# LinjianMa/pairwise-perturbation

Measured on AMD Instinct MI355X. Metric: ALS sweeps/sec (exact dimension-tree sweep, CP order-4 s=200 R=10), higher is better.
Workload: dtype f32

## Files before the change

__graft_entry__.py:

```python
import os
import subprocess
import sys

ROOT = os.path.dirname(os.path.abspath(__file__))
PKG = os.path.join(ROOT, "pairwise-perturbation_amd")


def _run(cmd, **kw):
    print("+", " ".join(cmd), flush=True)
    subprocess.check_call(cmd, **kw)


def build():
    jobs = str(min(8, os.cpu_count() or 1))
    _run(["make", "-j", jobs, "-C", PKG, "ARCH=gfx950"])
    _run(["make", "-C", os.path.join(ROOT, "oracle")])
    if os.path.isdir("/root/reference"):
        _run(["make", "-C", os.path.join(ROOT, "oracle"), "ref"])
    _run(["make", "-C", os.path.join(ROOT, "tests", "hostsim")])
    _run(["make", "-j", jobs, "-C", os.path.join(ROOT, "tests", "hipsim"), "ARCH=gfx950"])
    _run(["make", "-C", os.path.join(ROOT, "tests", "opshim")])
    _run(["make", "-C", os.path.join(ROOT, "tests", "slices_shim")])
    _run(["make", "-C", os.path.join(ROOT, "tests", "polar_shim")])
    _run(["make", "-C", os.path.join(ROOT, "tests", "shape_shim")])
    _run(["make", "-C", os.path.join(ROOT, "tests", "huber_shim")])
    _run(["make", "-C", os.path.join(ROOT, "tests", "parafac2_shim")])
    sys.path.insert(0, PKG)
    import ppals
    lib = ppals.lib()
    missing = [s for s in ppals.EXPORTS if not hasattr(lib, s)]
    if missing:
        raise RuntimeError(f"libppals.so lacks exported symbols: {missing}")
    print("built:", lib.ppals_version().decode(), flush=True)


def smoke():
    sys.path.insert(0, PKG)
    sys.path.insert(0, os.path.join(ROOT, "tests"))
    import numpy as np
    import ppals
    import oracle_lib as O

    lens, R = [24, 20, 16, 12], 5
    ctx = ppals.Context(0)
    Wt = ppals.init_factors(lens, R, 1000)
    W0 = ppals.init_factors(lens, R, 2000)
    G0 = ppals.init_factors(lens, R, 3000)
    V_ref = O.build_V(O.init_factors(lens, R, 1000))
    for dtype, tol in ((ppals.F32, 1e-5), (ppals.F64, 1e-9)):
        V = ppals.Tensor(ctx, lens, dtype).fill_cp(Wt)
        assert abs(V.norm() - np.linalg.norm(V_ref)) < 1e-6 * np.linalg.norm(V_ref)
        cp = ppals.CP(ctx, V, R)
        cp.set_factors(W0, G0)
        got = cp.tree_node("ab")
        want = O.tree_node(V_ref, W0, "ab").ravel(order="F")
        err = np.linalg.norm(got - want) / np.linalg.norm(want)
        assert err < (2e-6 if dtype == ppals.F32 else 1e-11), err
        cp.sweeps_dt(3)
        W = cp.get_factors()
        _, _, W_ref, _ = O.als_cp_dt(V_ref, W0, G0, tol=0.0, maxiter=2, resprint=10 ** 9)
        for a, b in zip(W, W_ref):
            e = np.linalg.norm(a - b) / np.linalg.norm(b)
            assert e < tol, (dtype, e)
        cp.close()
        V.close()
    ctx.close()
    print("smoke OK: HIP engine matches the fp64 oracle (f32 storage 1e-5, f64 storage 1e-9)")


if __name__ == "__main__":
    build()
    if len(sys.argv) > 1 and sys.argv[1] == "smoke":
        smoke()
```

pairwise-perturbation_amd/csrc/engine.cpp:

```cpp
#include "engine.h"
#include "assignment.h"
#include "run_report.h"

#include <algorithm>
#include <cmath>
#include <cstdio>
#include <cstdlib>
#include <cstring>
#include <fstream>
#include <iostream>
#include <limits>
#include <stdexcept>

namespace ppals {

int tensor_create(Ops &ops, Comm &comm, int order, const int64_t *glens, int dtype,
                  TensorDesc *out, std::string *err) {
  if (order < 2 || order > MAX_ORDER) {
    *err = "tensor order must be in [2, 8]";
    return -1;
  }
  if (!ops.supports_storage(dtype))
    throw Unsupported(dtype == BF16 ? "ppals: this back end cannot store a bf16 tensor"
                                    : "ppals: this back end cannot store this tensor type");
// ... 467 lines not shown
    for (int g = 0; g < f; g++) {
      const double ww = npls_ww(d, wall.data(), g, f);
      for (int64_t i = 0; i < I; i++) T[(size_t)(i + I * f)] -= T[(size_t)(i + I * g)] * ww;
    }
    for (int c = 0; c < M; c++) Q[(size_t)(c + M * f)] = q[(size_t)c];
    for (int64_t i = 0; i < I; i++) {
      double u = 0;
      for (int c = 0; c < M; c++) u += Yres[(size_t)(i + I * c)] * q[(size_t)c];
      Uy[(size_t)(i + I * f)] = u;
    }
    const int n = f + 1;
    std::vector<double> G((size_t)n * n), b((size_t)n);
    for (int g = 0; g < n; g++) {
      for (int h = 0; h < n; h++) G[g + (size_t)n * h] = dotn(&T[(size_t)I * g], &T[(size_t)I * h], I);
      b[(size_t)g] = dotn(&T[(size_t)I * g], &Uy[(size_t)I * f], I);
    }
    std::vector<double> TtT = G;
    solve_small(G, b, n);
    for (int g = 0; g < n; g++) B[g + (size_t)F * f] = b[(size_t)g];
    Yres.assign(Y, Y + (size_t)I * M);
    for (int h = 0; h < n; h++)
      for (int g = 0; g <= h; g++) {
        const double bgh = B[g + (size_t)F * h];
        if (bgh == 0) continue;
        for (int c = 0; c < M; c++) {
          const double bq = bgh * Q[(size_t)(c + M * h)];
          for (int64_t i = 0; i < I; i++) Yres[(size_t)(i + I * c)] -= T[(size_t)(i + I * g)] * bq;
        }
      }
    m.ssy.push_back(1.0 - dotn(Yres.data(), Yres.data(), I * M) / normY2);
    double res = normX2;
    for (int g = 0; g < n; g++) {
      res -= 2.0 * dotn(&T[(size_t)I * g], &S[(size_t)I * g], I);
      for (int h = 0; h < n; h++) res += TtT[g + (size_t)n * h] * npls_ww(d, wall.data(), g, h);
    }
    m.ssx.push_back(1.0 - res / normX2);
    m.status.push_back(status);
  }
  m.nf = f;
  m.T.assign(T.begin(), T.begin() + (size_t)I * f);
  m.U.assign(Uy.begin(), Uy.begin() + (size_t)I * f);
  m.Q.assign(Q.begin(), Q.begin() + (size_t)M * f);
  m.B.assign((size_t)f * f, 0.0);
  for (int g = 0; g < f; g++)
    for (int h = 0; h < f; h++) m.B[g + (size_t)f * h] = B[g + (size_t)F * h];
  m.W.resize((size_t)d.K);
  for (int k = 0; k < d.K; k++) {
    m.W[(size_t)k].resize((size_t)d.ext[k] * f);
    for (int g = 0; g < f; g++)
      std::copy(&wall[(size_t)(d.sum * g + d.off[k])], &wall[(size_t)(d.sum * g + d.off[k])] + d.ext[k],
                &m.W[(size_t)k][(size_t)d.ext[k] * g]);
  }
  *out = std::move(m);
}

void npls_predict(Ops &ops, const NplsModel &m, const TensorDesc &Xnew, int ncomp, double *Yhat, double *Tnew) {
  const PrepShape s = prep_shape(Xnew, m.mode);
  const int64_t I = s.J;
  const NplsDims d(m.order, m.lens, m.mode);
  const int k = ncomp;
  std::vector<double> wall((size_t)d.sum * k);
  for (int g = 0; g < k; g++)
    for (int j = 0; j < d.K; j++)
      std::copy(&m.W[(size_t)j][(size_t)d.ext[j] * g], &m.W[(size_t)j][(size_t)d.ext[j] * g] + d.ext[j],
                &wall[(size_t)(d.sum * g + d.off[j])]);
  DevBuf dwall(ops, d.sum * k), dW(ops, d.LT * k), dS(ops, I * k);
  ops.h2d(dwall.p, wall.data(), sizeof(double) * wall.size());
  for (int g = 0; g < k; g++) npls_outer(ops, d, dwall.p + d.sum * g, -1, dW.p + d.LT * g);
  ops.npls_slice_inner(Xnew.data, Xnew.dtype, s.L, I, s.T, dW.p, k, dS.p);
  std::vector<double> T((size_t)I * k);
  ops.d2h(T.data(), dS.p, sizeof(double) * T.size());
  for (int f = 0; f < k; f++)
    for (int g = 0; g < f; g++) {
      const double ww = npls_ww(d, wall.data(), g, f);
      for (int64_t i = 0; i < I; i++) T[(size_t)(i + I * f)] -= T[(size_t)(i + I * g)] * ww;
    }
  if (Tnew) std::copy(T.begin(), T.end(), Tnew);
  std::fill(Yhat, Yhat + (size_t)I * m.M, 0.0);
  for (int h = 0; h < k; h++)
    for (int g = 0; g <= h; g++) {
      const double bgh = m.B[g + (size_t)m.nf * h];
      if (bgh == 0) continue;
      for (int c = 0; c < m.M; c++) {
        const double bq = bgh * m.Q[(size_t)(c + m.M * h)];
        for (int64_t i = 0; i < I; i++) Yhat[(size_t)(i + I * c)] += T[(size_t)(i + I * g)] * bq;
      }
    }
}

static int total_columns(int R, int nstarts, const int *ranks) {
  if (!ranks) return R * nstarts;
  int t = 0;
  for (int b = 0; b < nstarts; b++) t += ranks[b];
  return t;
}

CpEngine::CpEngine(Ops &ops, Comm &comm, const TensorDesc &V, int R, int nstarts, bool multi, const int *ranks)
    : ops_(ops), comm_(comm), V_(V), N_(V.order), R_(total_columns(R, nstarts, ranks)), P_(comm.size()),
      rank_(comm.rank()), K_(nstarts), Rs_(R), multi_(multi || nstarts > 1 || ranks) {
  dist_ = P_ > 1 || (force_comm_path() && !comm.is_self());
  if (nstarts <= 0) throw std::runtime_error("ppals: the number of starts must be positive");
  if (multi_) {
    if (nstarts > kMaxStarts) throw std::runtime_error("ppals: too many starts");
    tab_.nstarts = nstarts;
    Rs_ = 0;
    for (int b = 0; b < nstarts; b++) {
      const int rb = ranks ? ranks[b] : R;
      if (rb <= 0) throw std::runtime_error("ppals: rank must be positive");
      tab_.col[b + 1] = tab_.col[b] + rb;
      tab_.sq[b + 1] = tab_.sq[b] + rb * rb;
      if (rb != tab_.rank(0)) ragged_ = true;
      Rs_ = std::max(Rs_, rb);
    }
  }
  if (Rs_ <= 0) throw std::runtime_error("ppals: rank must be positive");
  if (multi_ && dist_) throw Unsupported("ppals: a multi-start session runs on one rank");
  residual_form_ = residual_form_env();
  slice_work_cap_ = slice_work_cap_env();
  W_.resize(N_);
  gradW_.resize(N_);
  Wprev_.assign(N_, nullptr);
  Winit_.assign(N_, nullptr);
  dW_.assign(N_, nullptr);
  dM_.assign(N_, nullptr);
  Mm_.assign(N_, nullptr);
  for (int i = 0; i < N_; i++) {
    size_t n = (size_t)V_.glens[i] * R_ * sizeof(double);
    W_[i] = (double *)ops_.alloc(n);
    gradW_[i] = (double *)ops_.alloc(n);
    ops_.zero(W_[i], n);
    ops_.zero(gradW_[i], n);
    maxs_ = std::max(maxs_, V_.glens[i]);
    maxblk_ = std::max(maxblk_, block_rows(V_.glens[i], P_));
  }
  const size_t sys_n = multi_ ? (size_t)tab_.sq[K_] : (size_t)R_ * R_;
  G_ = (double *)ops_.alloc(sizeof(double) * N_ * sys_n);
  S_ = (double *)ops_.alloc(sizeof(double) * sys_n);
  Sinv_ = (double *)ops_.alloc(sizeof(double) * sys_n);
  gradsq_ = (double *)ops_.alloc(sizeof(double) * MAX_ORDER * K_);
  scal_ = (double *)ops_.alloc(sizeof(double) * 4 * MAX_ORDER);
  ops_.zero(gradsq_, sizeof(double) * MAX_ORDER * K_);
  if (dist_) {
    size_t n = sizeof(double) * (size_t)maxblk_ * P_ * R_;
    sendbuf_ = (double *)ops_.alloc(n);
    recvbuf_ = (double *)ops_.alloc(sizeof(double) * (size_t)maxblk_ * R_);
    gatherbuf_ = (double *)ops_.alloc(n);
    ops_.zero(sendbuf_, n);
    ops_.zero(gatherbuf_, n);
  }
  if (const char *e = std::getenv("PPALS_COMM_SMALL_BYTES")) small_msg_bytes_ = std::atoll(e);
  if (const char *e = std::getenv("PPALS_TEST_BLOCKED_UPDATE")) test_blocks_ = std::atoi(e);
  if (N_ < 3) schedule_ = 0;
  if (const char *e = std::getenv("PPALS_PLACE_TUNE")) ms_tune_enabled_ = std::atoi(e) != 0;
  if (const char *e = std::getenv("PPALS_PACK_LAYOUT")) pack_mode_ = std::atoi(e) == 0 ? 0 : (std::atoi(e) == 1 ? 1 : -1);
  if (N_ >= 3) {
    ms_set_roots(ms_choose_roots());
    ms_scales_ = (double *)ops_.alloc(sizeof(double) * 32);
  }
  if (V_.generation) tensor_gen_ = *V_.generation;
  {
    Layout nat;
    nat.ptr = V_.data;
    for (int m = 0; m < N_; m++) nat.order.push_back(m);
    lay_.push_back(nat);
  }
  size_t xmax = 0;
  const bool place = schedule_ == 1 && N_ >= 3 && ms_tune_enabled_ && ms_X_slack() > 0;
  if (place) {
    for (int r = 0; r < N_; r++) {
      if (ms_set_excluded(r, ms_k_, ms_excl_)) continue;
      xmax = std::max(xmax, ms_X_bytes(r, ms_k_));
    }
    const size_t avail = ops_.mem_available();
    const double tensor_bytes = (double)V_.nloc * dtype_size(V_.dtype);
    if (avail == (size_t)-1 || (double)avail > 2.0 * tensor_bytes + 6.0 * (double)(xmax + ms_X_slack()) + 8e9)
      ms_X_alt_ = ops_.try_alloc(xmax + ms_X_slack());
  }
  ensure_transposed();
  if (schedule_ == 1 && N_ >= 3)
    for (int r = 0; r < N_; r++) {
      ScanPlan pl;
      PackedSrc pk;
      if (!ms_set_excluded(r, ms_k_, ms_excl_) && plan_scan(r, ms_k_, false, pl) && pl.Lc > 1) packed_for(pl, pk);
    }
  if (place) {
    ms_X_base_ = big_alloc(xmax + ms_X_slack());
    ms_X_cap_ = xmax + ms_X_slack();
  }
  for (int i = 0; i < MAX_ORDER; i++) grad_replicated_[i] = !dist_;
  build_tree(0, N_ - 1, -1);
  leaf_.assign(N_, -1);
  for (size_t k = 0; k < nodes_.size(); k++)
    if (nodes_[k].lo == nodes_[k].hi) leaf_[nodes_[k].lo] = (int)k;
}

void CpEngine::set_schedule(int schedule) {
  if (schedule != 0 && schedule != 1) throw std::runtime_error("ppals: unknown sweep schedule");
  schedule_ = (N_ < 3) ? 0 : schedule;
  for (auto &n : nodes_) n.valid = false;
  ms_invalidate();
}

CpEngine::~CpEngine() {
  try {
    ops_.sync();
  } catch (...) {
  }
  for (auto p : W_) ops_.free(p);
  for (auto p : gradW_) ops_.free(p);
  for (auto p : Wprev_) ops_.free(p);
  for (auto p : Winit_) ops_.free(p);
  for (auto p : dW_) ops_.free(p);
  for (auto p : dM_) ops_.free(p);
  for (auto p : Mm_) ops_.free(p);
  for (auto &n : nodes_) ops_.free(n.buf);
  lr_release();
  pp_clear();
  for (auto &kv : pp_pool_) ops_.free(kv.second.buf);
  ops_.free(pp_norms_);
  ops_.free(G_);
  ops_.free(S_);
  ops_.free(Sinv_);
  ops_.free(gradsq_);
  ops_.free(scal_);
  ops_.free(sendbuf_);
  ops_.free(recvbuf_);
  ops_.free(gatherbuf_);
  ops_.free(test_blkbuf_);
  ops_.free(Mbuf_);
  ops_.free(Qbuf_);
  ops_.free(xq_);
  ops_.free(xp_);
  for (auto q : cc_P_) ops_.free(q);
  ops_.free(cc_flag_);
  ops_.free(cc_out_);
  ops_.free(cc_Y_.ptr);
  ops_.free(cc_chain_[0].ptr);
  ops_.free(cc_chain_[1].ptr);
  ops_.free(cc_core_.ptr);
  ops_.free(sl_row_.ptr);
  ops_.free(sl_col_.ptr);
  ops_.free(sl_out_.ptr);
  ops_.free(sl_work_.ptr);
  ops_.free(fms_out_.ptr);
  ops_.free(fms_work_.ptr);
  ops_.free(hold_keep_dev_);
  ops_.free(hold_scores_);
  ops_.free(Pbuf_);
  packs_release();
  for (auto &l : lay_)
    if (l.owned) ops_.free(l.ptr);
  for (auto &ex : ms_place_)
    if (ex.timer >= 0) ops_.timer_read(ex.timer);
  ops_.free(ms_X_base_);
  ops_.free(ms_X_alt_);
  ops_.free(ms_scales_);
  for (auto &n : ms_nodes_) {
    ops_.free(n.t.buf);
    for (auto &t : n.tmp) ops_.free(t.buf);
  }
}

static int64_t round_up(int64_t x, int64_t m) { return (x + m - 1) / m * m; }

void CpEngine::fill_layout(const Layout &l) {
  int h = l.order[0];
  const int64_t rows = h == 0 ? 1 : prod_ext(0, h - 1);
  const int64_t cols = h == 0 ? V_.nloc : prod_ext(h, N_ - 1);
  if (l.q == 0)
    ops_.transpose2d(V_.data, V_.dtype, rows, cols, l.ptr);
  else
    ops_.pad_layout(V_.data, V_.dtype, rows, cols, l.blk, l.ld, l.ptr);
}

bool CpEngine::optional_fits(size_t bytes) {
  const size_t esz = dtype_size(V_.dtype);
  int64_t min_ext = ext(0);
  for (int m = 1; m < N_; m++) min_ext = std::min(min_ext, ext(m));
  const size_t xbytes_max = (size_t)(V_.nloc / std::max<int64_t>(1, min_ext)) * R_ * esz;
  const size_t reserve = 3 * xbytes_max + ms_X_slack() + ((size_t)1 << 30);
  const size_t avail = ops_.mem_available();
  return avail == (size_t)-1 || avail >= bytes + reserve;
}

void CpEngine::ensure_transposed() {
  if (vt_state_ != 0) return;
  vt_state_ = -1;
  const char *env = std::getenv("PPALS_TRANSPOSED_COPY");
  if (env && std::atoi(env) == 0) return;
  if (N_ < 3) return;
  const size_t esz = dtype_size(V_.dtype);
  const int64_t line = 128 / (int64_t)esz;
  int pad_mode = -1;
  if (const char *e = std::getenv("PPALS_PAD_LAYOUT")) pad_mode = std::atoi(e);
  const double max_waste = pad_mode == 1 ? 100.0 : 0.03;
  const bool may_pad = pad_mode == 1 || (pad_mode != 0 && (double)V_.nloc * esz >= 1e8);
  auto choose_pad = [&](Layout &l, int qmax) {
    l.q = 0;
    if (!may_pad) return;
    int q_nat = N_;
    int64_t b = 1;
    for (int p = 1; p < N_; p++) {
      b *= ext(l.order[p - 1]);
      if (b % line == 0) {
        q_nat = p;
        break;
      }
    }
    b = 1;
    for (int q = 1; q < q_nat && q <= qmax; q++) {
      b *= ext(l.order[q - 1]);
      const int64_t ld = round_up(b, line);
      if ((double)(ld - b) <= max_waste * (double)b) {
        l.q = q;
        l.blk = b;
        l.ld = ld;
        return;
      }
    }
  };
  auto bytes_of = [&](const Layout &l) {
    return l.q ? (size_t)l.ld * (size_t)(V_.nloc / l.blk) * esz : (size_t)V_.nloc * esz;
  };
  const int mid = (N_ - 1) / 2;
  Layout t;
  for (int m = mid + 1; m < N_; m++) t.order.push_back(m);
  for (int m = 0; m <= mid; m++) t.order.push_back(m);
  choose_pad(t, std::min(N_ - 2, N_ - 1 - mid));
  auto fits = [&](size_t bytes) { return optional_fits(bytes); };
  if (!fits(bytes_of(t))) return;
  t.ptr = ops_.try_alloc(bytes_of(t));
  if (!t.ptr) return;
  t.owned = true;
  t.bytes = bytes_of(t);
  fill_layout(t);
  lay_.push_back(t);
  vt_state_ = 1;
  Layout a;
  for (int m = 0; m < N_; m++) a.order.push_back(m);
  choose_pad(a, N_ - 2);
  if (a.q > 0 && fits(bytes_of(a))) {
    a.ptr = ops_.try_alloc(bytes_of(a));
    if (a.ptr) {
      a.owned = true;
      a.bytes = bytes_of(a);
      fill_layout(a);
      lay_.push_back(a);
    }
  }
}

bool CpEngine::plan_scan(int first, int k, bool natural_only, ScanPlan &plan) {
  auto in_set = [&](int m) { return ((m - first + N_) % N_) < k; };
  const int64_t line = 128 / (int64_t)dtype_size(V_.dtype);
  const Layout *best = nullptr;
  int best_p0 = 0;
  int64_t best_L = 0;
  bool best_al = false;
  const size_t nlay = natural_only ? 1 : lay_.size();
  for (size_t li = 0; li < nlay; li++) {
    const Layout &l = lay_[li];
    int p0 = -1;
    for (int p = 0; p < N_; p++)
      if (in_set(l.order[p])) {
        p0 = p;
        break;
      }
    int len = 0;
    while (p0 + len < N_ && in_set(l.order[p0 + len])) len++;
    if (len != k || (l.q > 0 && p0 < l.q)) continue;
    int64_t L = 1;
    for (int p = 0; p < p0; p++) L *= ext(l.order[p]);
    const bool al = L >= 256 && (l.q > 0 || L % line == 0);
    if (!best || (al && !best_al) ||
        (al == best_al && (L > best_L || (L == best_L && l.q > 0 && best->q == 0)))) {
      best = &l;
      best_p0 = p0;
      best_L = L;
      best_al = al;
    }
  }
  if (!best) return false;
  plan = ScanPlan();
  plan.lay = best;
  for (int p = 0; p < N_; p++) {
    const int m = best->order[p];
    if (p < best_p0) {
      plan.Lc *= ext(m);
      plan.kept.push_back(m);
    } else if (p < best_p0 + k) {
      plan.J *= ext(m);
      plan.set.push_back(m);
    } else {
      plan.T *= ext(m);
      plan.kept.push_back(m);
    }
  }
  plan.L = plan.Lc;
  if (best->q > 0) {
    plan.L = plan.Lc / best->blk * best->ld;
    plan.pad.ld = best->ld;
    plan.pad.valid = best->blk;
  }
  return true;
}

namespace {
struct PackedScope {
  Ops &ops;
  PackedScope(Ops &o, const PackedSrc *pk) : ops(o) { ops.scan_packed_source(pk); }
  ~PackedScope() { ops.scan_packed_source(nullptr); }
};
}

void CpEngine::packs_release() {
  for (auto &t : packs_) {
    ops_.free(t.data);
    ops_.free(t.bases);
  }
  packs_.clear();
}

bool CpEngine::pack_fill(PackedTwin &t) {
  const int spread = ops_.pack_layout(t.src, V_.dtype, t.L, t.J, t.T, t.data, t.bases);
  if (spread >= 0 && spread < PACK_WINDOW) return true;
  ops_.free(t.data);
  ops_.free(t.bases);
  t.data = t.bases = nullptr;
  t.bytes = 0;
  t.reason = spread < 0 ? "scan shape has no packed route"
                        : "top bytes of a block span " + std::to_string(spread + 1) + " values (window 16)";
  return false;
}

const PackedSrc *CpEngine::packed_for(const ScanPlan &pl, PackedSrc &out) {
  if (pack_off_reason_.empty()) {
    if (pack_mode_ == 0) pack_off_reason_ = "PPALS_PACK_LAYOUT=0";
    else if (V_.dtype != F32) pack_off_reason_ = "not eligible: storage is not fp32";
    else if (R_ > 16) pack_off_reason_ = "not eligible: more than 16 result columns";
    else if (dist_) pack_off_reason_ = "not eligible: sharded session";
    else if (multi_) pack_off_reason_ = "not eligible: multi-start session";
    else if (pack_mode_ != 1 && (double)V_.nloc * 4.0 < 1e8) pack_off_reason_ = "tensor below 100 MB";
  }
  if (!pack_off_reason_.empty()) return nullptr;
  const int li = (int)(pl.lay - lay_.data());
  PackedTwin *t = nullptr;
  for (auto &c : packs_)
    if (c.layout == li && c.L == pl.L && c.J == pl.J && c.T == pl.T) t = &c;
  if (!t) {
    PackedTwin n;
    n.layout = li;
    n.src = pl.lay->ptr;
    n.L = pl.L;
    n.J = pl.J;
    n.T = pl.T;
    const size_t db = pack_data_bytes(n.L, n.J, n.T), bb = pack_base_bytes(n.L, n.J, n.T);
    if (pl.lay->q > 0) {
      n.reason = "padded layout";
    } else if (n.L < 4 || n.L % 4) {
      n.reason = "scan shape has no packed route";
    } else if (pack_mode_ != 1 && db + bb >= (size_t)n.L * (size_t)n.J * (size_t)n.T * 4) {
      n.reason = "row tiles would pad away what packing saves";
    } else if (!optional_fits(db + bb)) {
      n.reason = "no room beside what the session still allocates";
    } else {
      n.data = ops_.try_alloc(db);
      n.bases = n.data ? ops_.try_alloc(bb) : nullptr;
      if (!n.bases) {
        ops_.free(n.data);
        n.data = nullptr;
        n.reason = "allocation failed";
      } else {
        n.bytes = db + bb;
        pack_fill(n);
      }
    }
    packs_.push_back(n);
    t = &packs_.back();
  }
  if (!t->data) return nullptr;
  out.data = t->data;
  out.bases = t->bases;
  out.L = t->L;
  out.J = t->J;
  out.T = t->T;
  return &out;
}

void CpEngine::check_tensor_generation() {
  if (!V_.generation || *V_.generation == tensor_gen_) return;
  tensor_gen_ = *V_.generation;
  for (const auto &l : lay_)
    if (l.owned) fill_layout(l);
  if (++pack_regen_ >= 3) {
    ops_.sync();
    packs_release();
    if (pack_off_reason_.empty()) pack_off_reason_ = "tensor rewritten repeatedly";
  } else {
    ops_.sync();
    for (size_t k = 0; k < packs_.size();) {
      if (packs_[k].data && pack_fill(packs_[k])) {
        k++;
      } else if (packs_[k].data == nullptr && packs_[k].reason.compare(0, 9, "top bytes") != 0) {
        k++;
      } else {
        packs_.erase(packs_.begin() + k);
      }
    }
  }
  for (auto &n : nodes_) n.valid = false;
  ms_invalidate();
  pp_clear();
}

FactorRef CpEngine::fref(int m, double *const *W) const {
  FactorRef f;
  f.ptr = W[m] + (m == 0 ? V_.row0 : 0);
  f.rows = ext(m);
  f.ld = V_.glens[m];
  return f;
}
int64_t CpEngine::prod_ext(int lo, int hi) const {
  int64_t p = 1;
  for (int m = lo; m <= hi; m++) p *= ext(m);
  return p;
}

void CpEngine::build_tree(int lo, int hi, int parent) {
  if (hi <= lo) return;
  const int mid = (lo + hi) / 2;
  const int ranges[2][2] = {{lo, mid}, {mid + 1, hi}};
  int idx[2];
  for (int c = 0; c < 2; c++) {
    Node n;
    n.lo = ranges[c][0];
    n.hi = ranges[c][1];
    n.parent = parent;
    n.slo = ranges[1 - c][0];
    n.shi = ranges[1 - c][1];
    n.elems = 0;
    nodes_.push_back(n);
    idx[c] = (int)nodes_.size() - 1;
  }
  build_tree(lo, mid, idx[0]);
  build_tree(mid + 1, hi, idx[1]);
}
int CpEngine::find_node(int lo, int hi) const {
  for (size_t k = 0; k < nodes_.size(); k++)
    if (nodes_[k].lo == lo && nodes_[k].hi == hi) return (int)k;
  return -1;
}

void CpEngine::compute_node(int idx) {
  check_tensor_generation();
  Node &n = nodes_[idx];
  if (n.valid) return;
  n.elems = prod_ext(n.lo, n.hi);
  if (!n.buf) n.buf = (double *)ops_.alloc(sizeof(double) * (size_t)n.elems * R_);
  FactorRef f[MAX_ORDER];
  int nf = 0;
  for (int m = n.slo; m <= n.shi; m++) f[nf++] = fref(m, W_.data());
  const int64_t J = prod_ext(n.slo, n.shi);
  const bool sib_is_suffix = n.slo > n.hi;
  if (n.parent < 0) {
    ScanPlan pl;
    if (!plan_scan(n.slo, n.shi - n.slo + 1, false, pl))
      throw std::runtime_error("ppals: internal error (tree node not adjacent)");
    if (pl.Lc == 1 && !sib_is_suffix) {
      ops_.scan_contract(V_.data, V_.dtype, 1, J, n.elems, f, nf, R_, n.buf, F64, 1, n.elems);
    } else {
      if (pl.T != 1 || pl.Lc != n.elems || pl.J != J)
        throw std::runtime_error("ppals: internal error (tree node scan shape)");
      PackedSrc pk_store;
      PackedScope scope(ops_, packed_for(pl, pk_store));
      ops_.scan_contract(pl.lay->ptr, V_.dtype, pl.L, J, 1, f, nf, R_, n.buf, F64, n.elems, n.elems,
                         pl.pad);
    }
  } else {
    compute_node(n.parent);
    const Node &p = nodes_[n.parent];
    if (sib_is_suffix)
      ops_.mttv(p.buf, F64, n.elems, J, 1, f, nf, R_, n.buf, n.elems, 0, nullptr);
    else
      ops_.mttv(p.buf, F64, 1, J, n.elems, f, nf, R_, n.buf, n.elems, 0, nullptr);
  }
  n.valid = true;
}

void CpEngine::refresh_grams() {
  if (multi_ && ragged_) {
    for (int i = 0; i < N_; i++) ops_.gram_ragged(W_[i], V_.glens[i], V_.glens[i], tab_, N_, i, G_);
    return;
  }
  if (multi_) {
    for (int i = 0; i < N_; i++)
      ops_.gram_batched(W_[i], V_.glens[i], V_.glens[i], Rs_, K_, G_ + (size_t)i * Rs_ * Rs_,
                        (int64_t)N_ * Rs_ * Rs_);
    return;
  }
  for (int i = 0; i < N_; i++)
    ops_.gram(W_[i], V_.glens[i], V_.glens[i], R_, G_ + (size_t)i * R_ * R_);
}

void CpEngine::set_factors(const double *Wflat, const double *gradWflat) {
  if (multi_) throw std::logic_error("ppals: a multi-start session takes its factors start by start");
  const double *w = Wflat, *g = gradWflat;
  double gs = 0, gsi[MAX_ORDER] = {0};
  for (int i = 0; i < N_; i++) {
    size_t n = (size_t)V_.glens[i] * R_;
    ops_.h2d(W_[i], w, n * sizeof(double));
    w += n;
    if (g) {
      if (kind_[i] != kModeFixed) {
        ops_.h2d(gradW_[i], g, n * sizeof(double));
        for (size_t e = 0; e < n; e++) gsi[i] += g[e] * g[e];
        gs += gsi[i];
      }
      g += n;
    }
  }
  ops_.h2d(gradsq_, gsi, sizeof(double) * MAX_ORDER);
  for (int i = 0; i < MAX_ORDER; i++) grad_replicated_[i] = true;
  init_gradnorm_ = std::sqrt(gs);
  grad_from_sweep_ = false;
  refresh_grams();
  for (auto &n : nodes_) n.valid = false;
  ms_invalidate();
}

void CpEngine::set_nonneg(bool on) {
  if (on) {
    if (P_ > 1 || dist_) throw Unsupported("ppals: a non-negative session runs on one rank");
    if (Rs_ > 64) throw Unsupported("ppals: a non-negative session supports R <= 64");
    if (test_blocks_ > 1)
      throw Unsupported("ppals: PPALS_TEST_BLOCKED_UPDATE has no non-negative update");
// ... 1941 lines not shown
  return best;
}
std::string CpEngine::pp_parent(const std::string &seq) const {
  std::string p = seq;
  p.erase(p.find((char)('a' + pp_last_mode(seq))), 1);
  return p;
}

const CpEngine::PPOp &CpEngine::pp_get(const std::string &seq) {
  check_tensor_generation();
  auto it = pp_.find(seq);
  if (it != pp_.end()) return it->second;
  const int mode = pp_last_mode(seq);
  PPOp op;
  FactorRef f = fref(mode, W_.data());
  int64_t L = 1, T = 1;
  if (seq.size() == 1) {
    ScanPlan pl;
    if (!plan_scan(mode, 1, !(pp_fast_ && N_ >= 3), pl))
      throw std::runtime_error("ppals: internal error (single mode not adjacent)");
    L = pl.Lc;
    T = pl.T;
    op.modes = pl.kept;
    op.elems = L * T;
    op.dt = (pp_fast_ && N_ > 3) ? work_dt(V_.dtype) : F64;
    if (pp_fast_ && N_ > 3 && schedule_ == 1 && ms_k_ == 1 && ms_root_ == mode && ms_X_.valid &&
        ms_X_.dt == op.dt && !pp_no_borrow_) {
      op.buf = ms_X_.buf;
      op.owned = false;
      op.scale = ms_scale_of(ms_X_);
      op.modes = ms_X_.modes;
    } else {
      op.buf = pp_buffer(seq, dtype_size(op.dt) * (size_t)(V_.nloc / ext(mode)) * R_);
      if (!plan_scan(mode, 1, !(pp_fast_ && N_ >= 3), pl))
        throw std::runtime_error("ppals: internal error (single mode not adjacent)");
      L = pl.Lc;
      T = pl.T;
      op.modes = pl.kept;
      ops_.scan_contract(pl.lay->ptr, V_.dtype, pl.L, ext(mode), T, &f, 1, R_, op.buf, op.dt, L,
                         op.elems, pl.pad);
    }
  } else {
    const PPOp &par = pp_get(pp_parent(seq));
    bool before = true;
    for (int m : par.modes) {
      if (m == mode) {
        before = false;
        continue;
      }
      (before ? L : T) *= ext(m);
      op.modes.push_back(m);
    }
    op.elems = L * T;
    op.buf = pp_buffer(seq, sizeof(double) * (size_t)op.elems * R_);
    ops_.mttv(par.buf, par.dt, L, ext(mode), T, &f, 1, R_, (double *)op.buf, op.elems, 0, par.scale);
  }
  pp_[seq] = op;
  return pp_[seq];
}
void CpEngine::pp_contract_pair(const PPOp &T, int cmode, const FactorRef &f, double *out,
                                int64_t out_rows) {
  if (T.modes.size() != 2 || T.dt != F64) throw std::runtime_error("ppals: not a pair operator");
  if (T.modes[0] == cmode)
    ops_.mttv(T.buf, F64, 1, ext(cmode), ext(T.modes[1]), &f, 1, R_, out, out_rows, 1, nullptr);
  else
    ops_.mttv(T.buf, F64, ext(T.modes[0]), ext(cmode), 1, &f, 1, R_, out, out_rows, 1, nullptr);
}
void CpEngine::pp_clear() { pp_.clear(); }
void *CpEngine::pp_buffer(const std::string &seq, size_t bytes) {
  const bool scaffold = (int)seq.size() < N_ - 2;
  const std::string key = scaffold ? "#" + std::to_string(seq.size()) : seq;
  if (scaffold) {
    for (auto it = pp_.begin(); it != pp_.end();) {
      if (it->first.size() == seq.size() && it->second.owned) {
        it = pp_.erase(it);
      } else {
        ++it;
      }
    }
  }
  PPBuf &b = pp_pool_[key];
  if (b.cap < bytes) {
    ops_.free(b.buf);
    b.buf = nullptr;
    b.cap = 0;
    b.buf = big_alloc(bytes);
    b.cap = bytes;
  }
  return b.buf;
}
static std::string all_but(int N, int i, int j = -1) {
  std::string s;
  for (int m = 0; m < N; m++)
    if (m != i && m != j) s.push_back((char)('a' + m));
  return s;
}
void CpEngine::pp_build_all() {
  struct Timer {
    CpEngine &e;
    double t0 = 0;
    explicit Timer(CpEngine &eng) : e(eng) {
      e.pp_builds_++;
      if (e.pp_build_timed_) {
        e.ops_.sync();
        t0 = now();
      }
    }
    ~Timer() {
      if (e.pp_build_timed_) {
        try {
          e.ops_.sync();
        } catch (...) {
        }
        e.pp_build_s_ += now() - t0;
      }
    }
  } timer(*this);
  pp_clear();
  std::vector<std::pair<std::string, std::string>> pairs;
  for (int ii = 0; ii < N_; ii++)
    for (int jj = ii + 1; jj < N_; jj++) {
      const std::string key = all_but(N_, ii, jj);
      std::string chain = key;
      for (std::string k = key; k.size() > 1;) {
        k = pp_parent(k);
        chain = k + "|" + chain;
      }
      pairs.emplace_back(chain, key);
    }
  std::stable_sort(pairs.begin(), pairs.end(),
                   [](const std::pair<std::string, std::string> &a, const std::pair<std::string, std::string> &b) {
                     return a.first < b.first;
                   });
  for (const auto &pk : pairs) pp_get(pk.second);
  for (int ii = 0; ii < N_; ii++) pp_get(all_but(N_, ii));
  for (auto it = pp_.begin(); it != pp_.end();) {
    if ((int)it->first.size() < N_ - 2) {
      it = pp_.erase(it);
    } else {
      ++it;
    }
  }
  const size_t keep = (size_t)2 << 30;
  for (auto it = pp_pool_.begin(); it != pp_pool_.end();) {
    if (it->first[0] == '#' && it->second.cap > keep) {
      ops_.free(it->second.buf);
      it = pp_pool_.erase(it);
    } else {
      ++it;
    }
  }
}
std::string CpEngine::placement_report() const {
  char buf[400];
  std::string out = "{\"mode\": ";
  out += ms_tune_enabled_ && ms_X_slack() > 0 ? "\"online\"" : "\"off\"";
  out += ", \"setup_s\": 0.0, \"candidate_blocks_held\": ";
  out += ms_X_alt_ ? "2" : "1";
  out += ", \"roots\": [";
  bool firstrow = true;
  for (int r = 0; r < N_; r++) {
    const PlaceExplore &ex = ms_place_[r];
    if (ex.phase < 0 || ex.phase == 3 || ex.cands.empty()) continue;
    const PlaceCand *c = ex.chosen >= 0 ? &ex.cands[ex.chosen] : nullptr;
    double best = 1e300;
    for (const auto &q : ex.cands)
      if (q.samples > 0) best = std::min(best, q.best);
    snprintf(buf, sizeof buf,
             "%s{\"root\": %d, \"layout\": \"%s\", \"settled\": %s, \"visits\": %d, \"block\": %d, \"offset_mb\": %lld, "
             "\"store\": \"%s\", \"best_ms\": %.4f, \"worst_ms\": %.4f, \"gated\": %s}",
             firstrow ? "" : ", ", r, ex.layout == 1 ? "second (transposed) copy" : "tensor",
             ex.phase == 2 ? "true" : "false", ex.visits, c ? c->blk : 0, c ? (long long)(c->off >> 20) : 0LL,
             !c || c->nt < 0 ? "by size" : (c->nt == 1 ? "non-temporal" : "ordinary"),
             best < 1e299 ? best * 1e3 : 0.0, ex.worst * 1e3, ex.gated ? "true" : "false");
    out += buf;
    firstrow = false;
  }
  out += "]";
  out += ", \"packed\": {\"mode\": ";
  out += pack_mode_ == 0 ? "\"off\"" : (pack_mode_ == 1 ? "\"on\"" : "\"auto\"");
  out += ", \"refused\": \"" + pack_off_reason_ + "\", \"packed_scans\": " + std::to_string(ops_.scan_packed_launches()) +
         ", \"layouts\": [";
  for (size_t k = 0; k < packs_.size(); k++) {
    const PackedTwin &t = packs_[k];
    snprintf(buf, sizeof buf,
             "%s{\"layout\": \"%s\", \"rows\": %lld, \"reduced\": %lld, \"batches\": %lld, \"packed\": %s, "
             "\"bytes_per_element\": %.4f, \"reason\": \"%s\"}",
             k ? ", " : "", t.layout == 0 ? "tensor" : (t.layout == 1 ? "second (transposed) copy" : "padded copy"),
             (long long)t.L, (long long)t.J, (long long)t.T, t.data ? "true" : "false",
             t.data ? (double)t.bytes / ((double)t.L * (double)t.J * (double)t.T) : 4.0, t.reason.c_str());
    out += buf;
  }
  out += "]}}";
  return out;
}

int64_t CpEngine::pp_operator(const std::string &contracted, double *out_host) {
  for (size_t k = 0; k < contracted.size(); k++) {
    int m = contracted[k] - 'a';
    if (m < 0 || m >= N_ || (k > 0 && contracted[k] <= contracted[k - 1])) return -1;
  }
  if (contracted.empty() || (int)contracted.size() >= N_) return -1;
  pp_clear();
  struct Restore {
    CpEngine &e;
    bool fast;
    ~Restore() {
      e.pp_fast_ = fast;
      e.pp_no_borrow_ = false;
    }
  } restore{*this, pp_fast_};
  pp_no_borrow_ = true;
  const PPOp *op = &pp_get(contracted);
  if (op->dt != F64 || !std::is_sorted(op->modes.begin(), op->modes.end())) {
    pp_clear();
    pp_fast_ = false;
    op = &pp_get(contracted);
  }
  if (out_host) ops_.d2h(out_host, op->buf, sizeof(double) * (size_t)op->elems * R_);
  int64_t n = op->elems * R_;
  pp_clear();
  return n;
}

void CpEngine::sweep_pp(double lambda, double ratio) {
  if (nonneg()) throw Unsupported("ppals: a non-negative session has no pairwise-perturbation sweep");
  if (any_nonfree()) throw Unsupported("ppals: a session with constrained modes has no pairwise-perturbation sweep");
  ms_invalidate();
  if (!Mbuf_) Mbuf_ = (double *)ops_.alloc(sizeof(double) * (size_t)maxs_ * R_);
  if (!pp_norms_) {
    pp_norms_ = (double *)ops_.alloc(sizeof(double) * 2 * MAX_ORDER);
    ops_.zero(pp_norms_, sizeof(double) * 2 * MAX_ORDER);
  }
  bool norm_fused = false;
  for (int i = 0; i < N_; i++) {
    const int64_t si = ext(i);
    const PPOp &M0 = pp_get(all_but(N_, i));
    PPTerm terms[MAX_ORDER];
    int nt = 0;
    for (int ii = 0; ii < N_; ii++) {
      if (ii == i) continue;
      const PPOp &T = pp_get(all_but(N_, std::min(i, ii), std::max(i, ii)));
      if (T.modes.size() != 2 || T.dt != F64) throw std::runtime_error("ppals: not a pair operator");
      FactorRef f = fref(ii, dW_.data());
      terms[nt].T = (const double *)T.buf;
      terms[nt].ny = ext(ii);
      terms[nt].keep_first = T.modes[0] == i ? 1 : 0;
      terms[nt].dW = f.ptr;
      terms[nt].lddw = f.ld;
      nt++;
    }
    ops_.arm_gram_system(G_, N_, i, R_, lambda, S_, Sinv_);
    ops_.pp_correct((const double *)M0.buf, si, R_, terms, nt, Mbuf_);
    if (i == N_ - 1 && !dist_) {
      int64_t rows[MAX_ORDER];
      for (int q = 0; q < N_; q++) rows[q] = V_.glens[q];
      norm_fused = ops_.arm_normalize(W_.data(), rows, N_, R_, G_, i, pp_norms_ + 1);
    }
    mode_update(i, Mbuf_, si, lambda, true, ratio);
  }
  if (!norm_fused) {
    pp_norms_live_ = !dist_;
    normalize();
    pp_norms_live_ = false;
  }
  grad_from_sweep_ = true;
}

bool CpEngine::print_block(RunReport &rep, const CpOpts &o, int iter, int pp_flag, double &projnorm,
                           bool bench) {
  ops_.sync();
  double diffV = 0;
  rep.off_clock([&] {
    projnorm = gradnorm();
    diffV = residual();
  });
  if (!bench)
    rep.row(iter, projnorm, pp_flag, diffV);
  else if (pp_flag)
    rep.pp_bench_time(iter, o.maxiter);
  else if (iter != 0)
    rep.dt_bench_time();
  return agree(projnorm < o.tol || rep.elapsed() > o.timelimit);
}

int CpEngine::run_dt(const CpOpts &o, int *iters) {
  RunReport rep(o, rank_ == 0, V_.glens[0], "gradnorm");
  double projnorm = 0;
  int iter;
  for (iter = 0; iter <= o.maxiter; iter++) {
    if (iter % o.resprint == 0 || iter == o.maxiter) {
      if (print_block(rep, o, iter, 0, projnorm, o.bench)) break;
    }
    sweep_dt(o.lambda);
    rep.dot(iter);
  }
  ops_.sync();
  rep.finish(iter, "proj-grad", projnorm);
  if (iters) *iters = iter;
  return iter == o.maxiter + 1 ? 0 : 1;
}

ModeNorms CpEngine::read_norms(bool dt_phase) {
  int64_t n[MAX_ORDER];
  for (int i = 0; i < N_; i++) n[i] = V_.glens[i] * R_;
  ops_.diff_norms(W_.data(), dt_phase ? Wprev_.data() : nullptr, n, N_, dt_phase, dW_.data(),
                  dt_phase, scal_);
  return ModeNorms(ops_, scal_, N_);
}

void CpEngine::dt_sub(RunReport &rep, const CpOpts &o, double &projnorm, int &iter) {
  for (int i = 0; i < N_; i++)
    ops_.zero(Wprev_[i], sizeof(double) * V_.glens[i] * R_);
  for (; iter <= o.maxiter; iter++) {
    if (iter % o.resprint == 0 || iter == o.maxiter) {
      if (print_block(rep, o, iter, 0, projnorm, false)) break;
    }
    sweep_dt(o.lambda);
    if (read_norms(true).count(o.tol_init, false) == N_) return;
    rep.dot(iter);
  }
}

void CpEngine::pp_restart() {
  for (int j = 0; j < N_; j++) {
    size_t n = sizeof(double) * V_.glens[j] * R_;
    ops_.d2d(Winit_[j], W_[j], n);
    ops_.zero(dW_[j], n);
  }
  pp_build_all();
}

void CpEngine::pp_sub(RunReport &rep, const CpOpts &o, double &projnorm, int &iter) {
  const int init_iter = iter;
  rep.start_pp_phase();
  for (; iter <= o.maxiter; iter++) {
    int num_dw_break = 0;
    if (!o.bench) {
      const bool fused = iter != init_iter && !dist_ && pp_norms_;
      const ModeNorms m = fused ? ModeNorms(ops_, pp_norms_, N_) : read_norms(false);
      num_dw_break = m.count(o.tol_init, true);
    }
    if ((iter - init_iter) % 15 == 0 || num_dw_break > 0) {
// ... 118 lines not shown
```

pairwise-perturbation_amd/csrc/engine.h:

```cpp
#pragma once
#include <cstdint>
#include <cstdlib>
#include <functional>
#include <map>
#include <string>
#include <vector>

#include "ops.h"

namespace ppals {

struct TensorDesc {
  int order = 0;
  int64_t glens[MAX_ORDER];
  int64_t llens[MAX_ORDER];
  int64_t row0 = 0;
  int dtype = F32;
  void *data = nullptr;
  int64_t nloc = 0;
  uint64_t *generation = nullptr;
  uint64_t *prep_epoch = nullptr;
};

inline int64_t block_rows(int64_t s, int P) { return (s + P - 1) / P; }
// ... 268 lines not shown
  void ms_mode_update(int i, double lambda, bool last_of_sweep = false);
  bool ms_norm_fused_ = false;
  unsigned ms_collect_scales(unsigned *masks, unsigned *fresh, int skip_node);
  RTensor ms_X_;
  struct PlaceCand {
    int blk = 0;
    int64_t off = 0;
    int nt = -1;
    double best = 1e300;
    int samples = 0;
  };
  struct PlaceExplore {
    int phase = -1;
    size_t next = 0;
    int timer = -1;
    int timer_cand = -1;
    int chosen = -1;
    int layout = 0;
    double worst = 0;
    int visits = 0;
    bool gated = false;
    std::vector<PlaceCand> cands;
  };
  static constexpr int kPlaceGateSamples = 8;
  static constexpr double kPlaceGateSpread = 0.04;
  PlaceExplore ms_place_[MAX_ORDER];
  void ms_place_collect(PlaceExplore &ex);
  int ms_place_pick(PlaceExplore &ex);
  void *ms_X_base_ = nullptr;
  void *ms_X_alt_ = nullptr;
  void ms_place_release_unchosen();
  size_t ms_X_cap_ = 0;
  int64_t pp_builds_ = 0;
  double pp_build_s_ = 0;
  bool pp_build_timed_ = false;
  bool ms_tune_enabled_ = true;
  size_t ms_X_slack() const;
  static double place_min_bytes();
  size_t ms_X_bytes(int first, int k) const;
  void *big_alloc(size_t bytes);
  std::vector<MsNode> ms_nodes_;
  void lr_step_begin(int left, bool reuse, int r);
  void lr_mode_update(int i, double lambda, int r, const double *base);
  void lr_release();
  void *lr_cache_[MAX_ORDER] = {nullptr};
  bool lr_have_[MAX_ORDER] = {false};
  bool lr_random_ = false;
  uint64_t lr_random_calls_ = 0;
  RTensor lr_desc_[MAX_ORDER];
  void *ms_X_override_ = nullptr;
  double *lr_X_ = nullptr, *lr_Us_ = nullptr, *lr_G2_ = nullptr, *lr_small_ = nullptr;
  double *lr_T_ = nullptr;
  size_t lr_T_cap_ = 0;


  std::vector<int> ms_order_;
  std::vector<int> ms_leaf_;
  double *ms_scales_ = nullptr;
  const double *ms_scale_of(const RTensor &t) const { return t.pending ? ms_scales_ + t.slot : nullptr; }

  int64_t ext(int m) const { return m == 0 ? V_.llens[0] : V_.glens[m]; }
  FactorRef fref(int m, double *const *W) const;
  int64_t prod_ext(int lo, int hi) const;
  void build_tree(int lo, int hi, int parent);
  int find_node(int lo, int hi) const;
  void compute_node(int idx);
  void refresh_grams();
  void mode_update(int i, const double *M, int64_t ldm, double lambda, bool pp, double ratio);
  void normalize();
  const PPOp &pp_get(const std::string &seq);
  int pp_last_mode(const std::string &seq) const;
  std::string pp_parent(const std::string &seq) const;
  void pp_contract_pair(const PPOp &T, int cmode, const FactorRef &f, double *out, int64_t out_rows);
  bool pp_fast_ = true;
  bool pp_no_borrow_ = false;
  void pp_clear();
  void pp_build_all();
  void sweep_pp(double lambda, double ratio);
  double allreduce_scalar(double x);
  bool agree(bool local);
  ModeNorms read_norms(bool dt_phase);
  bool print_block(RunReport &rep, const CpOpts &o, int iter, int pp_flag, double &projnorm,
                   bool bench);
  void dt_sub(RunReport &rep, const CpOpts &o, double &projnorm, int &iter);
  void pp_restart();
  void pp_sub(RunReport &rep, const CpOpts &o, double &projnorm, int &iter);
  void pp_partupdate_sub(RunReport &rep, const CpOpts &o, double &projnorm, int &iter);
  int run_pp_common(const CpOpts &o, int *iters, bool partupdate);

  Ops &ops_;
  Comm &comm_;
  TensorDesc V_;
  int N_, R_, P_, rank_;
  int K_ = 1, Rs_ = 0;
  StartTable tab_;
  bool ragged_ = false;
  bool multi_ = false;
  int kind_[MAX_ORDER] = {0};
  int shape_[MAX_ORDER] = {0};
  void drop_stale_shapes() {
    for (int i = 0; i < N_; i++)
      if (kind_[i] != kModeNonneg) shape_[i] = kShapeNone;
  }
  bool any_fixed() const {
    for (int i = 0; i < N_; i++)
      if (kind_[i] == kModeFixed) return true;
    return false;
  }
  int hold_mode_ = -1;
  std::vector<uint8_t> hold_keep_;
  uint8_t *hold_keep_dev_ = nullptr;
  unsigned hold_mask_ = 0;
  double *hold_scores_ = nullptr;
  int64_t hold_rows_ = 0;
  void hold_apply(unsigned starts);
  bool dist_ = false;
  std::vector<double *> W_, gradW_, Wprev_, Winit_, dW_, dM_, Mm_;
  double *G_ = nullptr;
  double *S_ = nullptr, *Sinv_ = nullptr;
  double *gradsq_ = nullptr;
  double *scal_ = nullptr;
  double *sendbuf_ = nullptr, *recvbuf_ = nullptr, *gatherbuf_ = nullptr;
  double *Mbuf_ = nullptr;
  double *Qbuf_ = nullptr, *Pbuf_ = nullptr;
  double *xq_ = nullptr, *xp_ = nullptr;
  int64_t xq_cap_ = 0, xp_cap_ = 0;
  int residual_form_ = RESIDUAL_FUSED;
  std::vector<double *> cc_P_;
  int *cc_flag_ = nullptr;
  double *cc_out_ = nullptr;
  struct GrowBuf {
    void *ptr = nullptr;
    size_t cap = 0;
  };
  GrowBuf cc_Y_, cc_chain_[2], cc_core_;
  GrowBuf sl_row_, sl_col_, sl_out_, sl_work_;
  size_t slice_work_cap_ = (size_t)256 << 20;
  GrowBuf fms_out_, fms_work_;
  StartTable start_table() const;
  void *cc_reserve(GrowBuf &b, size_t bytes);
  struct Layout {
    void *ptr = nullptr;
    std::vector<int> order;
    int q = 0;
    int64_t blk = 0, ld = 0;
    bool owned = false;
    size_t bytes = 0;
  };
  std::vector<Layout> lay_;
  struct PackedTwin {
    int layout = 0;
    const void *src = nullptr;
    int64_t L = 0, J = 0, T = 0;
    void *data = nullptr, *bases = nullptr;
    size_t bytes = 0;
    std::string reason;
  };
  std::vector<PackedTwin> packs_;
  int pack_mode_ = -1;
  int pack_regen_ = 0;
  std::string pack_off_reason_;
  bool optional_fits(size_t bytes);
  bool pack_fill(PackedTwin &t);
  void packs_release();
  int vt_state_ = 0;
  uint64_t tensor_gen_ = 0;
  void ensure_transposed();
  void fill_layout(const Layout &l);
  struct ScanPlan {
    const Layout *lay = nullptr;
    int64_t L = 1, Lc = 1, J = 1, T = 1;
    RowPad pad;
    std::vector<int> set, kept;
  };
  bool plan_scan(int first, int k, bool natural_only, ScanPlan &plan);
  const PackedSrc *packed_for(const ScanPlan &pl, PackedSrc &out);
  void check_tensor_generation();
  void model_operands(const ModelBox &bx, ModelPlan &mp);
  void shard_groups(const ModelBox &bx, const int64_t *second, ModelPlan &mp) const;
  void side_step(const char *what, const ViewArgs &a, const void *data, const ViewArgs *w, const void *weights,
                 void *stream, double c, double *out);
  template <typename Step>
  int em_loop(Step &&step, const CpOpts &o, int inner_sweeps, double rel_change, int *iters, double *res);
  int64_t small_msg_bytes_ = 1 << 20;
  bool grad_replicated_[MAX_ORDER];
  int64_t maxs_ = 0, maxblk_ = 0;
  std::vector<Node> nodes_;
  std::vector<int> leaf_;
  std::map<std::string, PPOp> pp_;
  bool grad_from_sweep_ = false;
  double init_gradnorm_ = 0;
};

}
```

pairwise-perturbation_amd/csrc/hip_ops.hip:

```cpp
#include <dlfcn.h>
#include <hip/hip_runtime.h>
#include <chrono>

#include <algorithm>
#include <cstdio>
#include <cstdlib>
#include <stdexcept>
#include <string>
#include <map>
#include <type_traits>
#include <vector>

#include "hip_ops.h"
#include "roctx_ranges.h"
#include "preload_policy.h"
#include "kernels_scan.hip.h"
#include "kernels_pack.hip.h"
#include "kernels_small.hip.h"
#include "kernels_nn.hip.h"
#include "kernels_polar.hip.h"
#include "kernels_shape.hip.h"
#include "kernels_holdout.hip.h"
#include "kernels_corcondia.hip.h"
#include "kernels_fms.hip.h"
// ... 50 lines not shown
}

struct EigLibs {
  void *blas = nullptr, *solver = nullptr;
};
static bool g_hip_runtime_up = false;
static EigLibs &eig_libs() {
  static EigLibs l;
  if (l.blas && l.solver) return l;
  switch (late_preload_policy(false, g_hip_runtime_up, getenv("PPALS_STRICT_PRELOAD"))) {
    case kPreloadRefuse: throw Unsupported(late_preload_message());
    case kPreloadWarn: fprintf(stderr, "%s\n", late_preload_message()); fflush(stderr); break;
    default: break;
  }
  l.blas = dlopen("librocblas.so.5", RTLD_NOW | RTLD_GLOBAL);
  if (!l.blas) l.blas = dlopen("librocblas.so", RTLD_NOW | RTLD_GLOBAL);
  l.solver = dlopen("librocsolver.so.0", RTLD_NOW | RTLD_GLOBAL);
  if (!l.solver) l.solver = dlopen("librocsolver.so", RTLD_NOW | RTLD_GLOBAL);
  if (!l.blas || !l.solver)
    throw std::runtime_error(std::string("ppals: cannot load rocSOLVER: ") + dlerror());
  return l;
}

class HipOps : public Ops {
 public:
  explicit HipOps(int device) {
    int ndev = 0;
    hipError_t e = hipGetDeviceCount(&ndev);
    if (e != hipSuccess || ndev <= 0)
      throw std::runtime_error(
          "ppals: no HIP device available (the engine has no CPU fallback; hipGetDeviceCount: " +
          std::string(e == hipSuccess ? "0 devices" : hipGetErrorString(e)) + ")");
    if (device < 0 || device >= ndev)
      throw std::runtime_error("ppals: device index out of range");
    dev_ = device;
    g_hip_runtime_up = true;
    HIP_CHECK(hipSetDevice(dev_));
    HIP_CHECK(hipStreamCreateWithFlags(&st_, hipStreamNonBlocking));
    hipDeviceProp_t prop;
    HIP_CHECK(hipGetDeviceProperties(&prop, dev_));
    ncu_ = prop.multiProcessorCount;
    HIP_CHECK(hipFuncSetAttribute((const void *)k_gram_system,
                                  hipFuncAttributeMaxDynamicSharedMemorySize, 96 * 1024));
    HIP_CHECK(hipFuncSetAttribute((const void *)k_cp_update,
                                  hipFuncAttributeMaxDynamicSharedMemorySize, 96 * 1024));
    HIP_CHECK(hipFuncSetAttribute((const void *)k_top_eig_small,
                                  hipFuncAttributeMaxDynamicSharedMemorySize, 152 * 1024));
    HIP_CHECK(hipFuncSetAttribute((const void *)k_cp_mode_update<false, false>,
                                  hipFuncAttributeMaxDynamicSharedMemorySize, 152 * 1024));
    HIP_CHECK(hipFuncSetAttribute((const void *)k_cp_mode_update<true, true>,
                                  hipFuncAttributeMaxDynamicSharedMemorySize, 152 * 1024));
    HIP_CHECK(hipFuncSetAttribute((const void *)k_cp_mode_update_batched<false, false>,
                                  hipFuncAttributeMaxDynamicSharedMemorySize, 152 * 1024));
    HIP_CHECK(hipFuncSetAttribute((const void *)k_cp_mode_update_batched<true, true>,
                                  hipFuncAttributeMaxDynamicSharedMemorySize, 152 * 1024));
    HIP_CHECK(hipFuncSetAttribute((const void *)k_cp_mode_update_ragged<false, false>,
                                  hipFuncAttributeMaxDynamicSharedMemorySize, 152 * 1024));
    HIP_CHECK(hipFuncSetAttribute((const void *)k_cp_mode_update_ragged<true, true>,
                                  hipFuncAttributeMaxDynamicSharedMemorySize, 152 * 1024));
    if (const char *v = getenv("PPALS_FORCE_JACOBI")) force_jacobi_ = atoi(v);
    if (const char *v = getenv("PPALS_EIG_FAST")) {
      eig_fast_ = atoi(v);
      eig_cold_ = eig_fast_ != 2;
    }
    if (const char *v = getenv("PPALS_EIG_DEBUG")) eig_debug_ = atoi(v);
    if (const char *v = getenv("PPALS_EIG_SIGMA_SCALE")) eig_sigma_scale_ = atof(v);
    if (const char *v = getenv("PPALS_FORCE_EIGINV")) force_eiginv_ = atoi(v);
    HIP_CHECK(hipFuncSetAttribute((const void *)k_chol_rinv,
                                  hipFuncAttributeMaxDynamicSharedMemorySize, 72 * 1024));
    HIP_CHECK(hipFuncSetAttribute((const void *)k_chol_m,
                                  hipFuncAttributeMaxDynamicSharedMemorySize, 152 * 1024));
    HIP_CHECK(hipFuncSetAttribute((const void *)k_rr_apply,
                                  hipFuncAttributeMaxDynamicSharedMemorySize, 152 * 1024));
    if (const char *v = getenv("PPALS_SYM_LDS_MIN")) sym_lds_min_ = std::max(32, atoi(v));
    if (const char *v = getenv("PPALS_EIG_DEFER")) {
      eig_defer_ok_ = atoi(v);
      handover_ok_ = eig_defer_ok_ != 2;
    }
    if (const char *v = getenv("PPALS_EIG_DEFER_FAIL")) eig_defer_fail_ = atoi(v);
    if (const char *v = getenv("PPALS_SCAN_TAIL")) scan_tail_on_ = atoi(v) != 0;
    if (const char *v = getenv("PPALS_SCAN_WIDE")) wide_enabled_ = atoi(v) != 0;
    if (const char *v = getenv("PPALS_COLD_SUBSPACE_FROM")) cold_subspace_from_ = std::max(65, atoi(v));
    if (const char *v = getenv("PPALS_PERSIST_MULT")) persist_mult_ = std::max(1, atoi(v));
    HIP_CHECK(hipFuncSetAttribute((const void *)k_rmult_chol,
                                  hipFuncAttributeMaxDynamicSharedMemorySize, 152 * 1024));
    HIP_CHECK(hipFuncSetAttribute((const void *)k_jacobi_onesided,
                                  hipFuncAttributeMaxDynamicSharedMemorySize, 152 * 1024));
    HIP_CHECK(hipFuncSetAttribute((const void *)k_rr_small,
                                  hipFuncAttributeMaxDynamicSharedMemorySize, 152 * 1024));
    HIP_CHECK(hipFuncSetAttribute((const void *)k_gram_system_lds,
                                  hipFuncAttributeMaxDynamicSharedMemorySize, 152 * 1024));
    HIP_CHECK(hipFuncSetAttribute((const void *)k_gram_system_mfma,
                                  hipFuncAttributeMaxDynamicSharedMemorySize, 152 * 1024));
    const int mw_max = (int)mw_lds_bytes(MW_KMAX);
    HIP_CHECK(hipFuncSetAttribute((const void *)k_model_impute_wide<float, false>,
                                  hipFuncAttributeMaxDynamicSharedMemorySize, mw_max));
    HIP_CHECK(hipFuncSetAttribute((const void *)k_model_impute_wide<float, true>,
                                  hipFuncAttributeMaxDynamicSharedMemorySize, mw_max));
    HIP_CHECK(hipFuncSetAttribute((const void *)k_model_impute_wide<double, false>,
                                  hipFuncAttributeMaxDynamicSharedMemorySize, mw_max));
    HIP_CHECK(hipFuncSetAttribute((const void *)k_model_impute_wide<double, true>,
                                  hipFuncAttributeMaxDynamicSharedMemorySize, mw_max));
    const int wl_max = (int)wl_lds_bytes(WL_KMAX, sizeof(double));
    HIP_CHECK(hipFuncSetAttribute((const void *)k_model_wls<float, float>,
                                  hipFuncAttributeMaxDynamicSharedMemorySize, wl_max));
    HIP_CHECK(hipFuncSetAttribute((const void *)k_model_wls<float, double>,
                                  hipFuncAttributeMaxDynamicSharedMemorySize, wl_max));
    HIP_CHECK(hipFuncSetAttribute((const void *)k_model_wls<double, float>,
                                  hipFuncAttributeMaxDynamicSharedMemorySize, wl_max));
    HIP_CHECK(hipFuncSetAttribute((const void *)k_model_wls<double, double>,
                                  hipFuncAttributeMaxDynamicSharedMemorySize, wl_max));
    const void *huber_kernels[] = {
        (const void *)k_model_huber<float, float>,      (const void *)k_model_huber<float, double>,
        (const void *)k_model_huber<double, float>,     (const void *)k_model_huber<double, double>,
        (const void *)k_model_huber_now<float, float>,  (const void *)k_model_huber_now<float, double>,
        (const void *)k_model_huber_now<double, float>, (const void *)k_model_huber_now<double, double>,
        (const void *)k_model_absres_hist<float, true>, (const void *)k_model_absres_hist<float, false>,
        (const void *)k_model_absres_hist<double, true>, (const void *)k_model_absres_hist<double, false>};
    for (const void *k : huber_kernels)
      HIP_CHECK(hipFuncSetAttribute(k, hipFuncAttributeMaxDynamicSharedMemorySize,
                                    wl_max + (int)(sizeof(uint32_t) * WL_HIST_BINS)));
    HIP_CHECK(hipFuncSetAttribute((const void *)k_prep_rows<float, 4, 16, PREP_CENTER, true>,
                                  hipFuncAttributeMaxDynamicSharedMemorySize, 64 * 1024));
    HIP_CHECK(hipFuncSetAttribute((const void *)k_prep_rows<bf16s, 4, 16, PREP_CENTER, true>,
                                  hipFuncAttributeMaxDynamicSharedMemorySize, 64 * 1024));
    HIP_CHECK(hipFuncSetAttribute((const void *)k_prep_rows<double, 2, 16, PREP_CENTER, true>,
                                  hipFuncAttributeMaxDynamicSharedMemorySize, 64 * 1024));
    if (const char *v = getenv("PPALS_GJ_SCALAR")) gj_scalar_ = atoi(v);
    HIP_CHECK(hipFuncSetAttribute((const void *)k_fms_cross, hipFuncAttributeMaxDynamicSharedMemorySize,
                                  (int)fms_lds_bytes(FMS_MAXC, FMS_MAXC, false)));
    HIP_CHECK(hipFuncSetAttribute((const void *)k_polar_factor, hipFuncAttributeMaxDynamicSharedMemorySize,
                                  96 * 1024));
    HIP_CHECK(hipFuncSetAttribute((const void *)k_shape_columns, hipFuncAttributeMaxDynamicSharedMemorySize,
                                  (int)kShapeLdsBytes));
    HIP_CHECK(hipFuncSetAttribute((const void *)k_p2_polar, hipFuncAttributeMaxDynamicSharedMemorySize, 96 * 1024));
    const void *p2_wide[] = {(const void *)k_p2_project<float, 4>, (const void *)k_p2_project<double, 4>};
    for (const void *k : p2_wide)
      HIP_CHECK(hipFuncSetAttribute(k, hipFuncAttributeMaxDynamicSharedMemorySize, (int)p2_project_lds(64)));
  }
  ~HipOps() override {
    hipSetDevice(dev_);
    hipStreamSynchronize(st_);
    if (st2_) hipStreamSynchronize(st2_);
    for (auto &ev : events_) {
      hipEventDestroy(ev.a);
      hipEventDestroy(ev.b);
    }
    for (auto &t : timers_) {
      hipEventDestroy(t.a);
      hipEventDestroy(t.b);
    }
    if (ws_mttv_) hipFree(ws_mttv_);
    if (ws_pack_) hipFree(ws_pack_);
    if (pack_spread_) hipFree(pack_spread_);
    if (ws_mv_) hipFree(ws_mv_);
    if (ws_hist_) hipFree(ws_hist_);
    if (ws_slab_) hipFree(ws_slab_);
    if (ws_krp_) hipFree(ws_krp_);
    if (ws_part_) hipFree(ws_part_);
    if (ws_small_) hipFree(ws_small_);
    if (ws_big_) hipFree(ws_big_);
    if (ws_big2_) hipFree(ws_big2_);
    if (ws_eig_) hipFree(ws_eig_);
    if (ws_orth_) hipFree(ws_orth_);
    if (ws_pow_) hipFree(ws_pow_);
    if (ws_cold_) hipFree(ws_cold_);
    if (ws_cold2_) hipFree(ws_cold2_);
    if (ws_cholm_) hipFree(ws_cholm_);
    if (ws_gsfb_) hipFree(ws_gsfb_);
    if (ws_jac_) hipFree(ws_jac_);
    if (eig_host_) hipHostFree(eig_host_);
    if (ws_part2_) hipFree(ws_part2_);
    for (auto &kv : eig_state_) {
      if (kv.second.Q) hipFree(kv.second.Q);
      if (kv.second.Qn) hipFree(kv.second.Qn);
      free_lazy(kv.second);
    }
    for (auto &kv : eig_small_)
      if (kv.second.Q) hipFree(kv.second.Q);
    if (st2_) hipStreamDestroy(st2_);
    if (handover_) hipFree(handover_);
    if (io_ev_in_) hipEventDestroy(io_ev_in_);
    if (io_ev_out_) hipEventDestroy(io_ev_out_);
    hipStreamDestroy(st_);
  }

  void *alloc(size_t bytes) override {
    void *p = nullptr;
    HIP_CHECK(hipSetDevice(dev_));
    HIP_CHECK(hipMalloc(&p, bytes ? bytes : 8));
    return p;
  }
  void free(void *p) override {
    if (p) {
      hipStreamSynchronize(st_);
      hipFree(p);
    }
  }
  void h2d(void *dst, const void *src, size_t bytes) override {
    HIP_CHECK(hipMemcpyAsync(dst, src, bytes, hipMemcpyHostToDevice, st_));
    HIP_CHECK(hipStreamSynchronize(st_));
  }
  void d2h(void *dst, const void *src, size_t bytes) override {
    HIP_CHECK(hipMemcpyAsync(dst, src, bytes, hipMemcpyDeviceToHost, st_));
    HIP_CHECK(hipStreamSynchronize(st_));
  }
  void d2d(void *dst, const void *src, size_t bytes) override {
    HIP_CHECK(hipMemcpyAsync(dst, src, bytes, hipMemcpyDeviceToDevice, st_));
  }
  void zero(void *p, size_t bytes) override { HIP_CHECK(hipMemsetAsync(p, 0, bytes, st_)); }
  void sync() override { HIP_CHECK(hipStreamSynchronize(st_)); }
  void *stream() override { return (void *)st_; }
  void bind() override { HIP_CHECK(hipSetDevice(dev_)); }
  bool supports_storage(int dt) override { return dt == F32 || dt == F64 || dt == BF16; }

  void fill_uniform(void *V, int dt, int64_t l0, int64_t g0, int64_t row0, int64_t rest,
                    uint64_t seed, double lo, double hi) override {
    int64_t n = l0 * rest;
    int g = grid_for(n, 256, 16384);
    if (dt == F32)
      hipLaunchKernelGGL(k_fill_uniform<float>, dim3(g), dim3(256), 0, st_, (float *)V, l0, g0,
                         row0, rest, seed, lo, hi);
    else if (dt == BF16)
      hipLaunchKernelGGL(k_fill_uniform<bf16s>, dim3(g), dim3(256), 0, st_, (bf16s *)V, l0, g0,
                         row0, rest, seed, lo, hi);
    else
      hipLaunchKernelGGL(k_fill_uniform<double>, dim3(g), dim3(256), 0, st_, (double *)V, l0, g0,
                         row0, rest, seed, lo, hi);
    HIP_CHECK(hipGetLastError());
  }

  void fill_laplacian(void *V, int dt, int64_t l0, int64_t g0, int64_t row0, int64_t rest,
                      int ndigits, int s) override {
    int g = grid_for(l0 * rest, 256, 16384);
    if (dt == F32)
      hipLaunchKernelGGL(k_fill_laplacian<float>, dim3(g), dim3(256), 0, st_, (float *)V, l0, g0,
                         row0, rest, ndigits, s);
    else if (dt == BF16)
      hipLaunchKernelGGL(k_fill_laplacian<bf16s>, dim3(g), dim3(256), 0, st_, (bf16s *)V, l0, g0,
                         row0, rest, ndigits, s);
    else
      hipLaunchKernelGGL(k_fill_laplacian<double>, dim3(g), dim3(256), 0, st_, (double *)V, l0, g0,
                         row0, rest, ndigits, s);
    HIP_CHECK(hipGetLastError());
  }
  void add_uniform_noise(void *V, int dt, int64_t l0, int64_t g0, int64_t row0, int64_t rest,
                         uint64_t seed, double lo, double hi, double alpha) override {
    int g = grid_for(l0 * rest, 256, 16384);
    if (dt == F32)
      hipLaunchKernelGGL((k_uniform_noise<float, 0>), dim3(g), dim3(256), 0, st_, (float *)V, l0,
                         g0, row0, rest, seed, lo, hi, alpha, (double *)nullptr);
    else if (dt == BF16)
      hipLaunchKernelGGL((k_uniform_noise<bf16s, 0>), dim3(g), dim3(256), 0, st_, (bf16s *)V, l0,
                         g0, row0, rest, seed, lo, hi, alpha, (double *)nullptr);
    else
      hipLaunchKernelGGL((k_uniform_noise<double, 0>), dim3(g), dim3(256), 0, st_, (double *)V, l0,
                         g0, row0, rest, seed, lo, hi, alpha, (double *)nullptr);
    HIP_CHECK(hipGetLastError());
  }
  void uniform_sumsq(int64_t l0, int64_t g0, int64_t row0, int64_t rest, uint64_t seed, double lo,
                     double hi, double *out) override {
    int g = grid_for(l0 * rest, 256, 4096);
    double *part = (double *)ensure(ws_part_, ws_part_sz_, sizeof(double) * g);
    hipLaunchKernelGGL((k_uniform_noise<double, 1>), dim3(g), dim3(256), 0, st_, (double *)nullptr,
                       l0, g0, row0, rest, seed, lo, hi, 0.0, part);
    hipLaunchKernelGGL(k_sum_partials, dim3(1), dim3(1024), 0, st_, part, g, out);
    HIP_CHECK(hipGetLastError());
  }

  struct RankPlan {
    int nkb, nchunk, per, rem, RB;
    int64_t n_mtiles;
  };
  template <typename TV>
  bool rank_plan(int mode, const void *V, int64_t M, int64_t K, int R, RankPlan &pl) {
    constexpr int VEC = ScanTraits<TV>::VEC;
    if (R > 32 || M % VEC != 0 || M < VEC || (((uintptr_t)V) & 15) != 0 || K < 1)
      return false;
    const int64_t nkb64 = (K + 15) / 16;
    if (nkb64 > 0x7fffffff) return false;
    const int nkb = (int)nkb64;
    const int64_t n_mtiles = (M + 64 * VEC - 1) / (64 * VEC);
    const KSplit ks = k_split(nkb, std::min<int64_t>(nkb, ((int64_t)ncu_ * 16 + n_mtiles - 1) / n_mtiles),
                              std::min(nkb, 8));
    const int nchunk = ks.nsplit, per = (int)ks.per;
    if (n_mtiles > 0x7fffffff || nchunk > 65535) return false;
    int rem = ((mode == 1 || mode == 3) && R > 4 && R <= 17 && (R % 4 == 1 || (R % 4 == 2 && R <= 10))) ? R % 4 : 0;
    if (sizeof(double) * (size_t)per * 16 * rem > 48 * 1024) rem = 0;
    pl = {nkb, nchunk, per, rem, mode == 2 ? 1 : (R - rem + 3) / 4, n_mtiles};
    return true;
  }
  template <typename TV, int MODE>
  bool rank_mfma(void *V, int64_t M, int64_t K, const double *Q, const double *P, int R,
                 double *out) {
    RankPlan pl;
    if (!rank_plan<TV>(MODE, V, M, K, R, pl)) return false;
    const int nkb = pl.nkb, nchunk = pl.nchunk, per = pl.per, rem = pl.rem, RB = pl.RB;
    const int64_t n_mtiles = pl.n_mtiles;
    double *Ppk = nullptr;
    if (MODE != 2) {
      Ppk = (double *)ensure(ws_pack_, ws_pack_sz_, sizeof(double) * (size_t)nkb * RB * 64);
      hipLaunchKernelGGL(k_rank_pack, dim3(grid_for((int64_t)nkb * RB * 64, 256)), dim3(256), 0, st_,
                         P, K, R - rem, RB, nkb, Ppk);
    }
    dim3 grid((unsigned)n_mtiles, (unsigned)nchunk);
    double *part = nullptr;
    const int64_t npart = (int64_t)n_mtiles * nchunk;
// ... 939 lines not shown
    const bool a_unit = hist || mp.ga.view_unit();
    bool vec_st = a_unit && A % vw == 0 && (hist || (mp.voff % vw == 0 && ((uintptr_t)j.V) % 16 == 0));
    for (int i = 0; i < mp.gb.n && !hist; i++)
      if (mp.gb.len[i] > 1 && mp.gb.vs[i] % vw != 0) vec_st = false;
    int flags = (a_unit ? WL_A_UNIT : 0) | (vec_st ? WL_VEC_ST : 0);
    flags |= wls_side_flags(mp.ga, mp.gb, mp.ga.rs, mp.gb.rs, mp.roff, j.data, vw, vec_st, WL_X_ALONG_A, WL_X_UNIT,
                            WL_X_VEC);
    if (j.ws)
      flags |= wls_side_flags(mp.ga, mp.gb, j.ws->ga.vs, j.ws->gb.vs, j.ws->off, j.weights, vw, vec_st, WL_H_ALONG_A,
                              WL_H_UNIT, WL_H_VEC);
    const bool one_b = j.ws && !(flags & WL_X_ALONG_A) != !(flags & WL_H_ALONG_A);
    const size_t lds = wl_lds_bytes(K, one_b ? (j.vdt == DV_F32 ? 4 : 8) : 0) +
                       (hist ? sizeof(uint32_t) * WL_HIST_BINS : 0);
    const int64_t ntA = (A + MV_TILE - 1) / MV_TILE, ntB = (B + MV_TILE - 1) / MV_TILE;
    if (ntA > 0x7fffffff) throw std::runtime_error("ppals: model view too wide");
    const int nt = j.ws ? 3 : 2;
    int64_t *tab = (int64_t *)ensure(ws_mv_, ws_mv_sz_, sizeof(int64_t) * nt * (size_t)(A + B));
    hipLaunchKernelGGL(k_model_offsets, dim3(grid_for(A, 256)), dim3(256), 0, st_, mp.ga, tab, tab + A);
    if (j.ws) hipLaunchKernelGGL(k_model_offsets_side, dim3(grid_for(A, 256)), dim3(256), 0, st_, j.ws->ga, tab + 2 * A);
    hipLaunchKernelGGL(k_model_offsets, dim3(grid_for(B, 256)), dim3(256), 0, st_, mp.gb, tab + nt * A,
                       tab + nt * A + B);
    if (j.ws)
      hipLaunchKernelGGL(k_model_offsets_side, dim3(grid_for(B, 256)), dim3(256), 0, st_, j.ws->gb, tab + 3 * A + 2 * B);
    HIP_CHECK(hipGetLastError());
    const int64_t want = std::max<int64_t>(1, ((int64_t)ncu_ * 2 * wl_wgs_per_cu(lds) + ntA - 1) / ntA);
    const dim3 grid((unsigned)ntA, (unsigned)std::min<int64_t>(std::min<int64_t>(want, ntB), 65535));
    const int64_t npart = (int64_t)grid.x * grid.y;
    if (npart * nout > 0x7fffffff) throw std::runtime_error("ppals: model view too wide");
    double *part = hist ? nullptr : (double *)ensure(ws_part_, ws_part_sz_, sizeof(double) * npart * nout);
    const char *vn = j.vdt == DV_F32 ? "f32" : "f64";
    if (hist)
      route("model.absres_hist.%s%s K=%d flags=%d lds=%zu shift=%d", vn, j.ws ? "" : ".now", K, flags, lds, j.shift);
    else
      route("model.%s.%s.%s%s K=%d flags=%d lds=%zu", j.kind == WL_WLS ? "wls" : "huber", j.dt == F32 ? "f32" : "f64", vn,
            j.ws ? "" : ".now", K, flags, lds);
    if (!io_ev_in_) {
      HIP_CHECK(hipEventCreateWithFlags(&io_ev_in_, hipEventDisableTiming));
      HIP_CHECK(hipEventCreateWithFlags(&io_ev_out_, hipEventDisableTiming));
    }
    hipStream_t cs = (hipStream_t)caller_stream;
    HIP_CHECK(hipEventRecord(io_ev_in_, cs));
    HIP_CHECK(hipStreamWaitEvent(st_, io_ev_in_, 0));
    if (sdt == F32 && j.vdt == DV_F32)
      wl_launch<float, float>(j, grid, lds, Q, P, K, mp, tab, flags, part);
    else if (sdt == F32)
      wl_launch<float, double>(j, grid, lds, Q, P, K, mp, tab, flags, part);
    else if (j.vdt == DV_F32)
      wl_launch<double, float>(j, grid, lds, Q, P, K, mp, tab, flags, part);
    else
      wl_launch<double, double>(j, grid, lds, Q, P, K, mp, tab, flags, part);
    HIP_CHECK(hipGetLastError());
    HIP_CHECK(hipEventRecord(io_ev_out_, st_));
    HIP_CHECK(hipStreamWaitEvent(cs, io_ev_out_, 0));
    for (int i = 0; j.out && i < nout; i++) {
      hipLaunchKernelGGL(k_sum_partials, dim3(1), dim3(1024), 0, st_, part + i * npart, (int)npart, j.out + i);
      HIP_CHECK(hipGetLastError());
    }
  }
  void model_wls(const ModelPlan &plan, const ModelSide &ws, const double *Q, const double *P, int K,
                 const void *data, const void *weights, int vdt, void *V, int dt, double *sumsq,
                 void *caller_stream) override {
    wl_run(WlJob{WL_WLS, &ws, data, weights, vdt, V, dt, 0.0, sumsq, 0, 0, 0, 0, nullptr}, "model_wls", plan, Q, P, K,
           caller_stream);
  }
  void model_huber(const ModelPlan &plan, const ModelSide *ws, const double *Q, const double *P, int K,
                   const void *data, const void *weights, int vdt, void *V, int dt, double c, double *loss_clipped,
                   void *caller_stream) override {
    wl_run(WlJob{WL_HUBER, ws, data, ws ? weights : nullptr, vdt, V, dt, c, loss_clipped, 0, 0, 0, 0, nullptr},
           "model_huber", plan, Q, P, K, caller_stream);
  }
  void model_absres_hist(const ModelPlan &plan, const ModelSide *ws, const double *Q, const double *P, int K,
                         const void *data, const void *weights, int vdt, int pshift, uint32_t prefix, int shift,
                         uint32_t mask, uint64_t *hist , void *caller_stream) override {
    static_assert(sizeof(unsigned long long) == sizeof(uint64_t), "");
    HIP_CHECK(hipSetDevice(dev_));
    unsigned long long *gh =
        (unsigned long long *)ensure(ws_hist_, ws_hist_sz_, sizeof(unsigned long long) * WL_HIST_BINS);
    zero(gh, sizeof(unsigned long long) * WL_HIST_BINS);
    wl_run(WlJob{WL_HIST, ws, data, ws ? weights : nullptr, vdt, nullptr, 0, 0.0, nullptr, pshift, shift, prefix, mask,
                 gh},
           "model_absres_hist", plan, Q, P, K, caller_stream);
    d2h(hist, gh, sizeof(unsigned long long) * WL_HIST_BINS);
  }

  void parafac2_check() override {}
  void parafac2_init(double *P, int64_t I, int R, int64_t K) override {
    HIP_CHECK(hipSetDevice(dev_));
    hipLaunchKernelGGL(k_p2_init, dim3(grid_for(I * R * K, 256)), dim3(256), 0, st_, P, I, R, K);
    HIP_CHECK(hipGetLastError());
  }
  template <typename TX, int NT>
  void p2_launch(const Parafac2Step &s, int ti, int tj, double *part) {
    const TX *X = (const TX *)s.X;
    hipLaunchKernelGGL((k_p2_project<TX, NT>), dim3((unsigned)(ti * s.K)), dim3(256), p2_project_lds(s.R), st_, X, s.s1,
                       s.s2, s.I, s.J, s.R, s.A, s.B, s.C, s.K, ti, s.Q);
    const size_t lds_polar = sizeof(double) * (2 * (size_t)s.R * (s.R + 1) + 64 + 18) + sizeof(int) * 64;
    hipLaunchKernelGGL(k_p2_polar, dim3((unsigned)s.K), dim3(1024), lds_polar, st_, s.Q, s.I, s.R, s.min_ratio, s.T,
                       s.status);
    hipLaunchKernelGGL(k_p2_apply, dim3((unsigned)(ti * s.K)), dim3(256),
                       sizeof(double) * ((size_t)s.R * s.R + 64 * (size_t)s.R), st_, s.Q, s.T, s.status, s.I, s.R, ti,
                       s.P);
    if (s.dt == F32)
      hipLaunchKernelGGL((k_p2_compress<TX, float, NT>), dim3((unsigned)(tj * s.K)), dim3(256), p2_compress_lds(s.R),
                         st_, X, s.s1, s.s2, s.I, s.J, s.R, s.P, tj, (float *)s.Y, part);
    else
      hipLaunchKernelGGL((k_p2_compress<TX, double, NT>), dim3((unsigned)(tj * s.K)), dim3(256), p2_compress_lds(s.R),
                         st_, X, s.s1, s.s2, s.I, s.J, s.R, s.P, tj, (double *)s.Y, part);
  }
  void parafac2_step(const Parafac2Step &s, void *caller_stream) override {
    HIP_CHECK(hipSetDevice(dev_));
    if (s.R < 2 || s.R > 64 || s.I < s.R || s.J < s.R || s.K < 1)
      throw std::runtime_error("ppals: parafac2_step needs 2 <= R <= min(64, I, J) and K >= 1");
    if ((s.dt != F32 && s.dt != F64) || (s.vdt != DV_F32 && s.vdt != DV_F64))
      throw std::runtime_error("ppals: parafac2_step stores F32 or F64 and reads an F32 or F64 view");
    const int64_t ti = (s.I + P2_TILE - 1) / P2_TILE, tj = (s.J + P2_TILE - 1) / P2_TILE;
    if (ti * s.K > 0x7fffffff || tj * s.K > 0x3fffffff) throw std::runtime_error("ppals: parafac2_step: too many tiles");
    const int64_t npart = tj * s.K;
    double *part = (double *)ensure(ws_part_, ws_part_sz_, sizeof(double) * 2 * npart);
    const int nt = (s.R + 15) / 16;
    route("parafac2.step.%s.%s R=%d nt=%d tiles=%dx%d lds=%zu,%zu", s.dt == F32 ? "f32" : "f64",
          s.vdt == DV_F32 ? "f32" : "f64", s.R, nt, (int)ti, (int)tj, p2_project_lds(s.R), p2_compress_lds(s.R));
    join_stream(caller_stream);
    dispatch<1, 2, 3, 4>(nt, [&](auto NT) {
      if (s.vdt == DV_F32)
        p2_launch<float, NT()>(s, (int)ti, (int)tj, part);
      else
        p2_launch<double, NT()>(s, (int)ti, (int)tj, part);
    });
    HIP_CHECK(hipGetLastError());
    release_stream(caller_stream);
    if (s.out) {
      hipLaunchKernelGGL(k_sum_partials, dim3(1), dim3(1024), 0, st_, part, (int)npart, s.out);
      hipLaunchKernelGGL(k_sum_partials, dim3(1), dim3(1024), 0, st_, part + npart, (int)npart, s.out + 1);
      hipLaunchKernelGGL(k_p2_failed, dim3(1), dim3(1024), 0, st_, s.status, s.K, s.out + 2);
      HIP_CHECK(hipGetLastError());
    }
  }

  void *try_alloc(size_t bytes) override {
    void *p = nullptr;
    hipSetDevice(dev_);
    if (hipMalloc(&p, bytes ? bytes : 8) != hipSuccess) {
      (void)hipGetLastError();
      return nullptr;
    }
    return p;
  }
  void scan_store_mode(int mode) override { scan_nt_mode_ = mode; }
  void scan_packed_source(const PackedSrc *pk) override {
    scan_pk_ = pk ? *pk : PackedSrc();
  }
  PackedSrc scan_pk_;
  int64_t scan_pk_launches_ = 0;
  int64_t scan_packed_launches() override { return scan_pk_launches_; }
  int *pack_spread_ = nullptr;
  int pack_layout(const void *src, int dt, int64_t L, int64_t J, int64_t T, void *data, void *bases) override {
    const int64_t n_mtiles = (L + 255) / 256, nkb = (J + 15) / 16;
    if (dt != F32 || L < 4 || L % 4 || J < 1 || T < 1 || (((uintptr_t)src) & 15) || n_mtiles * T > 0x7fffffff ||
        n_mtiles * T * nkb > 0x7fffffff)
      return -1;
    if (!pack_spread_) pack_spread_ = (int *)alloc(sizeof(int));
    const unsigned nblocks = (unsigned)(n_mtiles * T * nkb);
    HIP_CHECK(hipMemsetAsync(pack_spread_, 0, sizeof(int), st_));
    hipLaunchKernelGGL(k_pk_prepass, dim3(nblocks), dim3(256), 0, st_, (const float *)src, L, J, (int)n_mtiles,
                       (int)nkb, (pk_u32 *)bases, pack_spread_);
    HIP_CHECK(hipGetLastError());
    int spread = 0;
    HIP_CHECK(hipMemcpyAsync(&spread, pack_spread_, sizeof(int), hipMemcpyDeviceToHost, st_));
    HIP_CHECK(hipStreamSynchronize(st_));
    if (spread >= PACK_WINDOW) return spread;
    hipLaunchKernelGGL(k_pk_pack, dim3(nblocks), dim3(256), 0, st_, (const float *)src, L, J, (int)n_mtiles, (int)nkb,
                       pack_tile_bytes(J), (const pk_u32 *)bases, (char *)data);
    HIP_CHECK(hipGetLastError());
    HIP_CHECK(hipStreamSynchronize(st_));
    return spread;
  }
  void scan_profile_slot(int slot) override { scan_slot_ = slot == 1 ? 1 : 0; }
  int scan_nt_mode_ = -1;
  size_t mem_available() override {
    size_t fr = 0, tot = 0;
    hipSetDevice(dev_);
    if (hipMemGetInfo(&fr, &tot) != hipSuccess) {
      (void)hipGetLastError();
      return (size_t)-1;
    }
    return fr;
  }
  void unpack_shards(const void *stage, int dt, int64_t s0, int64_t rest, int64_t blk, int P,
                     int64_t chunk_bytes, void *full) override {
    const int g = grid_for(s0 * rest, 256, 16384);
    if (dt == F32)
      hipLaunchKernelGGL(k_unpack_shards<float>, dim3(g), dim3(256), 0, st_, (const char *)stage,
                         s0, rest, blk, P, chunk_bytes, (float *)full);
    else if (dt == BF16)
      hipLaunchKernelGGL(k_unpack_shards<bf16s>, dim3(g), dim3(256), 0, st_, (const char *)stage,
                         s0, rest, blk, P, chunk_bytes, (bf16s *)full);
    else
      hipLaunchKernelGGL(k_unpack_shards<double>, dim3(g), dim3(256), 0, st_, (const char *)stage,
                         s0, rest, blk, P, chunk_bytes, (double *)full);
    HIP_CHECK(hipGetLastError());
  }
  void transpose2d(const void *src, int dt, int64_t rows, int64_t cols, void *dst) override {
    transpose_batched(src, dt, rows, cols, 1, dst);
  }
  void transpose_batched(const void *src, int dt, int64_t rows, int64_t cols, int64_t batch,
                         void *dst) override {
    const int64_t nb = ((rows + 63) / 64) * ((cols + 63) / 64);
    if (nb > 0x7fffffff) throw std::runtime_error("ppals: transpose grid too large");
    const size_t step = (size_t)rows * cols * dtype_size(dt);
    for (int64_t b0 = 0; b0 < batch; b0 += 65535) {
      const unsigned nby = (unsigned)std::min<int64_t>(65535, batch - b0);
      const char *s = (const char *)src + b0 * step;
      char *d = (char *)dst + b0 * step;
      if (dt == F32)
        hipLaunchKernelGGL(k_transpose<float>, dim3((unsigned)nb, nby), dim3(256), 0, st_,
                           (const float *)s, rows, cols, (float *)d);
      else if (dt == BF16)
        hipLaunchKernelGGL(k_transpose<bf16s>, dim3((unsigned)nb, nby), dim3(256), 0, st_,
                           (const bf16s *)s, rows, cols, (bf16s *)d);
      else
        hipLaunchKernelGGL(k_transpose<double>, dim3((unsigned)nb, nby), dim3(256), 0, st_,
                           (const double *)s, rows, cols, (double *)d);
    }
    HIP_CHECK(hipGetLastError());
  }

  static KrpArgs krp_args(const FactorRef *f, int nf, int64_t *J) {
    KrpArgs a;
    int64_t j = 1;
    if (nf > MAX_ORDER) throw std::runtime_error("ppals: too many Khatri-Rao factors");
    for (int i = 0; i < nf; i++) {
      a.ptr[i] = f[i].ptr;
      a.rows[i] = f[i].rows;
      a.ld[i] = f[i].ld;
      j *= f[i].rows;
    }
    a.nf = nf;
    *J = j;
    return a;
  }
  void krp(double *out, const FactorRef *f, int nf, int col0, int ncols) override {
    int64_t J;
    KrpArgs a = krp_args(f, nf, &J);
    hipLaunchKernelGGL(k_krp, dim3(grid_for(J * ncols, 256)), dim3(256), 0, st_, out, a, J, col0,
                       ncols);
    HIP_CHECK(hipGetLastError());
  }

  template <typename TV>
  void scan_t(const TV *V, int64_t L, int64_t J, int64_t T, const FactorRef *f, int nf, int R,
              double *out, int64_t out_tstride, int64_t out_rstride, int out32, RowPad pad) {
    constexpr int VEC = ScanTraits<TV>::VEC;
    int64_t Jc;
    KrpArgs a = krp_args(f, nf, &Jc);
    if (Jc != J) throw std::runtime_error("ppals: scan_contract factor extents do not match J");
    if (pad.ld && (L % pad.ld || pad.ld % VEC || pad.valid > pad.ld || pad.valid <= 0 || L == 1))
      throw std::runtime_error("ppals: scan_contract padded rows inconsistent");
    const bool aligned_base = (((uintptr_t)V) & 15) == 0;
    const bool wide_ok = sizeof(TV) == 4 && wide_enabled_ && L > 1 && aligned_base && (L % 4 == 0) &&
                         L >= 4 && (double)L * J * T >= 1.0e6 && 16.0 * (double)L * 4.0 < 2.0e9 &&
                         ((double)J / 16.0 + 1.0) * 8.0 * 1024.0 < 2.0e9;
    int col_step = 64;
    for (int col0 = 0; col0 < R; col0 += col_step) {
      if (wide_ok && R - col0 > 64) {
        col_step = std::min(128, R - col0);
        if constexpr (sizeof(TV) == 4)
          scan_wide((const float *)V, L, J, T, a, col0, col_step, out, out_tstride, out_rstride, out32, pad);
        continue;
      }
      col_step = 64;
      const int ncols = std::min(64, R - col0);
      const int NT = ncols <= 16 ? 1 : (ncols <= 32 ? 2 : (ncols <= 48 ? 3 : 4));
      const int64_t nblk64 = (J + 4 * VEC - 1) / (4 * VEC);
      if (nblk64 > 0x7fffffff) throw std::runtime_error("ppals: contraction extent too large");
      const int nblk = (int)nblk64;
      const size_t pack_bytes = (size_t)nblk * NT * 4 * 16 * VEC * sizeof(TV);
      TV *P = (TV *)ensure(ws_pack_, ws_pack_sz_, pack_bytes);
      const bool prefix = (L == 1);
      hipLaunchKernelGGL(k_krp_pack<TV>, dim3(grid_for((int64_t)nblk * NT * 64 * VEC, 256)),
                         dim3(256), 0, st_, P, nblk, NT, prefix ? 1 : 0, a, J, col0, ncols);
      HIP_CHECK(hipGetLastError());
      double *o = out32 ? (double *)((float *)out + (int64_t)col0 * out_rstride)
                        : out + (int64_t)col0 * out_rstride;
      const double bytes = (double)L * (double)J * (double)T * sizeof(TV) +
                           (double)L * (double)T * ncols * (out32 ? 4.0 : 8.0);
      if (prefix) {
        const int64_t M = J, K = T;
        const bool al = aligned_base && (M % VEC == 0);
        const int64_t ncolgrp = (K + 63) / 64;
        int want = 1;
        const int target = ncu_ * 4;
        if (ncolgrp < target) want = (int)std::min<int64_t>((target + ncolgrp - 1) / ncolgrp,
                                                            std::max(1, nblk / 64));
        const KSplit ks = k_split(nblk, want);
        const int nsplit = ks.nsplit, per = (int)ks.per;
        double *dst = o;
        int dst32 = out32;
        int64_t dst_ks = out_tstride, dst_ns = out_rstride, dst_ss = 0;
        if (nsplit > 1) {
          dst32 = 0;
          dst = (double *)ensure(ws_slab_, ws_slab_sz_, sizeof(double) * nsplit * ncols * K);
          dst_ks = 1;
          dst_ns = K;
          dst_ss = (int64_t)ncols * K;
        }
        if (al && M >= VEC)
          route("scan.%s.prefix.fast nt=%d nsplit=%d out32=%d", tname<TV>(), NT, nsplit, out32);
        else
          route("scan.%s.prefix.generic al=%d nt=%d nsplit=%d out32=%d", tname<TV>(), al ? 1 : 0, NT, nsplit, out32);
        dim3 grid((unsigned)ncolgrp, (unsigned)nsplit);
        dim3 grid_il((unsigned)((K + 15) / 16), (unsigned)nsplit);
        prof_begin(scan_slot_, bytes);
        dispatch<1, 2, 3, 4>(NT, [&](auto nt) {
          if (al && M >= VEC)
            hipLaunchKernelGGL((k_scan_prefix_fast<TV, nt, 12>), grid_il, dim3(256), 0, st_, V, M, K, P, per,
                               nblk, dst, dst_ks, dst_ns, dst_ss, ncols, dst32);
          else
            dispatch<true, false>(al, [&](auto alv) {
              hipLaunchKernelGGL((k_scan_prefix<TV, nt, alv, 4>), grid, dim3(256), 0, st_, V, M, K, P, per,
                                 nblk, dst, dst_ks, dst_ns, dst_ss, ncols, dst32);
            });
        });
        prof_end();
        HIP_CHECK(hipGetLastError());
        slab_combine(nsplit, dst, dst_ss, K, ncols, o, out_tstride, out_rstride, out32);
      } else {
        const int64_t M = L, K = J;
        const bool al = aligned_base && (M % VEC == 0);
        const int64_t n_mtiles64 = (M + 64 * VEC - 1) / (64 * VEC);
        const int n_mtiles = (int)n_mtiles64;
        int want = 1;
        const int target = ncu_ * 8;
        if (T == 1 && n_mtiles < target)
          want = (int)std::min<int64_t>((target + n_mtiles - 1) / n_mtiles,
                                        std::max(1, nblk / 32));
        else if (T > 1 && n_mtiles64 * T < ncu_ && (double)M * T * ncols * nblk / 4 * 8.0 < 64e6)
          want = (int)std::min<int64_t>(((int64_t)ncu_ * 2 + n_mtiles64 * T - 1) / (n_mtiles64 * T),
                                        std::max(1, nblk / 4));
        const KSplit ks = k_split(nblk, want);
        const int nsplit = ks.nsplit, per = (int)ks.per;
        const PassDst d = pass_dst(nsplit, M, T, ncols, o, out32, out_rstride, out_tstride, pad);
        const int64_t nblocks = (int64_t)n_mtiles * nsplit * T;
        if (nblocks > 0x7fffffff) throw std::runtime_error("ppals: scan grid too large");
        dim3 grid((unsigned)nblocks);
        const int64_t pgrid = nblocks < (int64_t)ncu_ * persist_mult_ ? (int64_t)ncu_ * std::min(persist_mult_, 6)
                                                                       : (int64_t)ncu_ * persist_mult_;
        dim3 grid_p((unsigned)std::min<int64_t>(nblocks, pgrid));
        bool nts = nt_store(nsplit, (double)M * T * ncols * (d.out32 ? 4.0 : 8.0));
        const bool buf_ok = (16.0 * (double)M * sizeof(TV) < 2.0e9) && (pack_bytes < 2000000000ull);
        const bool takes_buf = al && M >= VEC && buf_ok && (NT == 1 || sizeof(TV) == 8) &&
                               !(sizeof(TV) == 8 && nsplit > 1);
        const bool takes_tail = !takes_buf && al && M >= VEC && T == 1 && nsplit == 1 && NT <= 2 &&
                                d.row_ld == 0 && scan_tail_split<TV>(NT, n_mtiles) >= 0;
        if (takes_tail) nts = false;
        bool takes_pk = false;
        if constexpr (sizeof(TV) == 4)
          takes_pk = takes_buf && NT == 1 && nsplit == 1 && d.row_ld == 0 && scan_pk_.data && scan_pk_.L == L &&
                     scan_pk_.J == J && scan_pk_.T == T;
        prof_begin(scan_slot_, takes_pk ? (double)pack_data_bytes(L, J, T) + (double)pack_base_bytes(L, J, T) +
                                              (double)L * (double)T * ncols * (out32 ? 4.0 : 8.0)
                                        : bytes);
        if (takes_tail)
          route("scan.%s.suffix.tail nt=%d from=%d", tname<TV>(), NT, scan_tail_split<TV>(NT, n_mtiles));
        else if (takes_pk)
          route("scan.%s.suffix.pk nt=1 nsplit=1 nts=%d pad=0 out32=%d", tname<TV>(), nts ? 1 : 0, out32);
        else if (takes_buf || (al && M >= VEC))
          route("scan.%s.suffix.%s nt=%d nsplit=%d nts=%d pad=%d out32=%d", tname<TV>(), takes_buf ? "buf" : "fast",
                NT, nsplit, nts ? 1 : 0, pad.ld ? 1 : 0, out32);
        else
          route("scan.%s.suffix.generic al=%d nt=%d nsplit=%d pad=%d out32=%d", tname<TV>(), al ? 1 : 0, NT, nsplit,
                pad.ld ? 1 : 0, out32);
        if (takes_tail) {
          const int tail_from = scan_tail_split<TV>(NT, n_mtiles);
          const int64_t strips = ((M + 16 * VEC - 1) / (16 * VEC)) - (int64_t)tail_from * 4;
          dim3 grid_t((unsigned)(tail_from + strips));
          const size_t lds_t = sizeof(double) * 3 * (size_t)(VEC * NT * 4) * 64;
          dispatch<1, 2>(NT, [&](auto nt) {
            hipLaunchKernelGGL((k_scan_suffix_fast<TV, nt, 9>), grid_t, dim3(256), lds_t, st_, V, M, K, M * K, P,
                               n_mtiles, nsplit, per, nblk, d.p, d.nstride, d.split_stride, d.batch_stride, ncols,
                               d.out32, (int64_t)0, (int64_t)0, tail_from);
          });
        } else if (takes_pk) {
          scan_pk_launches_++;
          dispatch<5, 1>(nts ? 5 : 1, [&](auto opt) {
            hipLaunchKernelGGL((k_scan_suffix_pk<opt>), grid_p, dim3(256), 0, st_, (const char *)scan_pk_.data,
                               (const unsigned int *)scan_pk_.bases, pack_tile_bytes(J), M, (const float *)P, n_mtiles,
                               nblk, d.p, d.nstride, d.batch_stride, ncols, d.out32, nblocks);
          });
        } else {
          dispatch<1, 2, 3, 4>(NT, [&](auto nt) {
            if (takes_buf)
              dispatch<5, 1>(nts ? 5 : 1, [&](auto opt) {
                hipLaunchKernelGGL((k_scan_suffix_buf<TV, nt, opt>), grid_p, dim3(256), 0, st_, V, M, K, M * K, P,
                                   n_mtiles, nsplit, per, nblk, d.p, d.nstride, d.split_stride, d.batch_stride,
                                   ncols, d.out32, nblocks, d.row_ld, d.row_valid);
              });
            else if (al && M >= VEC)
              dispatch<5, 1>(nts ? 5 : 1, [&](auto opt) {
                hipLaunchKernelGGL((k_scan_suffix_fast<TV, nt, opt>), grid, dim3(256), 0, st_, V, M, K, M * K, P,
                                   n_mtiles, nsplit, per, nblk, d.p, d.nstride, d.split_stride, d.batch_stride,
                                   ncols, d.out32, d.row_ld, d.row_valid);
              });
            else
              dispatch<true, false>(al, [&](auto alv) {
                hipLaunchKernelGGL((k_scan_suffix<TV, nt, alv>), grid, dim3(256), 0, st_, V, M, K, M * K, P,
                                   n_mtiles, nsplit, per, nblk, d.p, d.nstride, d.split_stride, d.batch_stride,
                                   ncols, d.out32, d.row_ld, d.row_valid);
              });
          });
        }
        prof_end();
        HIP_CHECK(hipGetLastError());
        slab_combine(nsplit, d.p, d.split_stride, M, ncols, o, 1, out_rstride, out32, pad, T, d.batch_stride,
                     out_tstride);
      }
    }
  }
  void scan_wide(const float *V, int64_t L, int64_t J, int64_t T, const KrpArgs &a, int col0, int ncols,
                 double *out, int64_t out_tstride, int64_t out_rstride, int out32, RowPad pad) {
    const int NT = (ncols + 15) / 16;
    const int64_t nblk64 = (J + 15) / 16;
    if (nblk64 > 0x7fffffff) throw std::runtime_error("ppals: contraction extent too large");
    const int nblk = (int)nblk64;
    const size_t pack_bytes = (size_t)nblk * NT * 256 * sizeof(float);
    float *P = (float *)ensure(ws_pack_, ws_pack_sz_, pack_bytes);
    hipLaunchKernelGGL(k_krp_pack<float>, dim3(grid_for((int64_t)nblk * NT * 256, 256)), dim3(256), 0, st_,
                       P, nblk, NT, 0, a, J, col0, ncols);
    HIP_CHECK(hipGetLastError());
    double *o = out32 ? (double *)((float *)out + (int64_t)col0 * out_rstride)
                      : out + (int64_t)col0 * out_rstride;
    const int64_t M = L, K = J;
    const int64_t n_mtiles64 = (M + 63) / 64;
    if (n_mtiles64 * T > 0x7fffffff) throw std::runtime_error("ppals: scan grid too large");
    const int n_mtiles = (int)n_mtiles64;
    const void *kernel = nullptr;
    dispatch<5, 6, 7, 8>(NT, [&](auto nt) { kernel = (const void *)k_scan_wide<nt, 1>; });
    const double slots = (double)ncu_ * occupancy(wide_occ_[NT - 1], kernel, 512, 0, 2);
    const int64_t tiles = n_mtiles64 * T;
    int want = 1;
    if ((double)tiles < 8.0 * slots) {
      double best = -1.0;
      const int ns_max = (int)std::min<int64_t>(24, std::max(1, nblk / 16));
      for (int ns = 1; ns <= ns_max; ns++) {
        const double rounds = (double)tiles * ns / slots;
        const double score = rounds / std::ceil(rounds) - 0.004 * ns;
        if (score > best) {
          best = score;
          want = ns;
        }
      }
    }
    const KSplit ks = k_split(nblk, want);
    const int nsplit = ks.nsplit, per = (int)ks.per;
    const PassDst d = pass_dst(nsplit, M, T, ncols, o, out32, out_rstride, out_tstride, pad);
    const int64_t nblocks = (int64_t)n_mtiles * nsplit * T;
    if (nblocks > 0x7fffffff) throw std::runtime_error("ppals: scan grid too large");
    const double bytes = (double)L * (double)J * (double)T * 4.0 + (double)L * (double)T * ncols * (out32 ? 4.0 : 8.0);
    route("scan.f32.wide nt=%d nsplit=%d pad=%d out32=%d", NT, nsplit, pad.ld ? 1 : 0, out32);
    prof_begin(scan_slot_, bytes);
    dispatch<5, 6, 7, 8>(NT, [&](auto nt) {
      hipLaunchKernelGGL((k_scan_wide<nt, 1>), dim3((unsigned)nblocks), dim3(512), 0, st_, V, M, K, M * K, P,
                         n_mtiles, nsplit, per, nblk, d.p, d.nstride, d.split_stride, d.batch_stride, ncols, d.out32,
                         d.row_ld, d.row_valid);
    });
    prof_end();
    HIP_CHECK(hipGetLastError());
    slab_combine(nsplit, d.p, d.split_stride, M, ncols, o, 1, out_rstride, out32, pad, T, d.batch_stride,
                 out_tstride);
  }
  int gj_scalar_ = 0;
  bool wide_enabled_ = true;
  int wide_occ_[8] = {0, 0, 0, 0, 0, 0, 0, 0};
  template <typename TV>
  int scan_tail_split(int NT, int n_mtiles) {
    constexpr int VEC = ScanTraits<TV>::VEC;
    if (!scan_tail_on_) return -1;
    const size_t lds_t = sizeof(double) * 3 * (size_t)(VEC * NT * 4) * 64;
    const int per_cu = occupancy(scan_tail_occ_[(sizeof(TV) == 8 ? 2 : 0) + (NT - 1)],
                                 NT == 1 ? (const void *)k_scan_suffix_fast<TV, 1, 9>
                                         : (const void *)k_scan_suffix_fast<TV, 2, 9>,
                                 256, lds_t, -1);
    if (per_cu < 0) return -1;
    const int slots = ncu_ * per_cu;
    if (n_mtiles <= slots || n_mtiles > 4 * slots) return -1;
    const int rem = n_mtiles % slots;
    if (rem == 0 || rem * 4 > slots * 3) return -1;
    return n_mtiles - rem;
  }
  int scan_tail_occ_[4] = {0, 0, 0, 0};
  bool scan_tail_on_ = true;
  void scan_bf16(const uint16_t *V, int64_t L, int64_t J, int64_t T, const FactorRef *f, int nf, int R,
                 double *out, int64_t out_tstride, int64_t out_rstride, int out32, RowPad pad) {
    int64_t Jk;
    const KrpArgs a = krp_args(f, nf, &Jk);
    if (Jk != J) throw std::runtime_error("ppals: scan factor extents do not match the tensor");
    const bool aligned_base = (((uintptr_t)V) & 15) == 0;
    const int64_t nblk64 = (J + BF16_KB - 1) / BF16_KB;
    const int64_t n_mtiles64 = (L + 511) / 512;
    const bool mfma_ok = L > 1 && aligned_base && L % 8 == 0 && nblk64 * BF16_MAX_NT * 3 * 1024 < 2000000000ll &&
                         n_mtiles64 * T <= 0x7fffffff;
    const bool big = (double)BF16_KB * L * 2.0 >= 2.0e9;
    const double bytes_v = (double)L * J * T * 2.0;
    for (int col0 = 0; col0 < R; col0 += 16 * BF16_MAX_NT) {
      const int ncols = std::min(16 * BF16_MAX_NT, R - col0);
      double *o = out32 ? (double *)((float *)out + (int64_t)col0 * out_rstride) : out + (int64_t)col0 * out_rstride;
      prof_begin(scan_slot_, bytes_v + (double)L * T * ncols * (out32 ? 4.0 : 8.0));
      if (mfma_ok) {
        const int NT = (ncols + 15) / 16;
        const int nblk = (int)nblk64;
        uint16_t *P = (uint16_t *)ensure(ws_pack_, ws_pack_sz_, (size_t)nblk * NT * 3 * 1024);
        hipLaunchKernelGGL(k_krp_pack_bf16, dim3(grid_for((int64_t)nblk * NT * 512, 256)), dim3(256), 0, st_, P,
                           nblk, NT, a, J, col0, ncols);
        HIP_CHECK(hipGetLastError());
        const int64_t M = L;
        int want = 1;
        if (T == 1 && n_mtiles64 < (int64_t)ncu_ * 8)
          want = (int)std::min<int64_t>(((int64_t)ncu_ * 8 + n_mtiles64 - 1) / n_mtiles64,
                                        std::max(1, nblk / 16));
        else if (T > 1 && n_mtiles64 * T < ncu_ && (double)M * T * ncols * nblk / 4 * 8.0 < 64e6)
          want = (int)std::min<int64_t>(((int64_t)ncu_ * 2 + n_mtiles64 * T - 1) / (n_mtiles64 * T),
                                        std::max(1, nblk / 4));
        const KSplit ks = k_split(nblk, want);
        const int nsplit = ks.nsplit, per = (int)ks.per;
        if (n_mtiles64 * nsplit * T > 0x7fffffff) throw std::runtime_error("ppals: scan grid too large");
        const PassDst d = pass_dst(nsplit, M, T, ncols, o, out32, out_rstride, out_tstride, pad);
        const dim3 grid((unsigned)(n_mtiles64 * nsplit * T));
        const bool nts = nt_store(nsplit, (double)L * T * ncols * (out32 ? 4.0 : 8.0));
        route("scan.bf16.mfma nsplit=%d nts=%d pad=%d out32=%d", nsplit, nts ? 1 : 0, pad.ld ? 1 : 0, out32);
        dispatch<true, false>(nts, [&](auto ntsv) {
          dispatch<true, false>(big, [&](auto bigv) {
            hipLaunchKernelGGL((k_scan_suffix_bf16<BF16_MAX_NT, ntsv, bigv>), grid, dim3(256), 0, st_, V, L, J, P,
                               (int)n_mtiles64, nsplit, per, nblk, d.p, d.nstride, d.split_stride, d.batch_stride,
                               ncols, d.out32, d.row_ld, d.row_valid);
          });
        });
        HIP_CHECK(hipGetLastError());
        slab_combine(nsplit, d.p, d.split_stride, M, ncols, o, 1, out_rstride, out32, pad, T, d.batch_stride,
                     out_tstride);
      } else {
        double *B = (double *)ensure(ws_krp_, ws_krp_sz_, sizeof(double) * (size_t)J * ncols);
        krp(B, f, nf, col0, ncols);
// ... 2473 lines not shown
```

pairwise-perturbation_amd/csrc/kernels_pack.hip.h:

```cpp
#pragma once
#include <hip/hip_runtime.h>
#include <stdint.h>

#include "ops.h"

namespace ppals {

typedef unsigned int pk_u32;
typedef pk_u32 pk_u32x2 __attribute__((ext_vector_type(2)));

struct PkLane {
  pk_u32 e[4][4];
  bool ok[4][4];
};
__device__ inline PkLane pk_gather(const float *__restrict__ V, int64_t L, int64_t J, int n_mtiles, int nkb,
                                   int64_t gid, int tid) {
  const int lane = tid & 63, wave = tid >> 6, g = lane >> 4, j16 = lane & 15;
  const int64_t tile = gid / nkb;
  const int kb = (int)(gid % nkb);
  const int64_t mtile = tile % n_mtiles, batch = tile / n_mtiles;
  const int64_t m = (mtile * 4 + wave) * 64 + 4 * j16;
  PkLane r;
#pragma unroll
  for (int u = 0; u < 4; u++) {
    const int64_t k = (int64_t)kb * 16 + 4 * u + g;
#pragma unroll
    for (int jj = 0; jj < 4; jj++) {
      r.ok[u][jj] = k < J && m + jj < L;
      r.e[u][jj] = r.ok[u][jj] ? __float_as_uint(V[(batch * J + k) * L + m + jj]) : 0u;
    }
  }
  return r;
}

__global__ __launch_bounds__(256) void k_pk_prepass(const float *__restrict__ V, int64_t L, int64_t J,
                                                    int n_mtiles, int nkb, pk_u32 *__restrict__ bases,
                                                    int *__restrict__ spread) {
  __shared__ int smn[256], smx[256];
  const int64_t gid = blockIdx.x;
  const PkLane r = pk_gather(V, L, J, n_mtiles, nkb, gid, threadIdx.x);
  int mn = 255, mx = 0;
#pragma unroll
  for (int u = 0; u < 4; u++)
#pragma unroll
    for (int jj = 0; jj < 4; jj++)
      if (r.ok[u][jj]) {
        const int t = (int)(r.e[u][jj] >> 24);
        mn = min(mn, t);
        mx = max(mx, t);
      }
  smn[threadIdx.x] = mn;
  smx[threadIdx.x] = mx;
  __syncthreads();
  for (int s = 128; s > 0; s >>= 1) {
    if ((int)threadIdx.x < s) {
      smn[threadIdx.x] = min(smn[threadIdx.x], smn[threadIdx.x + s]);
      smx[threadIdx.x] = max(smx[threadIdx.x], smx[threadIdx.x + s]);
    }
    __syncthreads();
  }
  if (threadIdx.x == 0) {
    mn = smn[0];
    mx = smx[0];
    if (mx < mn) mn = mx = 0;
    bases[gid] = (pk_u32)mn * 0x01010101u;
    atomicMax(spread, mx - mn);
  }
}

__global__ __launch_bounds__(256) void k_pk_pack(const float *__restrict__ V, int64_t L, int64_t J, int n_mtiles,
                                                 int nkb, int64_t tile_bytes, const pk_u32 *__restrict__ bases,
                                                 char *__restrict__ out) {
  const int64_t gid = blockIdx.x;
  const int tid = threadIdx.x, lane = tid & 63, wave = tid >> 6;
  const PkLane r = pk_gather(V, L, J, n_mtiles, nkb, gid, tid);
  const pk_u32 base = bases[gid] & 0xffu;
  const int64_t tile = gid / nkb;
  const int kb = (int)(gid % nkb);
  char *blk = out + tile * tile_bytes + (int64_t)kb * PACK_BLOCK_BYTES;
  pk_u32 cw[2] = {0u, 0u};
#pragma unroll
  for (int u = 0; u < 4; u++) {
    pk_u32 e[4];
#pragma unroll
    for (int jj = 0; jj < 4; jj++) {
      e[jj] = r.ok[u][jj] ? r.e[u][jj] : base << 24;
      cw[u >> 1] |= ((e[jj] >> 24) - base) << (8 * jj + 4 * (u & 1));
    }
    if ((int64_t)kb * 16 + 4 * u < J) {
      pk_u32 *q = reinterpret_cast<pk_u32 *>(blk + PACK_CODE_BYTES + u * PACK_QUAD_BYTES + wave * 768 + lane * 12);
#pragma unroll
      for (int i = 0; i < 3; i++) q[i] = (e[i] & 0xffffffu) | (((e[3] >> (8 * i)) & 0xffu) << 24);
    }
  }
  *reinterpret_cast<pk_u32x2 *>(blk + wave * 512 + lane * 8) = pk_u32x2{cw[0], cw[1]};
}

}
```

pairwise-perturbation_amd/csrc/kernels_scan.hip.h:

```cpp
#pragma once
#include <hip/hip_runtime.h>
#include <stdint.h>

#include "ops.h"

namespace ppals {

typedef float f32x4 __attribute__((ext_vector_type(4)));
typedef double f64x4 __attribute__((ext_vector_type(4)));
typedef double f64x2 __attribute__((ext_vector_type(2)));

template <typename TV>
struct ScanTraits;
template <>
struct ScanTraits<float> {
  static constexpr int VEC = 4;
  typedef f32x4 vec;
  typedef f32x4 acc;
  static constexpr bool NEEDS_FLUSH = true;
  __device__ static inline acc mfma(float a, float b, acc c) {
    return __builtin_amdgcn_mfma_f32_16x16x4f32(a, b, c, 0, 0, 0);
  }
  __device__ static inline int row(int lane, int reg) { return (lane >> 4) * 4 + reg; }
};
// ... 480 lines not shown
    const TV *vbase;
    int voff, kb0, kb1;
    bool live;
  };
  auto decode = [&](int64_t id, Tile &t) {
    unsigned b = (unsigned)id;
    const int mtile = (int)(b % (unsigned)n_mtiles);
    b /= (unsigned)n_mtiles;
    const int split = (int)(b % (unsigned)nsplit);
    const int64_t batch = b / (unsigned)nsplit;
    const int64_t m0 = ((int64_t)mtile * 4 + wave) * (16 * VEC);
    t.live = m0 < M;
    t.m = m0 + (int64_t)VEC * j16;
    const int64_t m_ld = t.live ? min(t.m, M - VEC) : 0;
    t.voff = (int)(((int64_t)g * M + m_ld) * (int64_t)sizeof(TV));
    t.kb0 = split * kb_per_split;
    t.kb1 = min(nkb, t.kb0 + kb_per_split);
    t.vbase = V + batch * batch_stride;
    t.obase = split * out_split_stride + batch * out_batch_stride;
  };
#define PPALS_BUF_LOAD(vbase_, voff_, kb_, vv_, bb_)                                           \
  {                                                                                            \
    const int64_t boff_ = (int64_t)(kb_)*block_bytes;                                          \
    const int64_t rem_ = total_bytes - boff_;                                                  \
    const __amdgpu_buffer_rsrc_t rs_ = __builtin_amdgcn_make_buffer_rsrc(                      \
        (void *)((const char *)(vbase_) + boff_), 0, (int)min(rem_, block_bytes), 0x00020000); \
    _Pragma("unroll") for (int u = 0; u < VEC; u++) vv_[u] = __builtin_bit_cast(               \
        vec, __builtin_amdgcn_raw_buffer_load_b128(rs_, voff_, u * ustep, AUXV));              \
    _Pragma("unroll") for (int nt = 0; nt < NT; nt++) bb_[nt] = __builtin_bit_cast(            \
        vec, __builtin_amdgcn_raw_buffer_load_b128(                                            \
                 rsrcP, voffP, (int)(((kb_)*NT + nt) * (4 * 16 * VEC) * (int)sizeof(TV)), 0)); \
  }

  Tile cur, nxt;
  int64_t id = blockIdx.x;
  for (; id < ntiles; id += gridDim.x) {
    decode(id, cur);
    if (cur.live && cur.kb0 < cur.kb1) break;
  }
  if (id >= ntiles) return;
  vec cv[VEC], cb[NT];
  PPALS_BUF_LOAD(cur.vbase, cur.voff, cur.kb0, cv, cb);

  for (;;) {
    bool has_next = false;
    int64_t nid = id + gridDim.x;
    for (; nid < ntiles; nid += gridDim.x) {
      decode(nid, nxt);
      if (nxt.live && nxt.kb0 < nxt.kb1) {
        has_next = true;
        break;
      }
    }
    acc_t acc[VEC][NT];
    double acc64[TR::NEEDS_FLUSH ? VEC : 1][TR::NEEDS_FLUSH ? NT : 1][4];
#pragma unroll
    for (int a = 0; a < VEC; a++)
#pragma unroll
      for (int nt = 0; nt < NT; nt++) {
#pragma unroll
        for (int r = 0; r < 4; r++) acc[a][nt][r] = 0;
        if constexpr (TR::NEEDS_FLUSH) {
#pragma unroll
          for (int r = 0; r < 4; r++) acc64[a][nt][r] = 0;
        }
      }
    for (int kc = cur.kb0; kc < cur.kb1; kc += FLUSH) {
      const int ke = min(cur.kb1, kc + FLUSH);
      for (int kb = kc; kb < ke; kb++) {
        vec nv[VEC], nb[NT];
        const bool same = kb + 1 < cur.kb1;
        const TV *pv = (same || !has_next) ? cur.vbase : nxt.vbase;
        const int po = (same || !has_next) ? cur.voff : nxt.voff;
        const int pk = same ? kb + 1 : (has_next ? nxt.kb0 : kb);
        PPALS_BUF_LOAD(pv, po, pk, nv, nb);
#pragma unroll
        for (int u = 0; u < VEC; u++)
#pragma unroll
          for (int jj = 0; jj < VEC; jj++)
#pragma unroll
            for (int nt = 0; nt < NT; nt++)
              acc[jj][nt] = TR::mfma(cb[nt][u], cv[u][jj], acc[jj][nt]);
#pragma unroll
        for (int u = 0; u < VEC; u++) cv[u] = nv[u];
#pragma unroll
        for (int nt = 0; nt < NT; nt++) cb[nt] = nb[nt];
      }
      if constexpr (TR::NEEDS_FLUSH) {
#pragma unroll
        for (int a = 0; a < VEC; a++)
#pragma unroll
          for (int nt = 0; nt < NT; nt++)
#pragma unroll
            for (int r = 0; r < 4; r++) {
              acc64[a][nt][r] += (double)acc[a][nt][r];
              acc[a][nt][r] = 0;
            }
      }
    }
    const ScanRowMap rm = scan_row_map<VEC>(cur.m, M, row_ld, row_valid);
    const bool vec_ok =
        (((cur.obase | out_nstride | rm.mo) & (VEC - 1)) == 0) && rm.nvalid == VEC;
#pragma unroll
    for (int nt = 0; nt < NT; nt++)
#pragma unroll
      for (int r = 0; r < 4; r++) {
        const int n = 16 * nt + TR::row(lane, r);
        if (n < ncols && rm.nvalid > 0) {
          double val[VEC];
#pragma unroll
          for (int jj = 0; jj < VEC; jj++) {
            if constexpr (TR::NEEDS_FLUSH)
              val[jj] = acc64[jj][nt][r];
            else
              val[jj] = (double)acc[jj][nt][r];
          }
          int64_t idx = cur.obase + (int64_t)n * out_nstride + rm.mo;
          if constexpr (OPT & 2)
            idx = cur.obase + (cur.m >> 8) * ((int64_t)ncols << 8) + ((int64_t)n << 8) + (cur.m & 255);
          if (vec_ok && out32) {
            typedef float ovec_t __attribute__((ext_vector_type(VEC)));
            ovec_t ov;
#pragma unroll
            for (int jj = 0; jj < VEC; jj++) ov[jj] = (float)val[jj];
            if constexpr (OPT & 4)
              __builtin_nontemporal_store(ov, reinterpret_cast<ovec_t *>(reinterpret_cast<float *>(out) + idx));
            else
              *reinterpret_cast<ovec_t *>(reinterpret_cast<float *>(out) + idx) = ov;
          } else if (vec_ok) {
#pragma unroll
            for (int jj = 0; jj < VEC; jj += 2) {
              f64x2 ov = {val[jj], val[jj + 1]};
              if constexpr (OPT & 4)
                __builtin_nontemporal_store(ov, reinterpret_cast<f64x2 *>(out + idx + jj));
              else
                *reinterpret_cast<f64x2 *>(out + idx + jj) = ov;
            }
          } else {
#pragma unroll
            for (int jj = 0; jj < VEC; jj++)
              if (jj < rm.nvalid) scan_store(out, idx + jj, val[jj], out32);
          }
        }
      }
    if (!has_next) break;
    cur = nxt;
    id = nid;
  }
#undef PPALS_BUF_LOAD
}

typedef unsigned int scan_u32x2 __attribute__((ext_vector_type(2)));
typedef unsigned int scan_u32x3 __attribute__((ext_vector_type(3)));
template <int OPT>
__global__ __launch_bounds__(256) __attribute__((amdgpu_waves_per_eu(3, 3))) void k_scan_suffix_pk(
    const char *__restrict__ Vp, const unsigned int *__restrict__ bases, int64_t tile_bytes, int64_t M,
    const float *__restrict__ P, int n_mtiles, int nkb, double *__restrict__ out, int64_t out_nstride,
    int64_t out_batch_stride, int ncols, int out32, int64_t ntiles) {
  typedef ScanTraits<float> TR;
  typedef unsigned int u32;
  constexpr int VEC = 4, FLUSH = SCAN_FLUSH;
  constexpr int AUXV = (OPT & 1) ? 2 : 0;
  const int lane = threadIdx.x & 63, wave = threadIdx.x >> 6;
  const int g = lane >> 4, j16 = lane & 15;
  const int voffP = (int)((g * 16 + j16) * VEC * (int)sizeof(float));
  const int voffC = wave * 512 + lane * 8;
  const int voffQ = PACK_CODE_BYTES + wave * 768 + lane * 12;
  const __amdgpu_buffer_rsrc_t rsrcP = __builtin_amdgcn_make_buffer_rsrc(
      (void *)P, 0, (int)((int64_t)nkb * (4 * 16 * VEC) * (int64_t)sizeof(float)), 0x00020000);

  struct Tile {
    int64_t m, obase;
    bool live;
  };
  auto decode = [&](int64_t id, Tile &t) {
    const unsigned b = (unsigned)id;
    const int mtile = (int)(b % (unsigned)n_mtiles);
    const int64_t batch = b / (unsigned)n_mtiles;
    const int64_t m0 = ((int64_t)mtile * 4 + wave) * (16 * VEC);
    t.live = m0 < M;
    t.m = m0 + (int64_t)VEC * j16;
    t.obase = batch * out_batch_stride;
  };
  struct Raw {
    u32 w[12], c[2], b;
    f32x4 p;
  };
#define PPALS_PK_LOAD(tile_, kb_, r_)                                                                 \
  {                                                                                                   \
    const int t_ = __builtin_amdgcn_readfirstlane((int)(tile_));                                      \
    const int k_ = __builtin_amdgcn_readfirstlane((int)(kb_));                                        \
    const int64_t koff_ = (int64_t)k_ * PACK_BLOCK_BYTES;                                             \
    const __amdgpu_buffer_rsrc_t rs_ = __builtin_amdgcn_make_buffer_rsrc(                             \
        (void *)(Vp + (int64_t)t_ * tile_bytes + koff_), 0,                                           \
        (int)min(tile_bytes - koff_, (int64_t)PACK_BLOCK_BYTES), 0x00020000);                         \
    _Pragma("unroll") for (int u = 0; u < 4; u++) {                                                   \
      const scan_u32x3 q_ = __builtin_amdgcn_raw_buffer_load_b96(rs_, voffQ, u * PACK_QUAD_BYTES, AUXV); \
      r_.w[3 * u] = q_[0];                                                                            \
      r_.w[3 * u + 1] = q_[1];                                                                        \
      r_.w[3 * u + 2] = q_[2];                                                                        \
    }                                                                                                 \
    const scan_u32x2 c_ = __builtin_amdgcn_raw_buffer_load_b64(rs_, voffC, 0, AUXV);                  \
    r_.c[0] = c_[0];                                                                                  \
    r_.c[1] = c_[1];                                                                                  \
    r_.b = bases[(int64_t)t_ * nkb + k_];                                                             \
    r_.p = __builtin_bit_cast(f32x4, __builtin_amdgcn_raw_buffer_load_b128(                           \
                                         rsrcP, voffP, k_ * (4 * 16 * VEC) * (int)sizeof(float), 0)); \
  }
  auto unpack = [](const Raw &r, f32x4(&v)[4]) {
#pragma unroll
    for (int u = 0; u < 4; u++) {
      const u32 cw = r.c[u >> 1];
      const u32 T = (((u & 1) ? cw >> 4 : cw) & 0x0f0f0f0fu) + r.b;
      const u32 w0 = r.w[3 * u], w1 = r.w[3 * u + 1], w2 = r.w[3 * u + 2];
      v[u][0] = __uint_as_float(__builtin_amdgcn_perm(T, w0, 0x04020100u));
      v[u][1] = __uint_as_float(__builtin_amdgcn_perm(T, w1, 0x05020100u));
      v[u][2] = __uint_as_float(__builtin_amdgcn_perm(T, w2, 0x06020100u));
      v[u][3] = __uint_as_float(__builtin_amdgcn_perm(w1, w0, 0x0c0c0703u) |
                                __builtin_amdgcn_perm(T, w2, 0x07030c0cu));
    }
  };

  Tile cur, nxt;
  int64_t id = blockIdx.x;
  for (; id < ntiles; id += gridDim.x) {
    decode(id, cur);
    if (cur.live) break;
  }
  if (id >= ntiles || nkb <= 0) return;
  f32x4 cv[4], cb;
  {
    Raw r0;
    PPALS_PK_LOAD(id, 0, r0);
    unpack(r0, cv);
    cb = r0.p;
  }

  for (;;) {
    bool has_next = false;
    int64_t nid = id + gridDim.x;
    for (; nid < ntiles; nid += gridDim.x) {
      decode(nid, nxt);
      if (nxt.live) {
        has_next = true;
        break;
      }
    }
    f32x4 acc[VEC];
    double acc64[VEC][4];
#pragma unroll
    for (int a = 0; a < VEC; a++)
#pragma unroll
      for (int r = 0; r < 4; r++) {
        acc[a][r] = 0;
        acc64[a][r] = 0;
      }
    for (int kc = 0; kc < nkb; kc += FLUSH) {
      const int ke = min(nkb, kc + FLUSH);
      for (int kb = kc; kb < ke; kb++) {
        Raw nr;
        const bool same = kb + 1 < nkb;
        const int64_t pt = (same || !has_next) ? id : nid;
        const int pk = same ? kb + 1 : (has_next ? 0 : kb);
        PPALS_PK_LOAD(pt, pk, nr);
        __builtin_amdgcn_sched_barrier(0);
#pragma unroll
        for (int u = 0; u < VEC; u++)
#pragma unroll
          for (int jj = 0; jj < VEC; jj++) acc[jj] = TR::mfma(cb[u], cv[u][jj], acc[jj]);
        __builtin_amdgcn_sched_barrier(0);
        unpack(nr, cv);
        cb = nr.p;
      }
#pragma unroll
      for (int a = 0; a < VEC; a++)
#pragma unroll
        for (int r = 0; r < 4; r++) {
          acc64[a][r] += (double)acc[a][r];
          acc[a][r] = 0;
        }
    }
    const ScanRowMap rm = scan_row_map<VEC>(cur.m, M, 0, 0);
    const bool vec_ok = (((cur.obase | out_nstride | rm.mo) & (VEC - 1)) == 0) && rm.nvalid == VEC;
#pragma unroll
    for (int r = 0; r < 4; r++) {
      const int n = TR::row(lane, r);
      if (n < ncols && rm.nvalid > 0) {
        double val[VEC];
#pragma unroll
        for (int jj = 0; jj < VEC; jj++) val[jj] = acc64[jj][r];
        const int64_t idx = cur.obase + (int64_t)n * out_nstride + rm.mo;
        if (vec_ok && out32) {
          f32x4 ov;
#pragma unroll
          for (int jj = 0; jj < VEC; jj++) ov[jj] = (float)val[jj];
          if constexpr (OPT & 4)
            __builtin_nontemporal_store(ov, reinterpret_cast<f32x4 *>(reinterpret_cast<float *>(out) + idx));
          else
            *reinterpret_cast<f32x4 *>(reinterpret_cast<float *>(out) + idx) = ov;
        } else if (vec_ok) {
#pragma unroll
          for (int jj = 0; jj < VEC; jj += 2) {
            f64x2 ov = {val[jj], val[jj + 1]};
            if constexpr (OPT & 4)
              __builtin_nontemporal_store(ov, reinterpret_cast<f64x2 *>(out + idx + jj));
            else
              *reinterpret_cast<f64x2 *>(out + idx + jj) = ov;
          }
        } else {
#pragma unroll
          for (int jj = 0; jj < VEC; jj++)
            if (jj < rm.nvalid) scan_store(out, idx + jj, val[jj], out32);
        }
      }
    }
    if (!has_next) break;
    cur = nxt;
    id = nid;
  }
#undef PPALS_PK_LOAD
}

template <int NT, int OPT = 0>
__global__ __launch_bounds__(512) void k_scan_wide(
    const float *__restrict__ V, int64_t M, int64_t K, int64_t batch_stride,
    const float *__restrict__ P, int n_mtiles, int nsplit, int kb_per_split, int nkb,
    double *__restrict__ out, int64_t out_nstride, int64_t out_split_stride,
    int64_t out_batch_stride, int ncols, int out32, int64_t row_ld = 0, int64_t row_valid = 0) {
  constexpr int BM = 64, BK = 16;
  constexpr int PITCH = BM + 16;
  constexpr int NTA = (NT + 3) / 4;
  constexpr int VSZ = BK * PITCH, PSZ = 512 * 4;
  __shared__ __attribute__((aligned(16))) float Vs[2][2 * VSZ];
  __shared__ __attribute__((aligned(16))) float Ps[2][2 * PSZ];

  const int tid = threadIdx.x, lane = tid & 63;
  const int wave = __builtin_amdgcn_readfirstlane(tid >> 6);
  const int g = lane >> 4, j16 = lane & 15;
  const int wm = wave & 1, wn = wave >> 1;
  const int nt0 = NTA * wn, ntc = max(0, min(NTA, NT - nt0));

  unsigned b = blockIdx.x;
  const int mtile = (int)(b % (unsigned)n_mtiles);
  b /= (unsigned)n_mtiles;
  const int split = (int)(b % (unsigned)nsplit);
  const int64_t batch = b / (unsigned)nsplit;
  const int64_t m0 = (int64_t)mtile * BM;
  const int kb0 = split * kb_per_split;
  const int kb1 = min(nkb, kb0 + kb_per_split);
  const int nb = kb1 - kb0;
  if (nb <= 0) return;
  const int nstages = (nb + 1) >> 1;

  const int mq = tid & 15, kk = (tid >> 4) & 15, hv = wave >> 2;
  const int64_t m_ld = min(m0 + 4 * mq, M - 4);
  const char *__restrict__ vbase = (const char *)(V + batch * batch_stride);
  const int voffV = (int)(((int64_t)kk * M + m_ld) * 4);
  const int64_t block_bytes = (int64_t)BK * M * 4, total_bytes = K * M * 4;
  const int voffP = tid * 16;
  const int vdst = hv * VSZ + kk * PITCH + 4 * mq;
  const __amdgpu_buffer_rsrc_t rsrcP = __builtin_amdgcn_make_buffer_rsrc(
      (void *)P, 0, wave < NT ? (int)((int64_t)nkb * NT * 1024) : 0, 0x00020000);
  constexpr int AUXV = (OPT & 1) ? 2 : 0;

  f32x4 gv[2], gp[2][2];
#define PPALS_WIDE_LOAD(set_, st_)                                                                     \
  {                                                                                                    \
    _Pragma("unroll") for (int h_ = 0; h_ < 2; h_++) {                                                 \
      const int kb_ = kb0 + min(2 * (st_) + h_, nb - 1);                                               \
      gp[set_][h_] = __builtin_bit_cast(                                                               \
          f32x4, __builtin_amdgcn_raw_buffer_load_b128(rsrcP, voffP, kb_ * (NT * 1024), 0));           \
    }                                                                                                  \
    const int i_ = 2 * (st_) + hv;                   \
    const int64_t boff_ = (int64_t)(kb0 + min(i_, nb - 1)) * block_bytes;                              \
    const __amdgpu_buffer_rsrc_t rs_ = __builtin_amdgcn_make_buffer_rsrc(                              \
        (void *)(vbase + boff_), 0, i_ < nb ? (int)min(total_bytes - boff_, block_bytes) : 0,          \
        0x00020000);                                                                                   \
    gv[set_] = __builtin_bit_cast(f32x4, __builtin_amdgcn_raw_buffer_load_b128(rs_, voffV, 0, AUXV));  \
  }
#define PPALS_WIDE_STAGE(set_, buf_)                                                         \
  {                                                                                          \
    *reinterpret_cast<f32x4 *>(&Vs[buf_][vdst]) = gv[set_];                                  \
    _Pragma("unroll") for (int h_ = 0; h_ < 2; h_++)                                         \
        *reinterpret_cast<f32x4 *>(&Ps[buf_][h_ * PSZ + 4 * tid]) = gp[set_][h_];            \
  }

  f32x4 acc[2][NTA];
  double acc64[2][NTA][4];
#pragma unroll
  for (int ms = 0; ms < 2; ms++)
#pragma unroll
    for (int i = 0; i < NTA; i++)
#pragma unroll
      for (int r = 0; r < 4; r++) {
        acc[ms][i][r] = 0;
        acc64[ms][i][r] = 0;
      }

  PPALS_WIDE_LOAD(0, 0);
  PPALS_WIDE_LOAD(1, min(1, nstages - 1));
  PPALS_WIDE_STAGE(0, 0);
  __syncthreads();
  for (int j0 = 0; j0 < nstages; j0 += 2) {
#pragma unroll
    for (int sp = 0; sp < 2; sp++) {
      const int j = j0 + sp;
      if (j < nstages) {
        PPALS_WIDE_LOAD(sp, min(j + 2, nstages - 1));
#pragma unroll
        for (int h = 0; h < 2; h++) {
          float vb[2][4];
          const float *vs = &Vs[sp][h * VSZ + g * PITCH + 32 * wm + j16];
#pragma unroll
          for (int q = 0; q < 4; q++)
#pragma unroll
            for (int ms = 0; ms < 2; ms++) vb[ms][q] = vs[4 * q * PITCH + 16 * ms];
          f32x4 pa[NTA];
#pragma unroll
          for (int t = 0; t < NTA; t++)
            pa[t] = *reinterpret_cast<const f32x4 *>(
                &Ps[sp][h * PSZ + (min(nt0 + t, NT - 1) * 64 + lane) * 4]);
#pragma unroll
          for (int q = 0; q < 4; q++)
#pragma unroll
            for (int t = 0; t < NTA; t++) {
              if (t >= ntc) break;
#pragma unroll
              for (int ms = 0; ms < 2; ms++)
                acc[ms][t] = __builtin_amdgcn_mfma_f32_16x16x4f32(pa[t][q], vb[ms][q], acc[ms][t], 0, 0, 0);
            }
        }
        PPALS_WIDE_STAGE(sp ^ 1, sp ^ 1);
        __syncthreads();
      }
    }
#pragma unroll
    for (int ms = 0; ms < 2; ms++)
#pragma unroll
      for (int t = 0; t < NTA; t++)
#pragma unroll
        for (int r = 0; r < 4; r++) {
          acc64[ms][t][r] += (double)acc[ms][t][r];
          acc[ms][t][r] = 0;
        }
  }
#undef PPALS_WIDE_LOAD
#undef PPALS_WIDE_STAGE

  const int64_t obase = split * out_split_stride + batch * out_batch_stride;
#pragma unroll
  for (int ms = 0; ms < 2; ms++) {
    const int64_t m = m0 + 32 * wm + 16 * ms + j16;
    const ScanRowMap rm = scan_row_map<1>(m, M, row_ld, row_valid);
    if (rm.nvalid == 0) continue;
#pragma unroll
    for (int i = 0; i < NTA; i++) {
      if (i >= ntc) break;
#pragma unroll
      for (int r = 0; r < 4; r++) {
        const int n = 16 * (nt0 + i) + 4 * g + r;
        if (n < ncols)
          scan_store(out, obase + (int64_t)n * out_nstride + rm.mo,
                     acc64[ms][i][r] + (double)acc[ms][i][r], out32);
      }
    }
  }
}

template <typename TV, int NT, int OPT = 0>
__global__ __launch_bounds__(256) void k_scan_prefix_fast(
    const TV *__restrict__ V, int64_t M, int64_t K, const TV *__restrict__ P, int mb_per_split,
    int nmb, double *__restrict__ out, int64_t out_kstride, int64_t out_nstride,
    int64_t out_split_stride, int ncols, int out32) {
// ... 552 lines not shown
```

pairwise-perturbation_amd/csrc/ops.h:

```cpp
#pragma once
#include <cmath>
#include <cstddef>
#include <cstdint>
#include <limits>
#include <string>
#include <vector>

#include "bf16.h"
#include "device_view.h"
#include "preload_policy.h"

namespace ppals {

enum DType { F32 = 0, F64 = 1, BF16 = 3 };
inline size_t dtype_size(int dt) { return dt == F32 ? 4 : (dt == BF16 ? 2 : 8); }
inline int work_dt(int storage) { return storage == BF16 ? F32 : storage; }

struct RowPad {
  int64_t ld = 0, valid = 0;
};

constexpr int PACK_BLOCK_BYTES = 14336, PACK_CODE_BYTES = 2048, PACK_QUAD_BYTES = 3072;
constexpr int PACK_WINDOW = 16;
struct PackedSrc {
  const void *data = nullptr;
  const void *bases = nullptr;
  int64_t L = 0, J = 0, T = 0;
};
inline int64_t pack_tile_bytes(int64_t J) {
  const int64_t kfull = J / 16, rem = J - kfull * 16;
  return kfull * PACK_BLOCK_BYTES + (rem ? PACK_CODE_BYTES + (rem + 3) / 4 * PACK_QUAD_BYTES : 0);
}
inline int64_t pack_tiles(int64_t L, int64_t T) { return (L + 255) / 256 * T; }
inline size_t pack_data_bytes(int64_t L, int64_t J, int64_t T) {
  return (size_t)pack_tiles(L, T) * (size_t)pack_tile_bytes(J);
}
inline size_t pack_base_bytes(int64_t L, int64_t J, int64_t T) {
  return (size_t)pack_tiles(L, T) * (size_t)((J + 15) / 16) * 4;
}

constexpr int MAX_ORDER = 8;
constexpr double kNnFloor = 1e-16;
constexpr double kOrthoMinRatio = 0x1p-40;
enum ModeKind { kModeFree = 0, kModeNonneg = 1, kModeFixed = 2, kModeOrtho = 3 };
enum ModeShape { kShapeNone = 0, kShapeUnimodal = 1, kShapeIncreasing = 2, kShapeDecreasing = 3 };
constexpr size_t kShapeLdsBytes = 152 * 1024;
inline size_t shape_work_bytes(int64_t rows) { return 64 * (size_t)rows + 8; }

constexpr int kMaxStarts = 32;
struct StartTable {
  int nstarts = 0;
  int col[kMaxStarts + 1] = {0};
  int sq[kMaxStarts + 1] = {0};
  int rank(int b) const { return col[b + 1] - col[b]; }
  int max_rank() const {
    int m = 0;
    for (int b = 0; b < nstarts; b++) m = rank(b) > m ? rank(b) : m;
    return m;
  }
};
struct FactorRef {
  const double *ptr;
  int64_t rows;
  int64_t ld;
};

struct PPTerm {
  const double *T;
  int64_t ny;
  int keep_first;
  const double *dW;
  int64_t lddw;
};

struct ProfileSlot {
  int64_t launches = 0;
  double ms = 0;
  double bytes = 0;
};

class Ops {
 public:
  virtual ~Ops() {}
  virtual void *alloc(size_t bytes) = 0;
  virtual void free(void *p) = 0;
  virtual void h2d(void *dst, const void *src, size_t bytes) = 0;
  virtual void d2h(void *dst, const void *src, size_t bytes) = 0;
  virtual void d2d(void *dst, const void *src, size_t bytes) = 0;
  virtual void zero(void *p, size_t bytes) = 0;
  virtual void sync() = 0;
  virtual void *stream() { return nullptr; }
  virtual void bind() {}
  virtual bool supports_storage(int dt) { return dt == F32 || dt == F64; }

  virtual void fill_uniform(void *V, int dt, int64_t l0, int64_t g0, int64_t row0, int64_t rest,
                            uint64_t seed, double lo, double hi) = 0;
  virtual void fill_laplacian(void *V, int dt, int64_t l0, int64_t g0, int64_t row0, int64_t rest,
                              int ndigits, int s) = 0;
  virtual void add_uniform_noise(void *V, int dt, int64_t l0, int64_t g0, int64_t row0,
                                 int64_t rest, uint64_t seed, double lo, double hi,
                                 double alpha) = 0;
  virtual void uniform_sumsq(int64_t l0, int64_t g0, int64_t row0, int64_t rest, uint64_t seed,
                             double lo, double hi, double *out) = 0;
  virtual void fill_rank(void *V, int dt, int64_t M, int64_t K, const double *Q, const double *P,
                         int R) = 0;
  virtual void residual_sq(const void *V, int dt, int64_t M, int64_t K, const double *Q,
                           const double *P, int R, double *out) = 0;
  virtual void upload_shard(void *V, int dt, const double *host_full, int64_t l0, int64_t g0,
                            int64_t row0, int64_t rest) = 0;

  virtual void download_shard(const void *V, int dt, double *host_full, int64_t l0, int64_t g0,
                              int64_t row0, int64_t rest) = 0;

  virtual void transpose2d(const void *src, int dt, int64_t rows, int64_t cols, void *dst) = 0;
  virtual void transpose_batched(const void *src, int dt, int64_t rows, int64_t cols, int64_t batch,
                                 void *dst) {
    const size_t step = (size_t)rows * cols * dtype_size(dt);
    for (int64_t b = 0; b < batch; b++)
      transpose2d((const char *)src + b * step, dt, rows, cols, (char *)dst + b * step);
  }
  virtual void pad_layout(const void *src, int dt, int64_t rows, int64_t cols, int64_t blk,
                          int64_t ld, void *dst) = 0;
  virtual void unpack_shards(const void *stage, int dt, int64_t s0, int64_t rest, int64_t blk,
                             int P, int64_t chunk_bytes, void *full) = 0;
  virtual void *try_alloc(size_t bytes) { return alloc(bytes); }
  virtual void scan_store_mode(int mode) { (void)mode; }
  virtual size_t mem_available() { return (size_t)-1; }
  virtual int pack_layout(const void * , int , int64_t , int64_t , int64_t ,
                          void * , void * ) {
    return -1;
  }
  virtual void scan_packed_source(const PackedSrc * ) {}
  virtual int64_t scan_packed_launches() { return 0; }

  struct PtrInfo {
    bool is_device = false;
    int device = -1;
    uint64_t base = 0, size = 0;
  };
  virtual bool device_ptr_info(const void * , PtrInfo * , std::string * ) {
    throw Unsupported("ppals: this back end has no device views");
  }
  virtual void copy_view(const ViewPlan & , int , void * , int ,
                         void * , int , void * ) {
    throw Unsupported("ppals: this back end has no device views");
  }
  virtual void model_to_view(const ModelPlan & , const double * , const double * ,
                             int , bool , void * , int ,
                             const void * , int , void * ) {
    throw Unsupported("ppals: this back end has no device views");
  }
  virtual void model_impute(const ModelPlan & , const double * , const double * ,
                            int , bool , const void * , void * , int ,
                            double * , void * ) {
    throw Unsupported("ppals: this back end has no device views");
  }

  virtual void model_wls(const ModelPlan & , const ModelSide & , const double * ,
                         const double * , int , const void * , const void * ,
                         int , void * , int , double * , void * ) {
    throw Unsupported("ppals: this back end has no device views");
  }

  virtual void model_huber(const ModelPlan & , const ModelSide * , const double * ,
                           const double * , int , const void * , const void * ,
                           int , void * , int , double , double * ,
                           void * ) {
    throw Unsupported("ppals: this back end has no device views");
  }
  static constexpr int ABSRES_BINS = 2048;
  virtual void model_absres_hist(const ModelPlan & , const ModelSide * , const double * ,
                                 const double * , int , const void * , const void * ,
                                 int , int , uint32_t , int , uint32_t ,
                                 uint64_t * , void * ) {
    throw Unsupported("ppals: this back end has no device views");
  }

  struct Parafac2Step {
    int64_t I = 0, J = 0, K = 0;
    int R = 0;
    const void *X = nullptr;
    int vdt = 0;
    int64_t s1 = 0, s2 = 0;
    const double *B = nullptr;
    const double *A = nullptr;
    const double *C = nullptr;
    double *Q = nullptr, *P = nullptr, *T = nullptr;
    int *status = nullptr;
    double min_ratio = 0;
    void *Y = nullptr;
    int dt = 0;
    double *out = nullptr;
  };
  virtual void parafac2_check() { throw Unsupported("ppals: this back end has no device views"); }
  virtual void parafac2_init(double * , int64_t , int , int64_t ) {
    throw Unsupported("ppals: this back end has no device views");
  }
  virtual void parafac2_step(const Parafac2Step & , void * ) {
    throw Unsupported("ppals: this back end has no device views");
  }

  virtual void join_stream(void * ) { throw Unsupported("ppals: this back end has no device views"); }
  virtual void release_stream(void * ) {
    throw Unsupported("ppals: this back end has no device views");
  }

  static double prep_load(const void *V, int dt, size_t e) {
    return dt == F32 ? (double)((const float *)V)[e] : dt == BF16 ? (double)((const bf16s *)V)[e] : ((const double *)V)[e];
  }
  static void prep_store(void *V, int dt, size_t e, double x) {
    if (dt == F32)
      ((float *)V)[e] = (float)x;
    else if (dt == BF16)
      ((bf16s *)V)[e] = bf16s(x);
    else
      ((double *)V)[e] = x;
  }
  virtual void center_fibres(void *V, int dt, int64_t L, int64_t J, int64_t T, double *off) {
    const size_t n = (size_t)L * J * T;
    std::vector<char> h(n * dtype_size(dt));
    std::vector<double> o((size_t)L * T);
    d2h(h.data(), V, h.size());
    for (int64_t t = 0; t < T; t++)
      for (int64_t l = 0; l < L; l++) {
        double s = 0;
        for (int64_t j = 0; j < J; j++) s += prep_load(h.data(), dt, (size_t)(l + L * (j + J * t)));
        const double m = s / (double)J;
        o[(size_t)(l + L * t)] = m;
        for (int64_t j = 0; j < J; j++) {
          const size_t e = (size_t)(l + L * (j + J * t));
          prep_store(h.data(), dt, e, prep_load(h.data(), dt, e) - m);
        }
      }
    h2d(V, h.data(), h.size());
    if (off) h2d(off, o.data(), sizeof(double) * o.size());
  }
  virtual void shift_fibres(void *V, int dt, int64_t L, int64_t J, int64_t T, const double *off, double alpha) {
    const size_t n = (size_t)L * J * T;
    std::vector<char> h(n * dtype_size(dt));
    std::vector<double> o((size_t)L * T);
    d2h(h.data(), V, h.size());
    d2h(o.data(), off, sizeof(double) * o.size());
    for (int64_t t = 0; t < T; t++)
      for (int64_t j = 0; j < J; j++)
        for (int64_t l = 0; l < L; l++) {
          const size_t e = (size_t)(l + L * (j + J * t));
          prep_store(h.data(), dt, e, prep_load(h.data(), dt, e) + alpha * o[(size_t)(l + L * t)]);
        }
    h2d(V, h.data(), h.size());
  }
  virtual void slice_sumsq(const void *V, int dt, int64_t L, int64_t J, int64_t T, double *ss) {
    const size_t n = (size_t)L * J * T;
    std::vector<char> h(n * dtype_size(dt));
    std::vector<double> s((size_t)J, 0.0);
    d2h(h.data(), V, h.size());
    for (int64_t t = 0; t < T; t++)
      for (int64_t j = 0; j < J; j++)
        for (int64_t l = 0; l < L; l++) {
          const double v = prep_load(h.data(), dt, (size_t)(l + L * (j + J * t)));
          s[(size_t)j] += v * v;
        }
    h2d(ss, s.data(), sizeof(double) * s.size());
  }
  virtual void scale_slices(void *V, int dt, int64_t L, int64_t J, int64_t T, const double *fac) {
    const size_t n = (size_t)L * J * T;
    std::vector<char> h(n * dtype_size(dt));
    std::vector<double> f((size_t)J);
    d2h(h.data(), V, h.size());
    d2h(f.data(), fac, sizeof(double) * f.size());
    for (int64_t t = 0; t < T; t++)
      for (int64_t j = 0; j < J; j++) {
        if (f[(size_t)j] == 1.0) continue;
        for (int64_t l = 0; l < L; l++) {
          const size_t e = (size_t)(l + L * (j + J * t));
          prep_store(h.data(), dt, e, prep_load(h.data(), dt, e) * f[(size_t)j]);
        }
      }
    h2d(V, h.data(), h.size());
  }

  virtual void npls_contract(const void *X, int dt, int64_t L, int64_t I, int64_t T, const double *U, int C, double *Z) {
    if (L * T <= 0 || C <= 0) return;
    const size_t n = (size_t)L * I * T, LT = (size_t)L * T;
    std::vector<char> h(n * dtype_size(dt));
// ... 783 lines not shown
```

Baseline: 623.0.

## Add 26-bit packed tensor format with escape blocks for suffix scans

Adds a second packed encoding of the fp32 tensor that stores 2-bit exponent codes per element instead of 4-bit. Blocks whose exponent spread does not fit in that window are sent to a side escape buffer, indexed by ordinals kept in the per-block side words. A prepass now counts escape blocks, and auto mode picks the 26-bit format when escapes are at most one block in sixteen. The aim is to cut the HBM bytes the memory-bound suffix scan reads per element. In exchange the scan kernel does extra side-word prefetching and escape decoding.

```diff
diff --git a/__graft_entry__.py b/__graft_entry__.py
--- a/__graft_entry__.py
+++ b/__graft_entry__.py
@@ -25,6 +25,7 @@
     _run(["make", "-C", os.path.join(ROOT, "tests", "shape_shim")])
     _run(["make", "-C", os.path.join(ROOT, "tests", "huber_shim")])
     _run(["make", "-C", os.path.join(ROOT, "tests", "parafac2_shim")])
+    _run(["make", "-C", os.path.join(ROOT, "tests", "pack26_shim")])
     sys.path.insert(0, PKG)
     import ppals
     lib = ppals.lib()
diff --git a/pairwise-perturbation_amd/csrc/engine.cpp b/pairwise-perturbation_amd/csrc/engine.cpp
--- a/pairwise-perturbation_amd/csrc/engine.cpp
+++ b/pairwise-perturbation_amd/csrc/engine.cpp
@@ -643,7 +643,7 @@
   if (const char *e = std::getenv("PPALS_TEST_BLOCKED_UPDATE")) test_blocks_ = std::atoi(e);
   if (N_ < 3) schedule_ = 0;
   if (const char *e = std::getenv("PPALS_PLACE_TUNE")) ms_tune_enabled_ = std::atoi(e) != 0;
-  if (const char *e = std::getenv("PPALS_PACK_LAYOUT")) pack_mode_ = std::atoi(e) == 0 ? 0 : (std::atoi(e) == 1 ? 1 : -1);
+  if (const char *e = std::getenv("PPALS_PACK_LAYOUT")) pack_mode_ = std::atoi(e) >= 0 && std::atoi(e) <= 2 ? std::atoi(e) : -1;
   if (N_ >= 3) {
     ms_set_roots(ms_choose_roots());
     ms_scales_ = (double *)ops_.alloc(sizeof(double) * 32);
@@ -908,20 +908,55 @@
   for (auto &t : packs_) {
     ops_.free(t.data);
     ops_.free(t.bases);
+    ops_.free(t.esc);
   }
   packs_.clear();
 }
 
 bool CpEngine::pack_fill(PackedTwin &t) {
-  const int spread = ops_.pack_layout(t.src, V_.dtype, t.L, t.J, t.T, t.data, t.bases);
-  if (spread >= 0 && spread < PACK_WINDOW) return true;
-  ops_.free(t.data);
-  ops_.free(t.bases);
-  t.data = t.bases = nullptr;
-  t.bytes = 0;
-  t.reason = spread < 0 ? "scan shape has no packed route"
-                        : "top bytes of a block span " + std::to_string(spread + 1) + " values (window 16)";
-  return false;
+  auto drop = [&](const std::string &why) {
+    ops_.free(t.data);
+    ops_.free(t.bases);
+    ops_.free(t.esc);
+    t.data = t.bases = t.esc = nullptr;
+    t.bytes = t.esc_room = 0;
+    t.format = 0;
+    t.escapes = 0;
+    t.reason = why;
+    return false;
+  };
+  const bool forced = pack_mode_ == 1 || pack_mode_ == 2;
+  const size_t bb = pack_base_bytes(t.L, t.J, t.T);
+  if (!t.bases && !(t.bases = ops_.try_alloc(bb))) return drop("allocation failed");
+  const PackSurvey sv = ops_.pack_survey(t.src, V_.dtype, t.L, t.J, t.T, t.bases);
+  if (sv.spread < 0) return drop("scan shape has no packed route");
+  if (sv.spread >= PACK_WINDOW)
+    return drop("top bytes of a block span " + std::to_string(sv.spread + 1) + " values (window 16)");
+  const int fmt = pack_choose_format(pack_mode_, sv.spread, sv.escapes, pack_blocks_of(t.L, t.J, t.T));
+  if (!fmt) return drop("more escape blocks than the side word can number");
+  const size_t db = pack_data_bytes(fmt, t.L, t.J, t.T);
+  const size_t eb = fmt == PACK_FMT26 ? (size_t)sv.escapes * PACK26_ESC_BYTES : 0;
+  if (t.data && (fmt != t.format || eb > t.esc_room)) {
+    ops_.free(t.data);
+    ops_.free(t.esc);
+    t.data = t.esc = nullptr;
+    t.esc_room = 0;
+  }
+  if (!t.data) {
+    if (!forced && db + bb + eb >= (size_t)t.L * (size_t)t.J * (size_t)t.T * 4)
+      return drop("row tiles would pad away what packing saves");
+    if (!optional_fits(db + eb)) return drop("no room beside what the session still allocates");
+    t.data = ops_.try_alloc(db);
+    t.esc = t.data && eb ? ops_.try_alloc(eb) : nullptr;
+    if (!t.data || (eb && !t.esc)) return drop("allocation failed");
+    t.esc_room = eb;
+  }
+  t.format = fmt;
+  t.escapes = sv.escapes;
+  t.bytes = db + bb + eb;
+  t.reason.clear();
+  ops_.pack_write(t.src, t.L, t.J, t.T, fmt, t.bases, t.data, t.esc);
+  return true;
 }
 
 const PackedSrc *CpEngine::packed_for(const ScanPlan &pl, PackedSrc &out) {
@@ -931,7 +966,7 @@
     else if (R_ > 16) pack_off_reason_ = "not eligible: more than 16 result columns";
     else if (dist_) pack_off_reason_ = "not eligible: sharded session";
     else if (multi_) pack_off_reason_ = "not eligible: multi-start session";
-    else if (pack_mode_ != 1 && (double)V_.nloc * 4.0 < 1e8) pack_off_reason_ = "tensor below 100 MB";
+    else if (pack_mode_ < 0 && (double)V_.nloc * 4.0 < 1e8) pack_off_reason_ = "tensor below 100 MB";
   }
   if (!pack_off_reason_.empty()) return nullptr;
   const int li = (int)(pl.lay - lay_.data());
@@ -945,33 +980,21 @@
     n.L = pl.L;
     n.J = pl.J;
     n.T = pl.T;
-    const size_t db = pack_data_bytes(n.L, n.J, n.T), bb = pack_base_bytes(n.L, n.J, n.T);
-    if (pl.lay->q > 0) {
+    if (pl.lay->q > 0)
       n.reason = "padded layout";
-    } else if (n.L < 4 || n.L % 4) {
+    else if (n.L < 4 || n.L % 4)
       n.reason = "scan shape has no packed route";
-    } else if (pack_mode_ != 1 && db + bb >= (size_t)n.L * (size_t)n.J * (size_t)n.T * 4) {
-      n.reason = "row tiles would pad away what packing saves";
-    } else if (!optional_fits(db + bb)) {
-      n.reason = "no room beside what the session still allocates";
-    } else {
-      n.data = ops_.try_alloc(db);
-      n.bases = n.data ? ops_.try_alloc(bb) : nullptr;
-      if (!n.bases) {
-        ops_.free(n.data);
-        n.data = nullptr;
-        n.reason = "allocation failed";
-      } else {
-        n.bytes = db + bb;
-        pack_fill(n);
-      }
-    }
+    else
+      pack_fill(n);
     packs_.push_back(n);
     t = &packs_.back();
   }
   if (!t->data) return nullptr;
   out.data = t->data;
   out.bases = t->bases;
+  out.esc = t->esc;
+  out.format = t->format;
+  out.escapes = t->escapes;
   out.L = t->L;
   out.J = t->J;
   out.T = t->T;
@@ -3219,7 +3242,7 @@
   }
 }
 std::string CpEngine::placement_report() const {
-  char buf[400];
+  char buf[512];
   std::string out = "{\"mode\": ";
   out += ms_tune_enabled_ && ms_X_slack() > 0 ? "\"online\"" : "\"off\"";
   out += ", \"setup_s\": 0.0, \"candidate_blocks_held\": ";
@@ -3245,17 +3268,18 @@
   }
   out += "]";
   out += ", \"packed\": {\"mode\": ";
-  out += pack_mode_ == 0 ? "\"off\"" : (pack_mode_ == 1 ? "\"on\"" : "\"auto\"");
+  out += pack_mode_ == 0 ? "\"off\"" : (pack_mode_ > 0 ? "\"on\"" : "\"auto\"");
   out += ", \"refused\": \"" + pack_off_reason_ + "\", \"packed_scans\": " + std::to_string(ops_.scan_packed_launches()) +
          ", \"layouts\": [";
   for (size_t k = 0; k < packs_.size(); k++) {
     const PackedTwin &t = packs_[k];
     snprintf(buf, sizeof buf,
              "%s{\"layout\": \"%s\", \"rows\": %lld, \"reduced\": %lld, \"batches\": %lld, \"packed\": %s, "
-             "\"bytes_per_element\": %.4f, \"reason\": \"%s\"}",
+             "\"bytes_per_element\": %.4f, \"format\": %d, \"escape_blocks\": %lld, \"reason\": \"%s\"}",
              k ? ", " : "", t.layout == 0 ? "tensor" : (t.layout == 1 ? "second (transposed) copy" : "padded copy"),
              (long long)t.L, (long long)t.J, (long long)t.T, t.data ? "true" : "false",
-             t.data ? (double)t.bytes / ((double)t.L * (double)t.J * (double)t.T) : 4.0, t.reason.c_str());
+             t.data ? (double)t.bytes / ((double)t.L * (double)t.J * (double)t.T) : 4.0, t.format,
+             (long long)t.escapes, t.reason.c_str());
     out += buf;
   }
   out += "]}}";
diff --git a/pairwise-perturbation_amd/csrc/engine.h b/pairwise-perturbation_amd/csrc/engine.h
--- a/pairwise-perturbation_amd/csrc/engine.h
+++ b/pairwise-perturbation_amd/csrc/engine.h
@@ -444,7 +444,10 @@
     int layout = 0;
     const void *src = nullptr;
     int64_t L = 0, J = 0, T = 0;
-    void *data = nullptr, *bases = nullptr;
+    void *data = nullptr, *bases = nullptr, *esc = nullptr;
+    int format = 0;
+    int64_t escapes = 0;
+    size_t esc_room = 0;
     size_t bytes = 0;
     std::string reason;
   };
diff --git a/pairwise-perturbation_amd/csrc/hip_ops.hip b/pairwise-perturbation_amd/csrc/hip_ops.hip
--- a/pairwise-perturbation_amd/csrc/hip_ops.hip
+++ b/pairwise-perturbation_amd/csrc/hip_ops.hip
@@ -226,7 +226,7 @@
     }
     if (ws_mttv_) hipFree(ws_mttv_);
     if (ws_pack_) hipFree(ws_pack_);
-    if (pack_spread_) hipFree(pack_spread_);
+    if (pack_stats_) hipFree(pack_stats_);
     if (ws_mv_) hipFree(ws_mv_);
     if (ws_hist_) hipFree(ws_hist_);
     if (ws_slab_) hipFree(ws_slab_);
@@ -1472,28 +1472,43 @@
   }
   PackedSrc scan_pk_;
   int64_t scan_pk_launches_ = 0;
+  bool scan_pk2_branch_ = [] {
+    const char *e = getenv("PPALS_PK2_DECODE");
+    return e && std::string(e) == "branch";
+  }();
   int64_t scan_packed_launches() override { return scan_pk_launches_; }
-  int *pack_spread_ = nullptr;
-  int pack_layout(const void *src, int dt, int64_t L, int64_t J, int64_t T, void *data, void *bases) override {
+  int *pack_stats_ = nullptr;
+  PackSurvey pack_survey(const void *src, int dt, int64_t L, int64_t J, int64_t T, void *bases) override {
     const int64_t n_mtiles = (L + 255) / 256, nkb = (J + 15) / 16;
+    PackSurvey sv;
     if (dt != F32 || L < 4 || L % 4 || J < 1 || T < 1 || (((uintptr_t)src) & 15) || n_mtiles * T > 0x7fffffff ||
         n_mtiles * T * nkb > 0x7fffffff)
-      return -1;
-    if (!pack_spread_) pack_spread_ = (int *)alloc(sizeof(int));
+      return sv;
+    if (!pack_stats_) pack_stats_ = (int *)alloc(2 * sizeof(int));
     const unsigned nblocks = (unsigned)(n_mtiles * T * nkb);
-    HIP_CHECK(hipMemsetAsync(pack_spread_, 0, sizeof(int), st_));
+    HIP_CHECK(hipMemsetAsync(pack_stats_, 0, 2 * sizeof(int), st_));
     hipLaunchKernelGGL(k_pk_prepass, dim3(nblocks), dim3(256), 0, st_, (const float *)src, L, J, (int)n_mtiles,
-                       (int)nkb, (pk_u32 *)bases, pack_spread_);
-    HIP_CHECK(hipGetLastError());
-    int spread = 0;
-    HIP_CHECK(hipMemcpyAsync(&spread, pack_spread_, sizeof(int), hipMemcpyDeviceToHost, st_));
+                       (int)nkb, (pk_u32 *)bases, pack_stats_);
+    HIP_CHECK(hipGetLastError());
+    int stats[2] = {0, 0};
+    HIP_CHECK(hipMemcpyAsync(stats, pack_stats_, sizeof stats, hipMemcpyDeviceToHost, st_));
     HIP_CHECK(hipStreamSynchronize(st_));
-    if (spread >= PACK_WINDOW) return spread;
-    hipLaunchKernelGGL(k_pk_pack, dim3(nblocks), dim3(256), 0, st_, (const float *)src, L, J, (int)n_mtiles, (int)nkb,
-                       pack_tile_bytes(J), (const pk_u32 *)bases, (char *)data);
+    sv.spread = stats[0];
+    sv.escapes = stats[1];
+    return sv;
+  }
+  void pack_write(const void *src, int64_t L, int64_t J, int64_t T, int format, void *bases, void *data,
+                  void *esc) override {
+    const int64_t n_mtiles = (L + 255) / 256, nkb = (J + 15) / 16;
+    const unsigned nblocks = (unsigned)(n_mtiles * T * nkb);
+    hipLaunchKernelGGL(k_pk_side_words, dim3(1), dim3(1024), 0, st_, (pk_u32 *)bases, (int64_t)nblocks, format);
+    HIP_CHECK(hipGetLastError());
+    dispatch<PACK_FMT26, PACK_FMT28>(format, [&](auto fmt) {
+      hipLaunchKernelGGL((k_pk_pack<fmt>), dim3(nblocks), dim3(256), 0, st_, (const float *)src, L, J, (int)n_mtiles,
+                         (int)nkb, pack_tile_bytes(fmt, J), (const pk_u32 *)bases, (char *)data, (char *)esc);
+    });
     HIP_CHECK(hipGetLastError());
     HIP_CHECK(hipStreamSynchronize(st_));
-    return spread;
   }
   void scan_profile_slot(int slot) override { scan_slot_ = slot == 1 ? 1 : 0; }
   int scan_nt_mode_ = -1;
@@ -1677,13 +1692,17 @@
         if constexpr (sizeof(TV) == 4)
           takes_pk = takes_buf && NT == 1 && nsplit == 1 && d.row_ld == 0 && scan_pk_.data && scan_pk_.L == L &&
                      scan_pk_.J == J && scan_pk_.T == T;
-        prof_begin(scan_slot_, takes_pk ? (double)pack_data_bytes(L, J, T) + (double)pack_base_bytes(L, J, T) +
+        const bool pk26 = takes_pk && scan_pk_.format == PACK_FMT26;
+        prof_begin(scan_slot_, takes_pk ? (double)pack_data_bytes(scan_pk_.format, L, J, T) +
+                                              (double)pack_base_bytes(L, J, T) +
+                                              (pk26 ? (double)scan_pk_.escapes * PACK26_ESC_BYTES : 0.0) +
                                               (double)L * (double)T * ncols * (out32 ? 4.0 : 8.0)
                                         : bytes);
         if (takes_tail)
           route("scan.%s.suffix.tail nt=%d from=%d", tname<TV>(), NT, scan_tail_split<TV>(NT, n_mtiles));
         else if (takes_pk)
-          route("scan.%s.suffix.pk nt=1 nsplit=1 nts=%d pad=0 out32=%d", tname<TV>(), nts ? 1 : 0, out32);
+          route("scan.%s.suffix.%s nt=1 nsplit=1 nts=%d pad=0 out32=%d", tname<TV>(), pk26 ? "pk2" : "pk", nts ? 1 : 0,
+                out32);
         else if (takes_buf || (al && M >= VEC))
           route("scan.%s.suffix.%s nt=%d nsplit=%d nts=%d pad=%d out32=%d", tname<TV>(), takes_buf ? "buf" : "fast",
                 NT, nsplit, nts ? 1 : 0, pad.ld ? 1 : 0, out32);
@@ -1702,11 +1721,20 @@
           });
         } else if (takes_pk) {
           scan_pk_launches_++;
-          dispatch<5, 1>(nts ? 5 : 1, [&](auto opt) {
-            hipLaunchKernelGGL((k_scan_suffix_pk<opt>), grid_p, dim3(256), 0, st_, (const char *)scan_pk_.data,
-                               (const unsigned int *)scan_pk_.bases, pack_tile_bytes(J), M, (const float *)P, n_mtiles,
-                               nblk, d.p, d.nstride, d.batch_stride, ncols, d.out32, nblocks);
-          });
+          if (pk26)
+            dispatch<5, 1, 13, 9>((nts ? 5 : 1) | (scan_pk2_branch_ ? 8 : 0), [&](auto opt) {
+              hipLaunchKernelGGL((k_scan_suffix_pk2<opt>), grid_p, dim3(256), 0, st_, (const char *)scan_pk_.data,
+                                 (const unsigned int *)scan_pk_.bases, (const char *)scan_pk_.esc,
+                                 pack_tile_bytes(PACK_FMT26, J), M, (const float *)P, n_mtiles, nblk, d.p, d.nstride,
+                                 d.batch_stride, ncols, d.out32, nblocks);
+            });
+          else
+            dispatch<5, 1>(nts ? 5 : 1, [&](auto opt) {
+              hipLaunchKernelGGL((k_scan_suffix_pk<opt>), grid_p, dim3(256), 0, st_, (const char *)scan_pk_.data,
+                                 (const unsigned int *)scan_pk_.bases, pack_tile_bytes(PACK_FMT28, J), M,
+                                 (const float *)P, n_mtiles, nblk, d.p, d.nstride, d.batch_stride, ncols, d.out32,
+                                 nblocks);
+            });
         } else {
           dispatch<1, 2, 3, 4>(NT, [&](auto nt) {
             if (takes_buf)
diff --git a/pairwise-perturbation_amd/csrc/kernels_pack.hip.h b/pairwise-perturbation_amd/csrc/kernels_pack.hip.h
--- a/pairwise-perturbation_amd/csrc/kernels_pack.hip.h
+++ b/pairwise-perturbation_amd/csrc/kernels_pack.hip.h
@@ -35,7 +35,7 @@
 
 __global__ __launch_bounds__(256) void k_pk_prepass(const float *__restrict__ V, int64_t L, int64_t J,
                                                     int n_mtiles, int nkb, pk_u32 *__restrict__ bases,
-                                                    int *__restrict__ spread) {
+                                                    int *__restrict__ stats) {
   __shared__ int smn[256], smx[256];
   const int64_t gid = blockIdx.x;
   const PkLane r = pk_gather(V, L, J, n_mtiles, nkb, gid, threadIdx.x);
@@ -63,21 +63,48 @@
     mn = smn[0];
     mx = smx[0];
     if (mx < mn) mn = mx = 0;
-    bases[gid] = (pk_u32)mn * 0x01010101u;
-    atomicMax(spread, mx - mn);
+    const bool escape = mx - mn >= PACK26_WINDOW;
+    bases[gid] = (pk_u32)mn | (escape ? 0x100u : 0u);
+    atomicMax(stats, mx - mn);
+    if (escape) atomicAdd(stats + 1, 1);
   }
 }
 
+__global__ __launch_bounds__(1024) void k_pk_side_words(pk_u32 *__restrict__ bases, int64_t nblocks, int fmt) {
+  __shared__ unsigned int cnt[1024];
+  const int64_t per = (nblocks + 1023) / 1024;
+  const int64_t b0 = min(nblocks, (int64_t)threadIdx.x * per), b1 = min(nblocks, b0 + per);
+  unsigned int mine = 0;
+  if (fmt == PACK_FMT26)
+    for (int64_t b = b0; b < b1; b++) mine += (bases[b] >> 8) & 1u;
+  cnt[threadIdx.x] = mine;
+  __syncthreads();
+  for (int s = 1; s < 1024; s <<= 1) {
+    const unsigned int add = (int)threadIdx.x >= s ? cnt[threadIdx.x - s] : 0u;
+    __syncthreads();
+    cnt[threadIdx.x] += add;
+    __syncthreads();
+  }
+  unsigned int ordinal = cnt[threadIdx.x] - mine;
+  for (int64_t b = b0; b < b1; b++) {
+    const pk_u32 w = bases[b];
+    const bool escape = (w >> 8) & 1u;
+    bases[b] = pk_side_word(fmt, w & 0xffu, escape, ordinal);
+    ordinal += escape ? 1u : 0u;
+  }
+}
+
+template <int FMT>
 __global__ __launch_bounds__(256) void k_pk_pack(const float *__restrict__ V, int64_t L, int64_t J, int n_mtiles,
                                                  int nkb, int64_t tile_bytes, const pk_u32 *__restrict__ bases,
-                                                 char *__restrict__ out) {
+                                                 char *__restrict__ out, char *__restrict__ esc) {
   const int64_t gid = blockIdx.x;
   const int tid = threadIdx.x, lane = tid & 63, wave = tid >> 6;
   const PkLane r = pk_gather(V, L, J, n_mtiles, nkb, gid, tid);
-  const pk_u32 base = bases[gid] & 0xffu;
+  const pk_u32 side = bases[gid], base = side & 0xffu;
   const int64_t tile = gid / nkb;
   const int kb = (int)(gid % nkb);
-  char *blk = out + tile * tile_bytes + (int64_t)kb * PACK_BLOCK_BYTES;
+  char *blk = out + tile * tile_bytes + (int64_t)kb * pack_block_bytes(FMT);
   pk_u32 cw[2] = {0u, 0u};
 #pragma unroll
   for (int u = 0; u < 4; u++) {
@@ -85,15 +112,27 @@
 #pragma unroll
     for (int jj = 0; jj < 4; jj++) {
       e[jj] = r.ok[u][jj] ? r.e[u][jj] : base << 24;
-      cw[u >> 1] |= ((e[jj] >> 24) - base) << (8 * jj + 4 * (u & 1));
+      if constexpr (FMT == PACK_FMT26)
+        pk26_put(cw[0], cw[1], u, jj, (e[jj] >> 24) - base);
+      else
+        pk28_put(cw, u, jj, (e[jj] >> 24) - base);
     }
     if ((int64_t)kb * 16 + 4 * u < J) {
-      pk_u32 *q = reinterpret_cast<pk_u32 *>(blk + PACK_CODE_BYTES + u * PACK_QUAD_BYTES + wave * 768 + lane * 12);
+      pk_u32 *q = reinterpret_cast<pk_u32 *>(blk + pack_code_bytes(FMT) + u * PACK_QUAD_BYTES + pk_quad_offset(wave, lane));
+      pk_u32 qw[3];
+      pk_quad_encode(e, qw);
 #pragma unroll
-      for (int i = 0; i < 3; i++) q[i] = (e[i] & 0xffffffu) | (((e[3] >> (8 * i)) & 0xffu) << 24);
+      for (int i = 0; i < 3; i++) q[i] = qw[i];
     }
   }
-  *reinterpret_cast<pk_u32x2 *>(blk + wave * 512 + lane * 8) = pk_u32x2{cw[0], cw[1]};
+  if constexpr (FMT == PACK_FMT26) {
+    *reinterpret_cast<pk_u32 *>(blk + pk_code_offset(FMT, wave, lane)) = cw[0];
+    if (side >> 8)
+      *reinterpret_cast<pk_u32 *>(esc + (int64_t)((side >> 8) - 1u) * PACK26_ESC_BYTES +
+                                  pk_code_offset(FMT, wave, lane)) = cw[1];
+  } else {
+    *reinterpret_cast<pk_u32x2 *>(blk + pk_code_offset(FMT, wave, lane)) = pk_u32x2{cw[0], cw[1]};
+  }
 }
 
 }
diff --git a/pairwise-perturbation_amd/csrc/kernels_scan.hip.h b/pairwise-perturbation_amd/csrc/kernels_scan.hip.h
--- a/pairwise-perturbation_amd/csrc/kernels_scan.hip.h
+++ b/pairwise-perturbation_amd/csrc/kernels_scan.hip.h
@@ -656,20 +656,22 @@
 
 typedef unsigned int scan_u32x2 __attribute__((ext_vector_type(2)));
 typedef unsigned int scan_u32x3 __attribute__((ext_vector_type(3)));
-template <int OPT>
-__global__ __launch_bounds__(256) __attribute__((amdgpu_waves_per_eu(3, 3))) void k_scan_suffix_pk(
-    const char *__restrict__ Vp, const unsigned int *__restrict__ bases, int64_t tile_bytes, int64_t M,
-    const float *__restrict__ P, int n_mtiles, int nkb, double *__restrict__ out, int64_t out_nstride,
-    int64_t out_batch_stride, int ncols, int out32, int64_t ntiles) {
+template <int FMT, int OPT>
+__device__ __forceinline__ void scan_suffix_packed(
+    const char *__restrict__ Vp, const unsigned int *__restrict__ bases, const char *__restrict__ esc,
+    int64_t tile_bytes, int64_t M, const float *__restrict__ P, int n_mtiles, int nkb, double *__restrict__ out,
+    int64_t out_nstride, int64_t out_batch_stride, int ncols, int out32, int64_t ntiles) {
   typedef ScanTraits<float> TR;
   typedef unsigned int u32;
   constexpr int VEC = 4, FLUSH = SCAN_FLUSH;
   constexpr int AUXV = (OPT & 1) ? 2 : 0;
+  constexpr bool F26 = FMT == PACK_FMT26;
+  constexpr int BLOCK_BYTES = pack_block_bytes(FMT);
   const int lane = threadIdx.x & 63, wave = threadIdx.x >> 6;
   const int g = lane >> 4, j16 = lane & 15;
   const int voffP = (int)((g * 16 + j16) * VEC * (int)sizeof(float));
-  const int voffC = wave * 512 + lane * 8;
-  const int voffQ = PACK_CODE_BYTES + wave * 768 + lane * 12;
+  const int voffC = pk_code_offset(FMT, wave, lane);
+  const int voffQ = pack_code_bytes(FMT) + pk_quad_offset(wave, lane);
   const __amdgpu_buffer_rsrc_t rsrcP = __builtin_amdgcn_make_buffer_rsrc(
       (void *)P, 0, (int)((int64_t)nkb * (4 * 16 * VEC) * (int64_t)sizeof(float)), 0x00020000);
 
@@ -688,41 +690,72 @@
   };
   struct Raw {
     u32 w[12], c[2], b;
+    bool x;
     f32x4 p;
   };
-#define PPALS_PK_LOAD(tile_, kb_, r_)                                                                 \
+#define PPALS_PK_SIDE(tile_, kb_) \
+  bases[(int64_t)__builtin_amdgcn_readfirstlane((int)(tile_)) * nkb + __builtin_amdgcn_readfirstlane((int)(kb_))]
+#define PPALS_PK_LOAD(tile_, kb_, r_, side_)                                                          \
   {                                                                                                   \
     const int t_ = __builtin_amdgcn_readfirstlane((int)(tile_));                                      \
     const int k_ = __builtin_amdgcn_readfirstlane((int)(kb_));                                        \
-    const int64_t koff_ = (int64_t)k_ * PACK_BLOCK_BYTES;                                             \
+    const int64_t koff_ = (int64_t)k_ * BLOCK_BYTES;                                                  \
     const __amdgpu_buffer_rsrc_t rs_ = __builtin_amdgcn_make_buffer_rsrc(                             \
         (void *)(Vp + (int64_t)t_ * tile_bytes + koff_), 0,                                           \
-        (int)min(tile_bytes - koff_, (int64_t)PACK_BLOCK_BYTES), 0x00020000);                         \
+        (int)min(tile_bytes - koff_, (int64_t)BLOCK_BYTES), 0x00020000);                              \
     _Pragma("unroll") for (int u = 0; u < 4; u++) {                                                   \
       const scan_u32x3 q_ = __builtin_amdgcn_raw_buffer_load_b96(rs_, voffQ, u * PACK_QUAD_BYTES, AUXV); \
       r_.w[3 * u] = q_[0];                                                                            \
       r_.w[3 * u + 1] = q_[1];                                                                        \
       r_.w[3 * u + 2] = q_[2];                                                                        \
     }                                                                                                 \
-    const scan_u32x2 c_ = __builtin_amdgcn_raw_buffer_load_b64(rs_, voffC, 0, AUXV);                  \
-    r_.c[0] = c_[0];                                                                                  \
-    r_.c[1] = c_[1];                                                                                  \
-    r_.b = bases[(int64_t)t_ * nkb + k_];                                                             \
+    if constexpr (F26) {                                                                              \
+      const u32 s_ = (u32)__builtin_amdgcn_readfirstlane((int)(side_));                               \
+      const u32 op_ = s_ >> 8;        \
+      const __amdgpu_buffer_rsrc_t re_ = __builtin_amdgcn_make_buffer_rsrc(                           \
+          (void *)(esc + (int64_t)(op_ ? op_ - 1u : 0u) * PACK26_ESC_BYTES), 0,                       \
+          op_ ? PACK26_ESC_BYTES : 0, 0x00020000);                                                    \
+      r_.c[0] = __builtin_amdgcn_raw_buffer_load_b32(rs_, voffC, 0, AUXV);                            \
+      r_.c[1] = __builtin_amdgcn_raw_buffer_load_b32(re_, voffC, 0, AUXV);                            \
+      r_.b = (s_ & 0xffu) * 0x01010101u;                                                              \
+      r_.x = op_ != 0u;                                                                               \
+    } else {                                                                                          \
+      const scan_u32x2 c_ = __builtin_amdgcn_raw_buffer_load_b64(rs_, voffC, 0, AUXV);                \
+      r_.c[0] = c_[0];                                                                                \
+      r_.c[1] = c_[1];                                                                                \
+      r_.b = bases[(int64_t)t_ * nkb + k_];                                                           \
+      r_.x = false;                                                                                   \
+    }                                                                                                 \
     r_.p = __builtin_bit_cast(f32x4, __builtin_amdgcn_raw_buffer_load_b128(                           \
                                          rsrcP, voffP, k_ * (4 * 16 * VEC) * (int)sizeof(float), 0)); \
   }
   auto unpack = [](const Raw &r, f32x4(&v)[4]) {
+    u32 tops[4];
 #pragma unroll
     for (int u = 0; u < 4; u++) {
-      const u32 cw = r.c[u >> 1];
-      const u32 T = (((u & 1) ? cw >> 4 : cw) & 0x0f0f0f0fu) + r.b;
-      const u32 w0 = r.w[3 * u], w1 = r.w[3 * u + 1], w2 = r.w[3 * u + 2];
-      v[u][0] = __uint_as_float(__builtin_amdgcn_perm(T, w0, 0x04020100u));
-      v[u][1] = __uint_as_float(__builtin_amdgcn_perm(T, w1, 0x05020100u));
-      v[u][2] = __uint_as_float(__builtin_amdgcn_perm(T, w2, 0x06020100u));
-      v[u][3] = __uint_as_float(__builtin_amdgcn_perm(w1, w0, 0x0c0c0703u) |
-                                __builtin_amdgcn_perm(T, w2, 0x07030c0cu));
-    }
+      if constexpr (!F26)
+        tops[u] = pk28_tops(r.c[0], r.c[1], u, r.b);
+      else if constexpr (OPT & 8)
+        tops[u] = pk26_tops(r.c[0], u, r.b);
+      else
+        tops[u] = pk26_tops(r.c[0], u, r.b) + pk26_escape(r.c[1], u);
+    }
+    if constexpr (F26 && (OPT & 8)) {
+      if (r.x) {
+#pragma unroll
+        for (int u = 0; u < 4; u++) tops[u] += pk26_escape(r.c[1], u);
+      }
+    }
+#pragma unroll
+    for (int u = 0; u < 4; u++) {
+      u32 e[4];
+      pk_quad_decode(tops[u], r.w[3 * u], r.w[3 * u + 1], r.w[3 * u + 2], e);
+#pragma unroll
+      for (int jj = 0; jj < 4; jj++) v[u][jj] = __uint_as_float(e[jj]);
+    }
+  };
+  auto live_at = [&](int64_t t) {
+    return ((int64_t)((unsigned)t % (unsigned)n_mtiles) * 4 + wave) * (16 * VEC) < M;
   };
 
   Tile cur, nxt;
@@ -735,9 +768,22 @@
   f32x4 cv[4], cb;
   {
     Raw r0;
-    PPALS_PK_LOAD(id, 0, r0);
+    u32 sw0 = 0;
+    if constexpr (F26) sw0 = PPALS_PK_SIDE(id, 0);
+    PPALS_PK_LOAD(id, 0, r0, sw0);
     unpack(r0, cv);
     cb = r0.p;
+  }
+  u32 sw_next = 0;
+  if constexpr (F26) {
+    if (nkb > 1) {
+      sw_next = PPALS_PK_SIDE(id, 1);
+    } else {
+      int64_t t = id + gridDim.x;
+      for (; t < ntiles; t += gridDim.x)
+        if (live_at(t)) break;
+      sw_next = PPALS_PK_SIDE(t < ntiles ? t : id, 0);
+    }
   }
 
   for (;;) {
@@ -750,6 +796,12 @@
         break;
       }
     }
+    int64_t nnid = ntiles;
+    if constexpr (F26) {
+      if (nkb == 1 && has_next)
+        for (nnid = nid + gridDim.x; nnid < ntiles; nnid += gridDim.x)
+          if (live_at(nnid)) break;
+    }
     f32x4 acc[VEC];
     double acc64[VEC][4];
 #pragma unroll
@@ -766,7 +818,14 @@
         const bool same = kb + 1 < nkb;
         const int64_t pt = (same || !has_next) ? id : nid;
         const int pk = same ? kb + 1 : (has_next ? 0 : kb);
-        PPALS_PK_LOAD(pt, pk, nr);
+        u32 sw = 0;
+        if constexpr (F26) {
+          sw = sw_next;
+          const int64_t after = pt == id ? (has_next ? nid : ntiles) : nnid;
+          const bool stay = pk + 1 < nkb, hop = !stay && after < ntiles;
+          sw_next = PPALS_PK_SIDE(hop ? after : pt, stay ? pk + 1 : (hop ? 0 : pk));
+        }
+        PPALS_PK_LOAD(pt, pk, nr, sw);
         __builtin_amdgcn_sched_barrier(0);
 #pragma unroll
         for (int u = 0; u < VEC; u++)
@@ -823,6 +882,25 @@
     id = nid;
   }
 #undef PPALS_PK_LOAD
+#undef PPALS_PK_SIDE
+}
+
+template <int OPT>
+__global__ __launch_bounds__(256) __attribute__((amdgpu_waves_per_eu(3, 3))) void k_scan_suffix_pk(
+    const char *__restrict__ Vp, const unsigned int *__restrict__ bases, int64_t tile_bytes, int64_t M,
+    const float *__restrict__ P, int n_mtiles, int nkb, double *__restrict__ out, int64_t out_nstride,
+    int64_t out_batch_stride, int ncols, int out32, int64_t ntiles) {
+  scan_suffix_packed<PACK_FMT28, OPT>(Vp, bases, nullptr, tile_bytes, M, P, n_mtiles, nkb, out, out_nstride,
+                                      out_batch_stride, ncols, out32, ntiles);
+}
+
+template <int OPT>
+__global__ __launch_bounds__(256) __attribute__((amdgpu_waves_per_eu(3, 3))) void k_scan_suffix_pk2(
+    const char *__restrict__ Vp, const unsigned int *__restrict__ bases, const char *__restrict__ esc,
+    int64_t tile_bytes, int64_t M, const float *__restrict__ P, int n_mtiles, int nkb, double *__restrict__ out,
+    int64_t out_nstride, int64_t out_batch_stride, int ncols, int out32, int64_t ntiles) {
+  scan_suffix_packed<PACK_FMT26, OPT>(Vp, bases, esc, tile_bytes, M, P, n_mtiles, nkb, out, out_nstride,
+                                      out_batch_stride, ncols, out32, ntiles);
 }
 
 template <int NT, int OPT = 0>
diff --git a/pairwise-perturbation_amd/csrc/ops.h b/pairwise-perturbation_amd/csrc/ops.h
--- a/pairwise-perturbation_amd/csrc/ops.h
+++ b/pairwise-perturbation_amd/csrc/ops.h
@@ -8,6 +8,7 @@
 
 #include "bf16.h"
 #include "device_view.h"
+#include "pack_codec.h"
 #include "preload_policy.h"
 
 namespace ppals {
@@ -20,24 +21,24 @@
   int64_t ld = 0, valid = 0;
 };
 
-constexpr int PACK_BLOCK_BYTES = 14336, PACK_CODE_BYTES = 2048, PACK_QUAD_BYTES = 3072;
-constexpr int PACK_WINDOW = 16;
 struct PackedSrc {
   const void *data = nullptr;
   const void *bases = nullptr;
+  const void *esc = nullptr;
+  int format = 0;
+  int64_t escapes = 0;
   int64_t L = 0, J = 0, T = 0;
 };
-inline int64_t pack_tile_bytes(int64_t J) {
-  const int64_t kfull = J / 16, rem = J - kfull * 16;
-  return kfull * PACK_BLOCK_BYTES + (rem ? PACK_CODE_BYTES + (rem + 3) / 4 * PACK_QUAD_BYTES : 0);
+inline int64_t pack_tiles(int64_t L, int64_t T) { return (L + 255) / 256 * T; }
+inline int64_t pack_blocks_of(int64_t L, int64_t J, int64_t T) { return pack_tiles(L, T) * ((J + 15) / 16); }
+inline size_t pack_data_bytes(int fmt, int64_t L, int64_t J, int64_t T) {
+  return (size_t)pack_tiles(L, T) * (size_t)pack_tile_bytes(fmt, J);
 }
-inline int64_t pack_tiles(int64_t L, int64_t T) { return (L + 255) / 256 * T; }
-inline size_t pack_data_bytes(int64_t L, int64_t J, int64_t T) {
-  return (size_t)pack_tiles(L, T) * (size_t)pack_tile_bytes(J);
-}
-inline size_t pack_base_bytes(int64_t L, int64_t J, int64_t T) {
-  return (size_t)pack_tiles(L, T) * (size_t)((J + 15) / 16) * 4;
-}
+inline size_t pack_base_bytes(int64_t L, int64_t J, int64_t T) { return (size_t)pack_blocks_of(L, J, T) * 4; }
+struct PackSurvey {
+  int spread = -1;
+  int64_t escapes = 0;
+};
 
 constexpr int MAX_ORDER = 8;
 constexpr double kNnFloor = 1e-16;
@@ -126,10 +127,12 @@
   virtual void *try_alloc(size_t bytes) { return alloc(bytes); }
   virtual void scan_store_mode(int mode) { (void)mode; }
   virtual size_t mem_available() { return (size_t)-1; }
-  virtual int pack_layout(const void * , int , int64_t , int64_t , int64_t ,
-                          void * , void * ) {
-    return -1;
-  }
+  virtual PackSurvey pack_survey(const void * , int , int64_t , int64_t , int64_t ,
+                                 void * ) {
+    return PackSurvey();
+  }
+  virtual void pack_write(const void * , int64_t , int64_t , int64_t , int ,
+                          void * , void * , void * ) {}
   virtual void scan_packed_source(const PackedSrc * ) {}
   virtual int64_t scan_packed_launches() { return 0; }
 
diff --git a/pairwise-perturbation_amd/csrc/pack_codec.h b/pairwise-perturbation_amd/csrc/pack_codec.h
--- /dev/null
+++ b/pairwise-perturbation_amd/csrc/pack_codec.h
@@ -0,0 +1,96 @@
+#pragma once
+#include <stdint.h>
+
+#if defined(__HIPCC__)
+#define PPALS_PK_HD __host__ __device__ inline
+#else
+#define PPALS_PK_HD inline
+#endif
+
+namespace ppals {
+
+constexpr int PACK_FMT28 = 28, PACK_FMT26 = 26;
+constexpr int PACK_QUAD_BYTES = 3072;
+constexpr int PACK_CODE_BYTES = 2048, PACK26_CODE_BYTES = 1024;
+constexpr int PACK_BLOCK_BYTES = PACK_CODE_BYTES + 4 * PACK_QUAD_BYTES;
+constexpr int PACK26_BLOCK_BYTES = PACK26_CODE_BYTES + 4 * PACK_QUAD_BYTES;
+constexpr int PACK26_ESC_BYTES = 1024;
+constexpr int PACK_WINDOW = 16;
+constexpr int PACK26_WINDOW = 4;
+constexpr int64_t PACK26_MAX_ESCAPES = (1 << 24) - 1;
+
+constexpr int pack_code_bytes(int fmt) { return fmt == PACK_FMT26 ? PACK26_CODE_BYTES : PACK_CODE_BYTES; }
+constexpr int pack_block_bytes(int fmt) { return fmt == PACK_FMT26 ? PACK26_BLOCK_BYTES : PACK_BLOCK_BYTES; }
+PPALS_PK_HD int64_t pack_tile_bytes(int fmt, int64_t J) {
+  const int64_t kfull = J / 16, rem = J - kfull * 16;
+  return kfull * pack_block_bytes(fmt) + (rem ? pack_code_bytes(fmt) + (rem + 3) / 4 * PACK_QUAD_BYTES : 0);
+}
+
+PPALS_PK_HD int pk_code_offset(int fmt, int wave, int lane) {
+  return fmt == PACK_FMT26 ? wave * 256 + lane * 4 : wave * 512 + lane * 8;
+}
+PPALS_PK_HD int pk_quad_offset(int wave, int lane) { return wave * 768 + lane * 12; }
+
+PPALS_PK_HD int pack_choose_format(int mode, int spread, int64_t escapes, int64_t blocks) {
+  if (spread < 0 || spread >= PACK_WINDOW) return 0;
+  const bool ordinals_fit = escapes < PACK26_MAX_ESCAPES;
+  if (mode == 1) return PACK_FMT28;
+  if (mode == 2) return ordinals_fit ? PACK_FMT26 : 0;
+  return ordinals_fit && escapes * 16 <= blocks ? PACK_FMT26 : PACK_FMT28;
+}
+
+PPALS_PK_HD uint32_t pk_side_word(int fmt, uint32_t base, bool escape, uint32_t ordinal) {
+  if (fmt == PACK_FMT26) return base | (escape ? (ordinal + 1u) << 8 : 0u);
+  return base * 0x01010101u;
+}
+
+PPALS_PK_HD uint32_t pk_perm(uint32_t hi, uint32_t lo, uint32_t sel) {
+#if defined(__HIP_DEVICE_COMPILE__)
+  return __builtin_amdgcn_perm(hi, lo, sel);
+#else
+  const uint64_t both = ((uint64_t)hi << 32) | lo;
+  uint32_t r = 0;
+  for (int i = 0; i < 4; i++) {
+    const uint32_t s = (sel >> (8 * i)) & 0xffu;
+    uint32_t b;
+    if (s < 8) b = (uint32_t)(both >> (8 * s)) & 0xffu;
+    else if (s < 12) b = ((both >> (16 * (s - 8) + 15)) & 1u) ? 0xffu : 0u;
+    else if (s == 12) b = 0u;
+    else b = 0xffu;
+    r |= b << (8 * i);
+  }
+  return r;
+#endif
+}
+
+PPALS_PK_HD void pk_quad_encode(const uint32_t e[4], uint32_t q[3]) {
+  for (int i = 0; i < 3; i++) q[i] = (e[i] & 0xffffffu) | (((e[3] >> (8 * i)) & 0xffu) << 24);
+}
+PPALS_PK_HD void pk_quad_decode(uint32_t tops, uint32_t w0, uint32_t w1, uint32_t w2, uint32_t e[4]) {
+  e[0] = pk_perm(tops, w0, 0x04020100u);
+  e[1] = pk_perm(tops, w1, 0x05020100u);
+  e[2] = pk_perm(tops, w2, 0x06020100u);
+  e[3] = pk_perm(w1, w0, 0x0c0c0703u) |
+         pk_perm(tops, w2, 0x07030c0cu);
+}
+
+PPALS_PK_HD void pk28_put(uint32_t cw[2], int u, int jj, uint32_t code) {
+  cw[u >> 1] |= code << (8 * jj + 4 * (u & 1));
+}
+PPALS_PK_HD uint32_t pk28_tops(uint32_t cw0, uint32_t cw1, int u, uint32_t basew) {
+  const uint32_t cw = (u >> 1) ? cw1 : cw0;
+  return (((u & 1) ? cw >> 4 : cw) & 0x0f0f0f0fu) + basew;
+}
+
+PPALS_PK_HD void pk26_put(uint32_t &cw, uint32_t &ew, int u, int jj, uint32_t code) {
+  cw |= (code & 3u) << (8 * jj + 2 * u);
+  ew |= (code >> 2) << (8 * jj + 2 * u);
+}
+PPALS_PK_HD uint32_t pk26_tops(uint32_t cw, int u, uint32_t basew) {
+  return ((cw >> (2 * u)) & 0x03030303u) + basew;
+}
+PPALS_PK_HD uint32_t pk26_escape(uint32_t ew, int u) {
+  return (u == 0 ? ew << 2 : ew >> (2 * u - 2)) & 0x0c0c0c0cu;
+}
+
+}
```

Result: faster. 657.6, median of 6 (+5.6%).
